# pingooio/pingoo

Hardware: AMD Instinct MI355X
Metric: requests/sec matched (whole node), 1k-rule WAF (higher is better)
Workload: dtype u8

## Files before the change

### pingoo_amd/build.py

```python
from __future__ import annotations

import os
import shutil
import subprocess
import sys

HERE = os.path.dirname(os.path.abspath(__file__))
CSRC = os.path.join(HERE, "csrc")
LIB = os.path.join(HERE, "libpwaf.so")
SOURCES = ["frontend.cpp", "pattern.cpp", "dfa.cpp", "iptrie.cpp", "filter.cpp", "residual.cpp", "residual_jit.cpp", "rtc.cpp", "compile.cpp", "loaders.cpp", "batcher.cpp", "async.cpp", "node.cpp", "engine.cpp", "kernels.hip", "records.hip"]
HEADERS = ["frontend.h", "program.h", "kernels.h", "residual.h", "confirm.h", "records.h", "lscan_split.h", "dirtable.h", "georec.h", "unicode_data.inc", os.path.join("..", "..", "include", "pwaf.h")]


def hipcc() -> str:
    for cand in (os.environ.get("HIPCC"), shutil.which("hipcc"), "/opt/rocm/bin/hipcc"):
        if cand and os.path.exists(cand):
            return cand
    raise RuntimeError("hipcc not found (needed to build pingoo_amd/libpwaf.so)")


EMBED = os.path.join(CSRC, "residual_h.inc")


def embed() -> str:
    text = open(os.path.join(CSRC, "residual.h")).read()
    assert ')RVMH"' not in text
    out = 'R"RVMH(' + text + ')RVMH"\n'
    if not os.path.exists(EMBED) or open(EMBED).read() != out:
        with open(EMBED, "w") as f:
            f.write(out)
    return EMBED


def is_stale(lib: str = LIB) -> bool:
    if not os.path.exists(lib):
        return True
    t = os.path.getmtime(lib)
    return any(os.path.getmtime(os.path.join(CSRC, f)) > t for f in SOURCES + HEADERS)


def build(force: bool = False, verbose: bool = False, variant: str = "") -> str:
    lib = LIB if not variant else os.path.join(HERE, f"libpwaf_{variant}.so")
    if not force and not is_stale(lib):
        return lib
    embed()
    objs = []
    objdir = os.path.join(HERE, "build" + ("_" + variant if variant else ""))
    os.makedirs(objdir, exist_ok=True)
    cc = hipcc()
    common = ["-O3", "-std=c++17", "-fPIC", "-Wall", "-Wextra", "-Wno-unused-parameter", "-I", os.path.join(HERE, "..", "include")]
    common += os.environ.get("PWAF_EXTRA_CXXFLAGS", "").split()
    if variant == "prof":
        common.append("-DPWAF_PROFILING")
    procs = []
    for src in SOURCES:
        obj = os.path.join(objdir, src + ".o")
        objs.append(obj)
        path = os.path.join(CSRC, src)
        if not force and os.path.exists(obj) and os.path.getmtime(obj) > max(os.path.getmtime(path), *(os.path.getmtime(os.path.join(CSRC, h)) for h in HEADERS)):
            continue
        cmd = [cc, *common, "-c", path, "-o", obj]
        if src.endswith(".hip") or src in ("engine.cpp", "rtc.cpp"):
            cmd[1:1] = ["-x", "hip", "--offload-arch=gfx950"]
        else:
            cmd[1:1] = ["-x", "c++"] + (["-fsanitize=address,undefined", "-fno-omit-frame-pointer", "-g", "-O1"] if variant == "asan" else [])
        if verbose:
            print(" ".join(cmd), file=sys.stderr)
        procs.append((src, subprocess.Popen(cmd, stdout=subprocess.PIPE, stderr=subprocess.STDOUT, text=True)))
    for src, p in procs:
        out, _ = p.communicate()
        if p.returncode != 0:
            raise RuntimeError(f"hipcc failed on {src}:\n{out}")
        if verbose and out.strip():
            print(out, file=sys.stderr)
    link = [cc, "--offload-arch=gfx950", "-shared", "-fPIC", *(["-fsanitize=address,undefined", "-shared-libsan"] if variant == "asan" else []), "-o", lib, *objs]
    r = subprocess.run(link, stdout=subprocess.PIPE, stderr=subprocess.STDOUT, text=True)
    if r.returncode != 0:
        raise RuntimeError(f"link failed:\n{r.stdout}")
    return lib


if __name__ == "__main__":
    print(build(force="--force" in sys.argv, verbose=True, variant="prof" if "--prof" in sys.argv else "asan" if "--asan" in sys.argv else ""))
```

### pingoo_amd/csrc/engine.cpp

```cpp
#include <hip/hip_runtime_api.h>

#include <cstdio>
#include <algorithm>
#include <cstring>
#include <map>
#include <memory>
#include <mutex>
#include <string>
#include <type_traits>
#include <unordered_map>
#include <vector>

#include "dirtable.h"
#include "georec.h"
#include "frontend.h"
#include "kernels.h"
#include "lscan_split.h"
#include "program.h"
#include "records.h"

using namespace pwaf;

struct pwaf_program {
    std::unique_ptr<Program> p;
// ... 690 lines not shown
        pt[e->groups.size()] = PassInfo{P.fcmp_base, 0u};
        pt[e->groups.size() + (P.fcmp.empty() ? 0u : 1u)] = PassInfo{P.residual_base, e->residual_jit.function ? (3u << 24) : 0u};
        uint32_t fi = 0;
        for (size_t k = 0; k < e->groups.size(); k++) {
            const DevGroup &d = e->groups[k];
            pt[k].base = d.atom_base;
            pt[k].kind_slot = 0;
            if (d.short_lit) {
                pt[k].kind_slot = 3u << 24;
            } else if (d.filtered) {
                if (d.filter.heads.empty()) pt[k].kind_slot = (1u << 24) | fi;
                fi++;
            } else if (d.visit_slot >= 0) {
                pt[k].kind_slot = (2u << 24) | (uint32_t)d.visit_slot;
            }
        }
        if ((rc = upload(e->pass_table, pt))) return rc;
    }
    return upload(e->colmask, colmask);
}

Scratch &acquire_context(pwaf_engine *e, bool own, hipStream_t caller, std::unique_lock<std::mutex> &held, bool &must_wait) {
    must_wait = false;
    for (int pass = 0; pass < 2; pass++)
        for (auto &c : e->ctx) {
            std::unique_lock<std::mutex> l(c->mu, std::try_to_lock);
            if (!l.owns_lock()) continue;
            const bool ok = pass == 0 ? (c->used && (own ? c->last_own : (!c->last_own && c->last == caller))) : !c->used;
            if (ok) { held = std::move(l); return *c; }
        }
    size_t k;
    {
        std::lock_guard<std::mutex> lock(e->mu);
        k = e->next_ctx;
        e->next_ctx = (e->next_ctx + 1) % e->ctx.size();
    }
    held = std::unique_lock<std::mutex>(e->ctx[k]->mu);
    must_wait = e->ctx[k]->used;
    return *e->ctx[k];
}


struct Layout {
    size_t used = 0;
    size_t take(size_t bytes) { const size_t at = used; used = (used + bytes + 255) & ~(size_t)255; return at; }
    size_t size() const { return used; }
};

uint32_t slab_count(uint32_t total, uint32_t slab0) { return (uint32_t)(((uint64_t)total + kStreamSlab - 1) / kStreamSlab) - slab0; }
uint32_t slabs_of(const FilterArgs &f) { return slab_count(f.total, f.slab0); }
uint32_t pair_cap_of(uint32_t slabs, uint32_t n) { return (uint32_t)std::min<uint64_t>(0xFFFFFFF0u, (uint64_t)slabs * (kStreamSlab / 16) + n + 64); }

struct KernelTimer {
    pwaf_engine *e;
    hipStream_t stream;
    std::unique_lock<std::mutex> lock;
    size_t ev_i = 0;
    long last_main = -1;
    long open_begin = -1;
    bool streaming = false;
    const bool sync_each = switches().sync_each;
    KernelTimer(pwaf_engine *e_, hipStream_t stream_) : e(e_), stream(stream_) {
        if (!e->profiling) return;
        lock = std::unique_lock<std::mutex>(e->prof_mu);
        ev_i = e->n_timed;
    }
    bool off() const { return !e->profiling || (e->profiling == 2 && !streaming); }
    int record(hipStream_t on) {
        if (e->ev.size() < ev_i + 1) {
            hipEvent_t x;
            HIP_TRY(hipEventCreate(&x));
            e->ev.push_back(x);
        }
        HIP_TRY(hipEventRecord(e->ev[ev_i], on));
        ev_i++;
        return PWAF_OK;
    }
    int begin(hipStream_t side = nullptr) {
        if (off()) return PWAF_OK;
        if (!side && last_main >= 0) { open_begin = last_main; return PWAF_OK; }
        const int rc = record(side ? side : stream);
        if (rc) return rc;
        open_begin = (long)ev_i - 1;
        if (!side) last_main = open_begin;
        return PWAF_OK;
    }
    int end(const char *name, uint64_t alg_bytes, hipStream_t side = nullptr) {
        if (sync_each) {
            hipError_t se = hipStreamSynchronize(side ? side : stream);
            fprintf(stderr, "[pwaf] %s done: %s\n", name, hipGetErrorString(se));
        }
        if (off()) return PWAF_OK;
        const int rc = record(side ? side : stream);
        if (rc) return rc;
        if (!side) last_main = (long)ev_i - 1;
        pwaf_kernel_time t{};
        snprintf(t.name, sizeof t.name, "%s", name);
        t.alg_bytes = alg_bytes;
        e->times.push_back(t);
        e->time_ev.push_back({(size_t)open_begin, ev_i - 1});
        return PWAF_OK;
    }
    void commit() { e->n_timed = ev_i; }
};

struct ArgSlotMark {
    Scratch &S;
    hipStream_t stream;
    int slot = -1;
    int record() {
        if (slot < 0) return PWAF_OK;
        const int k = slot;
        slot = -1;
        S.arg_pending[k] = true;
        HIP_TRY(hipEventRecord(S.arg_ev[k], stream));
        return PWAF_OK;
    }
    ~ArgSlotMark() { (void)record(); }
};

struct BatchRun {
    pwaf_engine *e;
    Scratch &S;
    const Program &P;
    const pwaf_batch &db;
    hipStream_t stream;
    const std::vector<uint32_t> *col_begin;
    const Switches &sw;
    KernelTimer prof;
    ArgSlotMark arg_slot;
    uint32_t n, n_groups, residual_pass, n_passes, bit_words, pair_stride;
    size_t n_slots, ctrl_words;
    uint32_t pool_cap = 0;
    uint32_t *status_word = nullptr;
    bool zero_deferred = false;
    size_t zero_bytes = 0;
    std::vector<pwaf_strcol> cols;
    std::vector<uint32_t> col_bytes;
    std::vector<uint8_t> col_known;
    VerdictArgs v{};
    bool ipres_launched = false, attr_launched = false;
    pwaf_geo *d_geo = nullptr;
    ListShape lshapes[2];
    std::vector<uint32_t> filter_index;
    std::vector<FilterArgs> fall;
    std::vector<FilterArgs> by_stride[2];
    std::vector<ConfirmArgs> call;
    std::vector<ListScanArgs> la[2];
    ColPtrChunk ptrs{};
    uint64_t alg_bytes[3] = {0, 0, 0};
    const FilterArgs *d_all = nullptr, *d_s1 = nullptr, *d_s2 = nullptr;
    const ConfirmArgs *d_c = nullptr;
    const ListScanArgs *d_la[2] = {nullptr, nullptr};
    uint32_t *c_plan = nullptr, *l_plan = nullptr;

    BatchRun(pwaf_engine *e_, Scratch &S_, const pwaf_batch &db_, hipStream_t stream_, const std::vector<uint32_t> *col_begin_)
        : e(e_), S(S_), P(*e_->prog.p), db(db_), stream(stream_), col_begin(col_begin_), sw(switches()), prof(e_, stream_), arg_slot{S_, stream_} {
        n = db.n;
        n_groups = (n + 63) / 64;
        residual_pass = (uint32_t)e->groups.size() + (P.fcmp.empty() ? 0u : 1u);
        n_passes = residual_pass + (P.n_residual ? 1u : 0u);
        bit_words = 2 * n_groups;
        pair_stride = std::max(1u, e->n_bit_atoms + e->n_cmp_atoms + e->n_short);
        n_slots = (size_t)std::max(kGapLists, e->n_gated);
        ctrl_words = 2 + n_slots + e->n_filtered;
    }


    int reserve_scratch(bool sync_status) {
        int rc;
        const uint64_t pool_cap64 = std::max<uint64_t>(std::max<uint64_t>(1u << 20, (uint64_t)n * 8), S.pool_entries);
        pool_cap = (uint32_t)std::min<uint64_t>(pool_cap64, 0x7FFFFFF0u);
        S.pool_entries = pool_cap;
        if (!S.status.p) {
            if ((rc = S.status.reserve(8))) return rc;
            HIP_TRY(hipMemsetAsync(S.status.p, 0, 8, stream));
        }
        status_word = (uint32_t *)S.status.p + (sync_status ? 1 : 0);
        if ((rc = S.rec.reserve((size_t)std::max(1u, n_passes) * n * 4))) return rc;
        if ((rc = S.attr.reserve(((size_t)n_groups * pair_stride + 64) * 16 + (size_t)n_groups * 4))) return rc;
        if ((rc = S.pool.reserve((size_t)pool_cap * sizeof(PoolEntry)))) return rc;
        uint32_t n_conf = 0;
        for (const DevGroup &d : e->groups) n_conf += (d.filtered && d.confirm) ? 1u : 0u;
        Layout z;
        const size_t z_ctrl = z.take(4 * ctrl_words), z_cand = z.take((size_t)e->n_filtered * bit_words * 4), z_visit = z.take((size_t)e->n_visit * bit_words * 4),
                     z_walk = z.take((size_t)n_conf * bit_words * 4);
        zero_bytes = z.size();
        if ((rc = S.zero_block.reserve(zero_bytes))) return rc;
        zero_deferred = e->n_filtered != 0;
        for (const DevGroup &d : e->groups) zero_deferred = zero_deferred && (d.gate >= 0 || d.identity || d.short_lit);
        if (!zero_deferred) HIP_TRY(hipMemsetAsync(S.zero_block.p, 0, zero_bytes, stream));
        char *const zbase = (char *)S.zero_block.p;
        S.ctrl.p = zbase + z_ctrl;
        S.cand_bits.p = zbase + z_cand;
        S.visit_bits.p = zbase + z_visit;
        S.walk_bits.p = zbase + z_walk;
        if (e->n_gated && (rc = S.gate_lists.reserve((size_t)e->n_gated * n * 4))) return rc;
        if (e->n_need && (rc = S.need.reserve((size_t)e->n_need * n * 4))) return rc;
        return PWAF_OK;
    }

    int resolve_columns(bool totals_known) {
        int rc;
        cols.resize(e->n_fields);
        col_bytes.assign(e->n_fields, 0);
        for (int f = 0; f < PWAF_N_FIELDS; f++) {
            cols[(size_t)f] = db.field[f];
            col_bytes[(size_t)f] = db.field_bytes[f];
        }
        bool missing_header = false;
        for (uint32_t f = PWAF_N_FIELDS; f < e->n_fields; f++) {
            const uint32_t k = f - PWAF_N_FIELDS;
            if (k < db.n_headers && db.headers != nullptr && db.headers[k].data != nullptr && db.headers[k].offsets != nullptr) {
                cols[f] = db.headers[k];
                col_bytes[f] = db.header_bytes ? db.header_bytes[k] : 0u;
            } else {
                missing_header = true;
            }
        }
        if (missing_header) {
            if (S.zero_off.cap < (size_t)(n + 1) * 4 + PWAF_ARENA_PAD) {
                if ((rc = S.zero_off.reserve((size_t)(n + 1) * 4 + PWAF_ARENA_PAD))) return rc;
                HIP_TRY(hipMemsetAsync(S.zero_off.p, 0, S.zero_off.cap, stream));
            }
            for (uint32_t f = PWAF_N_FIELDS; f < e->n_fields; f++)
                if (cols[f].data == nullptr) {
                    cols[f].data = (const uint8_t *)S.zero_off.p;
                    cols[f].offsets = (const uint32_t *)S.zero_off.p;
                    col_bytes[f] = 0;
                }
        }
        col_known.assign(e->n_fields, totals_known ? 1 : 0);
        for (uint32_t f = 0; f < e->n_fields; f++)
            if (col_bytes[f] != 0 || cols[f].data == (const uint8_t *)S.zero_off.p) col_known[f] = 1;
        return PWAF_OK;
    }

    int fill_verdict_args(pwaf_verdict *d_out, pwaf_counts *d_counts, uint32_t *d_match_idx, uint32_t *d_n_matches) {
        int rc;
        v.n = n;
        v.n_groups = n_groups;
        v.force_global_tables = (P.flags & PWAF_OPT_GLOBAL_VERDICT_TABLES) ? 1u : 0u;
        v.sparse_mode = verdict_mode(P.flags);
        if (v.sparse_mode) {
            const VerdictShape vs = verdict_shape(P.n_cols, (uint32_t)P.rules.size(), e->n_trig, (uint32_t)P.lits.size(), v.force_global_tables != 0, (int)v.sparse_mode, n_passes);
            v.v_cap = vs.v_cap;
            const bool entry_list = v.sparse_mode >= 3;
            const uint32_t spill_cols = entry_list ? P.n_cols : P.n_cols - std::min(vs.v_cap, P.n_cols);
            if (entry_list || spill_cols) {
                if ((rc = S.verdict_spill.reserve((size_t)verdict_blocks_sp(vs, e->n_cus) * vs.waves * spill_cols * 8))) return rc;
                v.spill = (unsigned long long *)S.verdict_spill.p;
            }
        }
        v.debug_skip = sw.debug_skip | (sw.attr_prio ? 0x80000000u : 0u);
        for (int f = 0; f < PWAF_N_FIELDS; f++) v.off[f] = db.field[f].offsets;
        v.ip = db.ip;
        v.ip_is_v6 = db.ip_is_v6;
        v.port = db.port;
        v.flags = db.flags;
        v.asn = db.asn;
        v.country = db.country;
        v.n_cols = P.n_cols;
        v.n_passes = n_passes;
        v.rec = (const uint32_t *)S.rec.p;
        v.passes = (const PassInfo *)e->pass_table.p;
        if (P.n_residual && e->residual_jit.function) {
            v.res_words = (P.n_residual + 31u) / 32u;
            v.res_base = P.residual_base;
            if ((rc = S.res_words.reserve((size_t)v.res_words * n * 4))) return rc;
            v.res_match = (const uint32_t *)S.res_words.p;
        }
        v.cand_bits = (const uint32_t *)S.cand_bits.p;
        v.visit_bits = (const uint32_t *)S.visit_bits.p;
        v.bit_words = bit_words;
        v.n_hlen = (uint32_t)e->hlen_fields.size();
        for (size_t k = 0; k < e->hlen_fields.size(); k++) v.hoff[k] = cols[e->hlen_fields[k]].offsets;
        v.gpairs = (uint4 *)S.attr.p;
        v.ghdr = (uint32_t *)((char *)S.attr.p + ((size_t)n_groups * pair_stride + 64) * 16);
        v.pair_stride = pair_stride;
        v.attr_blocks = e->n_cus;
        v.pool = (const PoolEntry *)S.pool.p;
        v.cmp = (const CmpAtomDev *)e->num_atoms.p;
        v.n_cmp = e->n_cmp_atoms;
        v.cmp_vars = e->cmp_vars;
        v.lazy = (const CmpAtomDev *)e->lazy_atoms.p;
        v.n_lazy = e->n_lazy;
        v.n_lazy_var = (uint32_t)e->lazy_vars.size();
        for (size_t k = 0; k < e->lazy_vars.size(); k++) v.lazy_var[k] = e->lazy_vars[k];
        v.n_short = e->n_short;
        v.short_atoms = (const ShortAtom *)e->short_atoms.p;
        if (e->n_short) {
            v.short_data = cols[(size_t)e->short_field].data;
            v.short_off = cols[(size_t)e->short_field].offsets;
        }
        v.n_trig = e->n_trig;
        v.n_lits = (uint32_t)P.lits.size();
        v.bit_col = (const uint32_t *)e->bit_atoms.p;
        v.trig_off = (const uint32_t *)e->trig_off.p;
        v.trig_rules = (const uint16_t *)e->trig_rules.p;
        v.always_rules = (const uint32_t *)e->always_rules.p;
        for (int var = 0; var < 2; var++) {
            v.iu_vals[var] = (const int64_t *)e->iu_vals[var].p;
            v.iu_masks[var] = (const uint32_t *)e->iu_masks[var].p;
            v.iu_n[var] = e->iu_n[var];
            v.iu_words[var] = e->iu_words[var];
        }
        v.country_masks = (const uint32_t *)e->country_luts.p;
        v.cc_words = e->cc_words;
        v.rules = (const DevRule *)e->rules.p;
        v.n_rules = (uint32_t)P.rules.size();
        v.lits = (const uint32_t *)e->lits.p;
        set_trie_args(e, v);
        if ((rc = S.ipres.reserve((size_t)n * (v.ipres_packed ? 4 : 8) + 64))) return rc;
        v.ipres = (uint32_t *)S.ipres.p;
        v.out = d_out;
        v.counts = (unsigned long long *)d_counts;
        v.match_idx = d_match_idx;
        v.n_matches = d_n_matches;
        return PWAF_OK;
    }

    int zero_head_records() {
        for (size_t k = 0; k < e->groups.size();) {
            size_t k1 = k;
            while (k1 < e->groups.size() && e->groups[k1].filtered && !e->groups[k1].filter.heads.empty()) k1++;
            if (k1 == k) { k++; continue; }
            HIP_TRY(hipMemsetAsync((uint32_t *)S.rec.p + k * (size_t)n, 0, (k1 - k) * (size_t)n * 4, stream));
            k = k1;
        }
        return PWAF_OK;
    }

    void pick_list_shapes() {
        uint32_t variant[2] = {2, 0};
        bool all_confirm = e->n_filtered != 0;
        for (const DevGroup &d : e->groups) all_confirm = all_confirm && (!d.filtered || d.confirm);
        if (all_confirm) variant[0] = 0;
        if (sw.list_shape >= 0) {
            variant[0] = (uint32_t)sw.list_shape & 15u;
            variant[1] = (uint32_t)sw.list_shape >> 4;
        }
        for (int phase = 0; phase < 2; phase++) lshapes[phase] = list_shape(variant[phase]);
    }


    template <class Launch>
    int timed(const char *name, uint64_t bytes, const char *what, Launch &&launch, hipStream_t side = nullptr) {
        const int rc = prof.begin(side);
        if (rc) return rc;
        const int he = launch();
        if (he) return fail(PWAF_E_DEVICE, std::string(what) + " launch failed: " + hipGetErrorString((hipError_t)he));
        return prof.end(name, bytes, side);
    }

    template <class Launch>
    int side_stage(hipStream_t q, const char *name, uint64_t code, const char *what, Launch &&launch) {
        const hipStream_t side = q != stream ? q : nullptr;
        const int rc = timed(name, code, what, launch, side);
        if (rc) return rc;
        if (side) HIP_TRY(hipEventRecord(S.ev_join, q));
        return PWAF_OK;
    }
    int ipres_stage(hipStream_t q) {
        if (ipres_launched) return PWAF_OK;
        ipres_launched = true;
        if (q != stream) {
            HIP_TRY(hipEventRecord(S.ev_fork, stream));
            HIP_TRY(hipStreamWaitEvent(q, S.ev_fork, 0));
        }
        const int rc = side_stage(q, "ipres", 0xFAu, "ipres kernel", [&] { return sw.skip_ipres ? (int)hipMemsetAsync(v.ipres, 0, (size_t)n * (v.ipres_packed ? 4 : 8), q) : launch_ipres(v, q); });
        if (rc || !d_geo) return rc;
        GeoRecArgs ga{};
        set_georec_args(e, ga);
        ga.ip = db.ip;
        ga.ip_is_v6 = db.ip_is_v6;
        ga.asn = db.asn;
        ga.country = db.country;
        ga.n = n;
        ga.out = (uint2 *)d_geo;
        return side_stage(q, "georec", 25ull * n, "georec kernel", [&] { return launch_georec(ga, q); });
    }
    int attr_stage(hipStream_t q) {
        if (attr_launched) return PWAF_OK;
        attr_launched = true;
        if (q == stream && sw.placement == 0) HIP_TRY(hipStreamWaitEvent(stream, S.ev_join, 0));
        return side_stage(q, "attr", 0xFEu, "attribute kernel", [&] { return sw.skip_attr ? (int)hipMemsetAsync(v.ghdr, 0, (size_t)n_groups * 4, q) : launch_attr(v, q); });
    }
    int attr_at_start() {
        int rc;
        if (sw.placement == 0) return ipres_stage(S.side);
        if (sw.placement == 3) return (rc = ipres_stage(S.side)) ? rc : attr_stage(S.side);
        return PWAF_OK;
    }
    int attr_after_filter() {
        int rc;
        switch (sw.placement) {
        case 0: return attr_stage(stream);
        case 1: return (rc = ipres_stage(stream)) ? rc : attr_stage(stream);
        case 2: return (rc = ipres_stage(S.side)) ? rc : attr_stage(S.side);
        default: return PWAF_OK;
        }
    }
    int join_side() {
        if (sw.placement >= 2) HIP_TRY(hipStreamWaitEvent(stream, S.ev_join, 0));
        return PWAF_OK;
    }

    int launch_plain_scans() {
        static const char *fn[5] = {"host", "url", "path", "method", "user_agent"};
        for (size_t gi = 0; gi < e->groups.size(); gi++) {
            const DevGroup &d = e->groups[gi];
            if (d.gate >= 0 || d.identity || d.short_lit) continue;
            const ScanArgs a = scan_args(gi);
            char nm[48];
            if (d.field < PWAF_N_FIELDS) snprintf(nm, sizeof nm, "scan_%s_g%zu", fn[d.field], gi);
            else snprintf(nm, sizeof nm, "scan_hdr%u_g%zu", d.field - PWAF_N_FIELDS, gi);
            prof.streaming = true;
            const int rc = timed(nm, (uint64_t)col_bytes[d.field] + 4ull * (n + 1), "scan kernel", [&] { return launch_scan(a, stream); });
            prof.streaming = false;
            if (rc) return rc;
        }
        return PWAF_OK;
    }

    int launch_filter_stage() {
        prof.streaming = true;
        const int rc = timed(by_stride[1].empty() ? "filter_s1" : by_stride[0].empty() ? "filter_s2" : "filter_mix", alg_bytes[1] + alg_bytes[2], "filter kernel", [&] {
            return launch_filter(by_stride[0].data(), (uint32_t)by_stride[0].size(), d_s1, by_stride[1].data(), (uint32_t)by_stride[1].size(), d_s2, stream);
        });
        prof.streaming = false;
        return rc;
    }
    int launch_resolve_stage() {
        bool any_list = false;
        for (const DevGroup &d : e->groups) any_list = any_list || (d.filtered && !d.confirm);
        return timed("resolve+compact", 0xFCu, "resolve / compact kernel", [&] {
            const int he = launch_resolve(fall.data(), (uint32_t)fall.size(), d_all, stream);
            return !he && any_list ? launch_compact(fall.data(), (uint32_t)fall.size(), d_all, stream) : he;
        });
    }
    int launch_confirm_stage() {
        if (call.empty()) return PWAF_OK;
        return timed("confirm", 0xF8u, "confirm kernel", [&] { return launch_confirm(call.data(), (uint32_t)call.size(), d_c, c_plan, e->n_cus, stream); });
    }
    int launch_list_scans() {
        uint32_t *plan_at = l_plan;
        for (int phase = 0; phase < 2; phase++) {
            uint32_t first = 0;
            for (const uint32_t cnt : e->lscan_launches[phase]) {
                char nm[48];
                snprintf(nm, sizeof nm, "lscan_x%u", cnt);
                const int rc = timed(nm, 0xFDu, "gated scan kernel", [&] { return launch_scan_gated(la[phase].data() + first, cnt, d_la[phase] + first, plan_at, lshapes[phase], stream); });
                if (rc) return rc;
                plan_at += 2 * cnt + 1;
                first += cnt;
            }
        }
        return PWAF_OK;
    }
    int launch_fcmp_stage() {
        if (P.fcmp.empty()) return PWAF_OK;
        FcmpArgs fa{};
        std::vector<uint32_t> slots;
        for (size_t k = 0; k < P.fcmp.size(); k++) {
            uint32_t sl[2];
            const uint32_t fld[2] = {P.fcmp[k].a, P.fcmp[k].b};
            for (int q = 0; q < 2; q++) {
                size_t at = std::find(slots.begin(), slots.end(), fld[q]) - slots.begin();
                if (at == slots.size()) slots.push_back(fld[q]);
                sl[q] = (uint32_t)at;
            }
            fa.atoms[k] = P.fcmp[k].op | (sl[0] << 8) | (sl[1] << 16);
        }
        for (size_t q = 0; q < slots.size() && q < kMaxFcmpFields; q++) {
            fa.data[q] = cols[slots[q]].data;
            fa.off[q] = cols[slots[q]].offsets;
        }
        fa.n = n;
        fa.n_atoms = (uint32_t)P.fcmp.size();
        fa.rec = (uint32_t *)S.rec.p + e->groups.size() * (size_t)n;
        set_pool(fa);
        return timed("fcmp", 0xFBu, "field comparison kernel", [&] { return launch_fcmp(fa, stream); });
    }
    template <class Args>
    int residual_inputs(Args &a) {
        a.data = (const uint8_t *const *)S.res_cols.p;
        a.off = (const uint32_t *const *)((const char *)S.res_cols.p + (size_t)e->n_fields * 8);
        a.blob = (const uint8_t *)e->residual_blob.p;
        a.n = n;
        a.n_rules = P.n_residual;
        a.ip = db.ip;
        a.ip_is_v6 = db.ip_is_v6;
        a.port = db.port;
        a.asn = db.asn;
        a.country = db.country;
        a.has_geo = (P.has_geo && P.residual_needs_geo) ? 1u : 0u;
        a.geo_root4 = (const uint32_t *)e->geo_rec_root4.p;
        a.geo_root6 = (const uint32_t *)e->geo_rec_root6.p;
        a.geo_nodes = (const uint32_t *)e->geo_rec_nodes.p;
        a.geo_recs = (const GeoRec *)e->geo_recs.p;
        a.rule_errors = (unsigned long long *)e->residual_errors.p;
        if (S.retry) {
            const int rc = S.err_sink.reserve((size_t)P.n_residual * 8);
            if (rc) return rc;
            a.rule_errors = (unsigned long long *)S.err_sink.p;
        }
        return PWAF_OK;
    }
    int launch_residual_stage() {
        if (!P.n_residual) return PWAF_OK;
        int rc;
        if (e->residual_jit.function) {
            ResidualJitArgs ja{};
            if ((rc = residual_inputs(ja))) return rc;
            ja.match_words = (uint32_t *)S.res_words.p;
            return timed("residual_jit", 0xF9u, "specialized residual kernel", [&] { return launch_residual_jit(e->residual_jit, ja, e->n_cus, stream); });
        }
        ResidualArgs ra{};
        if ((rc = residual_inputs(ra))) return rc;
        ra.rec = (uint32_t *)S.rec.p + (size_t)residual_pass * n;
        set_pool(ra);
        return timed("residual", 0xF9u, "residual kernel", [&] { return launch_residual(ra, stream); });
    }
    int launch_verdict_stage() { return timed("verdict", 0xFFu, "verdict kernel", [&] { return launch_verdict(v, stream); }); }
    int dump_counts() {
        std::vector<uint32_t> cw(ctrl_words);
        HIP_TRY(hipStreamSynchronize(stream));
        HIP_TRY(hipMemcpy(cw.data(), S.ctrl.p, 4 * ctrl_words, hipMemcpyDeviceToHost));
        fprintf(stderr, "[pwaf] n %u pool %u status %u |", n, cw[0], cw[1]);
        for (size_t k = 0; k < e->groups.size(); k++) {
            const DevGroup &d = e->groups[k];
            if (d.gate >= 0) fprintf(stderr, " pass %zu field %u %s list %u", k, d.field, d.filtered ? (d.confirm ? "confirm" : "filtered") : "gap", cw[2 + (size_t)d.gate]);
        }
        for (uint32_t k = 0; k < e->n_filtered; k++) fprintf(stderr, " pairs[%u] %u", k, cw[2 + n_slots + k]);
        fprintf(stderr, "\n");
        return PWAF_OK;
    }


    template <class Args>
    void set_pool(Args &a) const {
        a.pool = (PoolEntry *)S.pool.p;
        a.pool_count = (uint32_t *)S.ctrl.p;
        a.pool_cap = pool_cap;
        a.status = status_word;
    }
    bool feeds_gates(size_t gi) const { return e->n_gap && e->owns_factors[gi]; }
    template <class Args>
    void set_gate_feed(Args &a, const DevGroup &d) const {
        a.colmask_local = (const uint32_t *)e->colmask.p + d.atom_base;
        a.n_local = d.n_local;
        a.gate_lists = (uint32_t *)S.gate_lists.p;
        a.gate_count = (uint32_t *)S.ctrl.p + 2;
        if constexpr (!std::is_same<Args, ScanArgs>::value) {
            a.enq_bits = (uint32_t *)S.visit_bits.p;
            a.enq_words = bit_words;
        }
    }

    ScanArgs scan_args(size_t gi) const {
        const DevGroup &d = e->groups[gi];
        ScanArgs a{};
        if (feeds_gates(gi)) set_gate_feed(a, d);
        a.data = cols[d.field].data;
        a.off = cols[d.field].offsets;
        a.n = n;
        a.tab = (const uint16_t *)d.tab.p;
        a.classmap = (const uint8_t *)d.classmap.p;
        a.umap = d.scalar_mode ? (const uint8_t *)d.classmap.p + kUmapAt : nullptr;
        a.ill_class = d.ill_class;
        a.special = (const SpecialCell *)d.special.p;
        a.list_off = (const uint32_t *)d.list_off.p;
        a.list = (const uint16_t *)d.list.p;
        a.start_emit = d.start_emit;
        a.emit_base = d.emit_base;
        a.n_cus = e->n_cus;
        a.chunks = d.chunks;
        a.special_base = d.special_base;
        a.n_states = d.n_states;
        a.stride = d.stride;
        a.n_classes = d.n_classes;
        a.n_hot = d.n_hot;
        a.rec = (uint32_t *)S.rec.p + gi * (size_t)n;
        set_pool(a);
        return a;
    }

    int learn_arena_sizes() {
        bool ask = false;
        for (const DevGroup &d : e->groups)
            if (d.filtered && !col_known[d.field]) {
                HIP_TRY(hipMemcpyAsync(&col_bytes[d.field], cols[d.field].offsets + n, 4, hipMemcpyDeviceToHost, stream));
                ask = true;
            }
        if (ask) HIP_TRY(hipStreamSynchronize(stream));
        return PWAF_OK;
    }

    uint32_t slab0_of(uint32_t field) const { return col_begin ? (*col_begin)[field] / kStreamSlab : 0u; }

    int build_filter_args() {
        int rc;
        filter_index.assign(e->groups.size(), 0);
        if (!e->n_filtered) return PWAF_OK;
        const uint32_t words = (n + 31) / 32, n_cblocks = (words + kCompactWords - 1) / kCompactWords;
        uint64_t sub_entries = 0, n_slabs_all = 0, pair_bytes = 0;
        for (const DevGroup &d : e->groups)
// ... 69 lines not shown
        }
        return PWAF_OK;
    }

    ConfirmArgs confirm_args(const FilterArgs &f, const DevGroup &d, size_t gi, uint32_t wi) const {
        ConfirmArgs c{};
        c.data = f.data;
        c.off = f.off;
        c.n = n;
        c.total = f.total;
        c.pairs = f.pairs;
        c.pair_count = f.pair_count;
        c.pair_cap = f.pair_cap;
        c.mul = f.mul;
        c.stride = f.stride;
        c.init = f.init;
        c.ftable = f.table;
        c.c_head = (const uint32_t *)d.c_head.p;
        c.c_entries = (const ConfirmEntry *)d.c_entries.p;
        c.c_bytes = (const uint8_t *)d.c_bytes.p;
        c.c_classes = (const uint32_t *)d.c_classes.p;
        c.n_entries = (uint32_t)d.filter.confirm.entries.size();
        c.n_bytes = (uint32_t)d.filter.confirm.bytes.size() & ~3u;
        c.n_class_words = (uint32_t)d.filter.confirm.classes.size();
        c.rec = f.rec;
        c.valid_bits = f.bitmap;
        c.dense_flag = f.dense_flag;
        c.dense_thresh = f.dense_thresh;
        c.walk_bits = (uint32_t *)S.walk_bits.p + (size_t)wi * bit_words;
        if (d.confirm_walk) {
            c.walk_list = f.list;
            c.walk_count = f.list_count;
        }
        set_pool(c);
        if (feeds_gates(gi)) {
            set_gate_feed(c, d);
            c.shared_bits = d.shared_bits;
        }
        return c;
    }
    void build_confirm_args() {
        for (size_t gi = 0; gi < e->groups.size(); gi++) {
            const DevGroup &d = e->groups[gi];
            if (d.filtered && d.confirm) call.push_back(confirm_args(fall[filter_index[gi]], d, gi, (uint32_t)call.size()));
        }
    }

    ListScanArgs list_args(size_t gi, const ListShape &lshape, bool full_table = false) const {
        const DevGroup &d = e->groups[gi];
        ListScanArgs a{};
        const DevGroup &src = d.share_owner >= 0 ? e->groups[(size_t)d.share_owner] : d;
        if (!d.identity) {
            a.req_list = (const uint32_t *)S.gate_lists.p + (size_t)src.gate * n;
            a.n_list = (const uint32_t *)S.ctrl.p + 2 + src.gate;
        }
        if (d.visit_slot >= 0) a.visited = (uint32_t *)S.visit_bits.p + (size_t)d.visit_slot * bit_words;
        if (d.share_owner >= 0) {
            a.need_in = (const uint32_t *)S.need.p + (size_t)src.need_slot * n;
            a.need_bit = (uint32_t)d.gate;
        }
        if (feeds_gates(gi)) {
            set_gate_feed(a, d);
            if (d.need_slot >= 0) {
                a.need_out = (uint32_t *)S.need.p + (size_t)d.need_slot * n;
                a.shared_bits = d.shared_bits;
            }
        }
        if (d.confirm) a.merge_rec = 1;
        a.behind_filter = d.filtered ? 1u : 0u;
        a.data = cols[d.field].data;
        a.off = cols[d.field].offsets;
        a.n = n;
        const FlatDev &F = (d.confirm && d.rt.n_states && !full_table) ? d.rt : d.fl;
        a.flat = (const uint16_t *)F.flat.p;
        a.classmap = (const uint8_t *)F.flat_classmap.p;
        a.umap = F.scalar_mode ? (const uint8_t *)F.flat_classmap.p + kUmapAt : nullptr;
        a.ill_class = F.ill_class;
        a.n_classes = F.n_classes;
        const uint32_t row_bytes = 2u * (F.n_classes + 3u), hb = list_hot_bytes(lshape);
        if (F.n_delta && (uint64_t)F.n_full * row_bytes + 48u + 8ull * F.n_delta <= hb) {
            a.n_hot = F.n_full;
            a.n_delta = F.n_delta;
            a.delta = (const uint64_t *)F.delta.p;
        } else {
            a.n_hot = std::min<uint32_t>(F.n_delta ? F.n_full : F.n_states, (hb - 48u) / row_bytes);
        }
        a.emit_off = (const uint32_t *)F.emit_off.p;
        a.emit_list = (const uint16_t *)F.emit_list.p;
        a.end_off = (const uint32_t *)F.end_off.p;
        a.end_list = (const uint16_t *)F.end_list.p;
        a.rec = (uint32_t *)S.rec.p + gi * (size_t)n;
        set_pool(a);
        a.n_cus = e->n_cus;
        return a;
    }
    const FilterArgs *dense_of(size_t gi) const {
        const FilterArgs *f = e->groups[gi].filtered ? &fall[filter_index[gi]] : nullptr;
        return f && f->dense_flag ? f : nullptr;
    }
    static void set_dense(ListScanArgs &a, const FilterArgs &f, uint32_t mode) {
        a.dense_flag = f.dense_flag;
        a.dense_thresh = f.dense_thresh;
        a.dense_mode = mode;
    }
    void build_list_args() {
        for (int phase = 0; phase < 2; phase++)
            for (size_t gi = 0; gi < e->groups.size(); gi++) {
                const DevGroup &d = e->groups[gi];
                if (d.identity ? phase != 0 : (d.gate < 0 || d.filtered != (phase == 0))) continue;
                const FilterArgs *const dense = phase == 0 && d.confirm ? dense_of(gi) : nullptr;
                const FilterArgs *const owner_dense = d.share_owner >= 0 ? dense_of((size_t)d.share_owner) : nullptr;
                if (dense) {
                    ListScanArgs a = list_args(gi, lshapes[phase], true);
                    a.req_list = nullptr;
                    a.n_list = nullptr;
                    a.merge_rec = 0;
                    a.visited = (uint32_t *)S.cand_bits.p + (size_t)filter_index[gi] * bit_words;
                    set_dense(a, *dense, 1);
                    la[phase].push_back(a);
                }
                if (d.confirm && !d.confirm_walk) continue;
                if (sw.skip_identity && d.identity) continue;
                ListScanArgs a = list_args(gi, lshapes[phase]);
                if (dense) set_dense(a, *dense, 2);
                else if (owner_dense) set_dense(a, *owner_dense, 3);
                la[phase].push_back(a);
            }
    }
    int check_list_plan() const {
        for (int phase = 0; phase < 2; phase++) {
            size_t planned = 0;
            for (const uint32_t c : e->lscan_launches[phase]) planned += c;
            if (planned != la[phase].size()) return fail(PWAF_E_DEVICE, "list-scan launch plan does not match the batch's descriptors");
        }
        return PWAF_OK;
    }
    void build_column_pointers() {
        if (!P.n_residual) return;
        const size_t nc = e->n_fields;
        ptrs.count = (uint32_t)(2 * nc);
        for (size_t f = 0; f < nc; f++) { ptrs.p[f] = cols[f].data; ptrs.p[nc + f] = cols[f].offsets; }
    }

    int upload_descriptors() {
        int rc;
        struct Part { size_t at; const void *src; size_t bytes; };
        const size_t b_all = fall.size() * sizeof(FilterArgs), b_s1 = by_stride[0].size() * sizeof(FilterArgs), b_s2 = by_stride[1].size() * sizeof(FilterArgs),
                     b_c = call.size() * sizeof(ConfirmArgs), b_l0 = la[0].size() * sizeof(ListScanArgs), b_l1 = la[1].size() * sizeof(ListScanArgs),
                     b_ptrs = (size_t)ptrs.count * sizeof(void *);
        Layout L;
        const Part up[7] = {{L.take(b_all), fall.data(), b_all}, {L.take(b_s1), by_stride[0].data(), b_s1}, {L.take(b_s2), by_stride[1].data(), b_s2}, {L.take(b_c), call.data(), b_c},
                            {L.take(b_l0 + sizeof(ListScanArgs)), la[0].data(), b_l0}, {L.take(b_l1 + sizeof(ListScanArgs)), la[1].data(), b_l1}, {L.take(b_ptrs), ptrs.p, b_ptrs}};
        const size_t up_bytes = L.size();
        const size_t a_cplan = L.take((call.size() + 2) * 4), a_lplan = L.take((lsplit::plan_words(e->lscan_launches[0]) + lsplit::plan_words(e->lscan_launches[1])) * 4);
        if ((rc = S.args.reserve(L.size()))) return rc;
        char *const abase = (char *)S.args.p;
        d_all = (const FilterArgs *)(abase + up[0].at);
        d_s1 = (const FilterArgs *)(abase + up[1].at);
        d_s2 = (const FilterArgs *)(abase + up[2].at);
        d_c = (const ConfirmArgs *)(abase + up[3].at);
        d_la[0] = (const ListScanArgs *)(abase + up[4].at);
        d_la[1] = (const ListScanArgs *)(abase + up[5].at);
        S.res_cols.p = abase + up[6].at;
        c_plan = (uint32_t *)(abase + a_cplan);
        l_plan = (uint32_t *)(abase + a_lplan);
        if (up_bytes) {
            const uint32_t slot = S.arg_next++ % Scratch::kArgSlots;
            if (S.arg_pending[slot]) HIP_TRY(hipEventSynchronize(S.arg_ev[slot]));
            if ((rc = S.arg_slot[slot].reserve(up_bytes))) return rc;
            char *const hb = (char *)S.arg_slot[slot].p;
            for (const Part &p : up)
                if (p.bytes) memcpy(hb + p.at, p.src, p.bytes);
            arg_slot.slot = (int)slot;
            const int he = upload_args_block(hb, S.args.p, up_bytes, zero_deferred ? S.zero_block.p : nullptr, zero_deferred ? zero_bytes : 0, stream);
            if (he) return fail(PWAF_E_DEVICE, std::string("descriptor upload failed: ") + hipGetErrorString((hipError_t)he));
        } else if (zero_deferred) {
            HIP_TRY(hipMemsetAsync(S.zero_block.p, 0, zero_bytes, stream));
        }
        zero_deferred = false;
        return PWAF_OK;
    }
};

int run_pipeline(pwaf_engine *e, Scratch &S, const pwaf_batch &db , pwaf_verdict *d_out, pwaf_counts *d_counts, uint32_t *d_match_idx,
                 uint32_t *d_n_matches, hipStream_t stream, bool totals_known = false, const std::vector<uint32_t> *col_begin = nullptr, bool sync_status = false,
                 pwaf_geo *d_geo = nullptr, const HitOut *d_hits = nullptr) {
    if (db.n == 0) return PWAF_OK;
    BatchRun b(e, S, db, stream, col_begin);
    b.d_geo = d_geo;
    int rc;
    if ((rc = b.reserve_scratch(sync_status)) || (rc = b.resolve_columns(totals_known))) return rc;
    if ((rc = b.fill_verdict_args(d_out, d_counts, d_match_idx, d_n_matches)) || (rc = b.zero_head_records())) return rc;
    if (d_hits && d_hits->any()) {
        b.v.hits = d_hits->hits;
        b.v.hits_cap = d_hits->cap;
        b.v.n_hits = d_hits->n_hits;
        b.v.rule_hits = (unsigned long long *)d_hits->rule_hits;
    }
    b.pick_list_shapes();
    if ((rc = b.attr_at_start()) || (rc = b.launch_plain_scans())) return rc;
    if ((rc = b.learn_arena_sizes()) || (rc = b.build_filter_args())) return rc;
    b.build_confirm_args();
    b.build_list_args();
    b.build_column_pointers();
    if ((rc = b.check_list_plan()) || (rc = b.upload_descriptors())) return rc;
    if (e->n_filtered) {
        if ((rc = b.launch_filter_stage())) return rc;
        if (!b.sw.attr_after_compact && (rc = b.attr_after_filter())) return rc;
        if ((rc = b.launch_resolve_stage()) || (rc = b.launch_confirm_stage())) return rc;
    }
    if ((rc = b.attr_after_filter())) return rc;
    if ((rc = b.launch_list_scans()) || (rc = b.launch_fcmp_stage()) || (rc = b.launch_residual_stage())) return rc;
    if ((rc = b.join_side()) || (rc = b.launch_verdict_stage())) return rc;
    if (b.sw.dump_counts && (rc = b.dump_counts())) return rc;
    if ((rc = b.arg_slot.record())) return rc;
    b.prof.commit();
    return PWAF_OK;
}

hipError_t mark_context_used(Scratch &S, hipStream_t s, bool own) {
    S.used = true;
    S.last = s;
    S.last_own = own;
    return hipEventRecord(S.done, s);
}

int device_error(const char *call, hipError_t he) { return fail(PWAF_E_DEVICE, std::string(call) + ": " + hipGetErrorString(he)); }

template <class After>
int run_with_retry(pwaf_engine *e, Scratch &S, const pwaf_batch &db, pwaf_verdict *d_out, pwaf_counts *d_counts, bool known, const std::vector<uint32_t> *begins, bool counts_zero,
                   After &&after, pwaf_geo *d_geo = nullptr, const HitOut *d_hits = nullptr) {
    const hipStream_t s = S.stream;
    int r = S.pin_status.reserve(16);
    volatile uint32_t *const st = (volatile uint32_t *)S.pin_status.p;
    for (int attempt = 0;; attempt++) {
        hipError_t he = hipSuccess;
        if (!r && d_counts && !(counts_zero && attempt == 0) && (he = hipMemsetAsync(d_counts, 0, sizeof *d_counts, s)) != hipSuccess) r = device_error("hipMemsetAsync", he);
        if (!r && d_hits && d_hits->n_hits && (he = hipMemsetAsync(d_hits->n_hits, 0, 4, s)) != hipSuccess) r = device_error("hipMemsetAsync", he);
        if (!r && d_hits && d_hits->rule_hits && e->prog.p->n_user_rules && (he = hipMemsetAsync(d_hits->rule_hits, 0, (size_t)e->prog.p->n_user_rules * 8, s)) != hipSuccess)
            r = device_error("hipMemsetAsync", he);
        if (!r) {
            S.retry = attempt > 0;
            r = run_pipeline(e, S, db, d_out, d_counts, nullptr, nullptr, s, known, begins, true, d_geo, d_hits);
            S.retry = false;
        }
        if (!r) {
            he = hipMemcpyAsync((void *)&st[0], (uint32_t *)S.status.p + 1, 4, hipMemcpyDeviceToHost, s);
            if (he == hipSuccess) he = hipMemcpyAsync((void *)&st[1], S.ctrl.p, 4, hipMemcpyDeviceToHost, s);
            r = he != hipSuccess ? device_error("hipMemcpyAsync", he) : after();
        }
        const hipError_t re = mark_context_used(S, s, true), se = hipStreamSynchronize(s);
        if (r) return r;
        if (re != hipSuccess) return device_error("hipEventRecord", re);
        if (se != hipSuccess) return device_error("hipStreamSynchronize", se);
        if (!st[0]) return PWAF_OK;
        HIP_TRY(hipMemsetAsync((uint32_t *)S.status.p + 1, 0, 4, s));
        if (attempt >= 2 || st[1] >= 0x7FFFFFF0u) return fail(PWAF_E_NOMEM, "scan overflow pool exhausted: verdicts of this batch are incomplete");
        S.pool_entries = (uint64_t)st[1] + st[1] / 4 + 1024;
    }
}

struct DeviceBatch {
    pwaf_batch db{};
    std::vector<pwaf_strcol> hdr_cols;
    std::vector<uint32_t> hdr_bytes;
    DeviceBatch(uint32_t n, uint32_t n_fields) : hdr_cols(n_fields - PWAF_N_FIELDS, pwaf_strcol{nullptr, nullptr}), hdr_bytes(n_fields - PWAF_N_FIELDS, 0) {
        db.struct_size = sizeof db;
        db.n = n;
        db.memory = PWAF_MEM_DEVICE;
        db.n_headers = (uint32_t)hdr_cols.size();
        db.headers = hdr_cols.empty() ? nullptr : hdr_cols.data();
        db.header_bytes = hdr_bytes.empty() ? nullptr : hdr_bytes.data();
    }
    DeviceBatch(const DeviceBatch &) = delete;
    void set_col(uint32_t f, const void *data, const void *offsets, uint32_t bytes) {
        const pwaf_strcol c{(const uint8_t *)data, (const uint32_t *)offsets};
        if (f < PWAF_N_FIELDS) {
            db.field[f] = c;
            db.field_bytes[f] = bytes;
        } else {
            hdr_cols[f - PWAF_N_FIELDS] = c;
            hdr_bytes[f - PWAF_N_FIELDS] = bytes;
        }
    }
    void set_fixed(const void *ip, const void *ip_is_v6, const void *port, const void *flags, const void *asn, const void *country) {
        db.ip = (const uint8_t *)ip;
        db.ip_is_v6 = (const uint8_t *)ip_is_v6;
        db.port = (const uint16_t *)port;
        db.flags = (const uint8_t *)flags;
        db.asn = (const uint32_t *)asn;
        db.country = (const uint16_t *)country;
    }
};

}

extern "C" {

uint32_t pwaf_abi_version(void) { return PWAF_ABI_VERSION; }
const char *pwaf_last_error(void) { return g_last_error.c_str(); }

int pwaf_compile_expression(const char *expression, char *errbuf, size_t errbuf_len) {
    Syntax syn;
    std::string err;
    bool ok = expression && parse_expression(expression, syn, err);
    if (!ok) {
        std::string m = "Expression is not valid: " + (expression ? err : std::string("null expression"));
        if (errbuf && errbuf_len) snprintf(errbuf, errbuf_len, "%s", m.c_str());
        return fail(PWAF_E_SYNTAX, m);
    }
    return PWAF_OK;
}

int pwaf_validate_expression(const char *expression, char *errbuf, size_t errbuf_len) {
    auto bad = [&](const std::string &why) {
        std::string m = "Expression is not valid: " + why;
        if (errbuf && errbuf_len) snprintf(errbuf, errbuf_len, "%s", m.c_str());
        return fail(PWAF_E_SYNTAX, m);
// ... 1418 lines not shown
```

### pingoo_amd/csrc/kernels.h

```cpp
#pragma once
#include <cstdint>
#include <string>
#include <vector>

#include "program.h"

namespace pwaf {

static constexpr int kMaxPasses = 250;
static constexpr int kVerdictPre = 12;
static constexpr uint32_t kGapLists = 32;
static constexpr uint32_t kMaxHeaderLens = 8;
static constexpr uint32_t kDirChunkWords = 32;

static constexpr uint32_t REC_OVERFLOW = 0x80000000u;
struct PoolEntry {
    uint32_t atom;
    uint32_t next;
};

struct SpecialCell {
    uint32_t next_off;
    uint32_t emit;
};
struct ScanArgs {
    const uint8_t *data;
    const uint32_t *off;
    uint32_t n;
    const uint16_t *tab;
    const uint8_t *classmap;
    const uint8_t *umap;
    uint32_t ill_class;
    const SpecialCell *special;
    const uint32_t *list_off;
    const uint16_t *list;
    uint32_t n_states, stride, n_classes, n_hot;
    uint32_t start_emit;
    uint32_t emit_base, special_base;
    uint32_t n_cus;
    uint32_t chunks;
    uint32_t *rec;
    PoolEntry *pool;
    uint32_t *pool_count;
    uint32_t pool_cap;
    uint32_t *status;
    const uint32_t *colmask_local;
    uint32_t n_local;
    uint32_t *gate_lists;
    uint32_t *gate_count;
};

static constexpr uint32_t kListThreads = 512;
static constexpr uint32_t kListWalks = 1;
static constexpr uint32_t kListHotBytes = 48 * 1024;
struct ListScanArgs {
    const uint8_t *data;
    const uint32_t *off;
    uint32_t n;
    const uint16_t *flat;
    const uint8_t *classmap;
    const uint8_t *umap;
    uint32_t ill_class;
    uint32_t n_classes;
    uint32_t n_hot;
    const uint64_t *delta;
    uint32_t n_delta;
    const uint32_t *emit_off;
    const uint16_t *emit_list;
    const uint32_t *end_off;
    const uint16_t *end_list;
    uint32_t *rec;
    PoolEntry *pool;
    uint32_t *pool_count;
    uint32_t pool_cap;
    uint32_t *status;
    const uint32_t *colmask_local;
    uint32_t n_local;
    uint32_t *gate_lists;
    uint32_t *gate_count;
    uint32_t *enq_bits;
    uint32_t enq_words;
    uint32_t behind_filter;
    const uint32_t *req_list;
    const uint32_t *n_list;
    uint32_t *visited;
    uint32_t *need_out;
    uint32_t shared_bits;
    const uint32_t *need_in;
    uint32_t need_bit;
    uint32_t merge_rec;
    uint32_t n_cus;
    const uint32_t *dense_flag;
    uint32_t dense_thresh;
    uint32_t dense_mode;
};
struct ListOf {
    const uint32_t *req_list;
    uint32_t n_l;
};

struct ConfirmArgs {
    const uint8_t *data;
    const uint32_t *off;
    uint32_t n;
    uint32_t total;
    const uint2 *pairs;
    const uint32_t *pair_count;
    uint32_t pair_cap;
    uint32_t mul, stride, init;
    const uint32_t *ftable;
    const uint32_t *c_head;
    const ConfirmEntry *c_entries;
    const uint8_t *c_bytes;
    const uint32_t *c_classes;
    uint32_t n_entries, n_bytes, n_class_words;
    uint32_t *rec;
    uint32_t *valid_bits;
    uint32_t *walk_bits;
    uint32_t *walk_list;
    uint32_t *walk_count;
    PoolEntry *pool;
    uint32_t *pool_count;
    uint32_t pool_cap;
    uint32_t *status;
    const uint32_t *colmask_local;
    uint32_t n_local;
    uint32_t *gate_lists;
    uint32_t *gate_count;
    uint32_t *enq_bits;
    uint32_t enq_words;
    uint32_t shared_bits;
    const uint32_t *dense_flag;
    uint32_t dense_thresh;
};
static constexpr uint32_t kConfirmThreads = 1024;
static constexpr uint32_t kConfirmPoolBytes = 40 * 1024;
struct ConfirmTableDev {
    const ConfirmArgs *c;
    uint32_t count;
};
int launch_confirm(const ConfirmArgs *host, uint32_t count, const ConfirmArgs *dev, uint32_t *plan, uint32_t n_cus, void *stream);

static constexpr uint32_t kStreamSlab = 128 * 1024;
static constexpr uint32_t kStreamIter = 4096;
static constexpr uint32_t kFilterWaves = 4;
static constexpr uint32_t kCompactWords = 2048;
struct FilterArgs {
    const uint8_t *data;
    const uint32_t *off;
    uint32_t n;
    uint32_t total;
    uint32_t slab0;
    uint32_t init;
    uint32_t mul;
    uint32_t stride;
    const uint32_t *table;
    uint32_t n_heads;
    uint32_t head_w[2][4];
    uint32_t head_m[2][4];
    uint32_t head_len[2];
    uint32_t head_code[2];
    uint32_t *rec;
    uint32_t *chunk_bits;
    uint32_t *sub_count;
    uint32_t *bitmap;
    uint32_t *block_count;
    uint32_t *list;
    uint32_t *list_count;
    uint2 *pairs;
    uint32_t *pair_count;
    uint32_t pair_cap;
    uint32_t *pair_base;
    const uint32_t *dense_flag;
    uint32_t dense_thresh;
    uint32_t first_block;
    uint32_t debug;
};
int upload_args_block(const void *host_pinned, void *dev, size_t bytes, void *zero , size_t zero_bytes, void *stream);
struct FilterTable {
    const FilterArgs *f;
    uint32_t count;
};
struct FilterMix {
    const FilterArgs *f1, *f2;
    uint32_t count1, count2, blocks1, blocks2;
};
int launch_filter(const FilterArgs *host1, uint32_t count1, const FilterArgs *dev1, const FilterArgs *host2, uint32_t count2, const FilterArgs *dev2, void *stream);
int launch_resolve(const FilterArgs *host, uint32_t count, const FilterArgs *dev, void *stream);
int launch_compact(const FilterArgs *host, uint32_t count, const FilterArgs *dev, void *stream);
int configure_kernels(int device);

static constexpr uint32_t kSrcSet = 0, kSetWordsMax = 16, kSrcCc = 16, kCcWordsMax = 8, kSrcPort = 24, kSrcAsn = 28, kIntWordsMax = 4, kSrcAcmp = 32, kAcmpWordsMax = 4,
                          kSrcWords = 36;
struct PassInfo {
    uint32_t base;
    uint32_t kind_slot;
};
struct FcmpArgs {
    const uint8_t *data[kMaxFcmpFields];
    const uint32_t *off[kMaxFcmpFields];
    uint32_t atoms[kMaxFcmpAtoms];
    uint32_t n, n_atoms;
    uint32_t *rec;
    PoolEntry *pool;
    uint32_t *pool_count;
    uint32_t pool_cap;
    uint32_t *status;
};
int launch_fcmp(const FcmpArgs &a, void *stream);
struct ResidualArgs {
    const uint8_t *const *data;
    const uint32_t *const *off;
    const uint8_t *blob;
    uint32_t n, n_rules;
    const uint8_t *ip;
    const uint8_t *ip_is_v6;
    const uint16_t *port;
    const uint32_t *asn;
    const uint16_t *country;
    uint32_t has_geo;
    const uint32_t *geo_root4, *geo_root6, *geo_nodes;
    const GeoRec *geo_recs;
    uint32_t *rec;
    PoolEntry *pool;
    uint32_t *pool_count;
    uint32_t pool_cap;
    uint32_t *status;
    unsigned long long *rule_errors;
};
int launch_residual(const ResidualArgs &a, void *stream);
struct ResidualJitArgs {
    const uint8_t *const *data;
    const uint32_t *const *off;
    const uint8_t *blob;
    uint32_t n, n_rules;
    const uint8_t *ip;
    const uint8_t *ip_is_v6;
    const uint16_t *port;
    const uint32_t *asn;
    const uint16_t *country;
    uint32_t has_geo, pad;
    const uint32_t *geo_root4, *geo_root6, *geo_nodes;
    const GeoRec *geo_recs;
    uint32_t *match_words;
    unsigned long long *rule_errors;
};
struct JitKernel {
    void *module = nullptr, *function = nullptr;
};
static constexpr uint32_t kMaxJitRules = 256;
bool rvm_specialize(const uint8_t *blob, size_t len, std::string &out, std::string &why);
bool rvm_jit_program(const uint8_t *blob, size_t len, std::string &out, std::string &why);
bool rtc_compile(const std::string &source, const std::string &arch, std::vector<char> &code, std::string &why);
bool jit_load(const std::vector<char> &code, JitKernel &out, std::string &why);
void jit_release(JitKernel &k);
int launch_residual_jit(const JitKernel &k, const ResidualJitArgs &a, uint32_t n_cus, void *stream);
struct ColPtrChunk {
    const void *p[2 * (PWAF_N_FIELDS + kMaxHeaders)];
    uint32_t count;
};
struct CmpAtomDev {
    uint32_t col, c;
};
struct ShortAtom {
    uint32_t col;
    uint32_t len_exact;
    uint32_t lit_lo, lit_hi;
};
struct VerdictArgs {
    uint32_t n, n_groups;
    uint32_t debug_skip;
    uint32_t force_global_tables;
    uint32_t sparse_mode;
    uint32_t v_cap;
    unsigned long long *spill;
    const uint32_t *off[PWAF_N_FIELDS];
    const uint8_t *ip;
    const uint8_t *ip_is_v6;
    const uint16_t *port;
    const uint8_t *flags;
    const uint32_t *asn;
    const uint16_t *country;
    uint32_t n_passes;
    const uint32_t *rec;
    const PassInfo *passes;
    const uint32_t *res_match;
    uint32_t res_words, res_base;
    const uint32_t *cand_bits, *visit_bits;
    uint32_t bit_words;
    const uint32_t *hoff[kMaxHeaderLens];
    const ShortAtom *short_atoms;
    uint32_t n_short;
    const uint8_t *short_data;
    const uint32_t *short_off;
    uint32_t n_hlen;
    const PoolEntry *pool;
    uint32_t n_cols;
    const CmpAtomDev *cmp;
    uint32_t n_cmp;
    uint32_t cmp_vars;
    const CmpAtomDev *lazy;
    uint32_t n_lazy;
    uint32_t lazy_var[4], n_lazy_var;
    const uint32_t *bit_col;
    const int64_t *iu_vals[2];
    const uint32_t *iu_masks[2];
    uint32_t iu_n[2], iu_words[2];
    const uint32_t *country_masks;
    uint32_t cc_words;
    const DevRule *rules;
    uint32_t n_rules;
    const uint32_t *lits;
    uint32_t n_lits, n_trig;
    const uint32_t *trig_off;
    const uint16_t *trig_rules;
    const uint32_t *always_rules;
    const uint32_t *ip_root4, *ip_root6, *ip_nodes;
    const uint32_t *set_masks;
    uint32_t set_words;
    uint32_t n_ip_lists;
    const uint32_t *geo_root4, *geo_root6, *geo_nodes;
    const uint32_t *dir24;
    const uint32_t *dir_chunks, *dir_vals;
    const uint32_t *dir_summary;
    uint32_t dir_sum_shift, dir_common;
    const uint2 *dir_esc;
    const uint32_t *class_rows;
    uint32_t class_words;
    uint32_t acmp_words;
    uint32_t geo_default;
    uint32_t *ipres;
    uint32_t ipres_packed;
    uint32_t has_geo;
    uint4 *gpairs;
    uint32_t *ghdr;
    uint32_t pair_stride;
    uint32_t attr_blocks;
    pwaf_verdict *out;
    unsigned long long *counts;
    uint32_t *match_idx;
    uint32_t *n_matches;
    pwaf_rule_hit *hits;
    uint32_t hits_cap;
    uint32_t *n_hits;
    unsigned long long *rule_hits;
};

int launch_scan(const ScanArgs &a, void *stream);
struct GatedTable {
    const ListScanArgs *g;
    uint32_t count;
    uint32_t debug;
};
struct ListShape {
    uint32_t threads, hot_bytes, wg_per_cu;
};
ListShape list_shape(uint32_t variant);
uint32_t list_hot_bytes(const ListShape &shape);
int launch_scan_gated(const ListScanArgs *host, uint32_t count, const ListScanArgs *dev, uint32_t *plan, const ListShape &shape, void *stream);
int launch_verdict(const VerdictArgs &a, void *stream);
int launch_ipres(const VerdictArgs &a, void *stream);
int launch_attr(const VerdictArgs &a, void *stream);
int launch_dir24(const VerdictArgs &a, void *out , void *esc, void *esc_count, void *stream);
struct GeoRecArgs {
    const uint8_t *ip, *ip_is_v6;
    const uint32_t *asn;
    const uint16_t *country;
    uint32_t n, has_geo;
    const uint32_t *root4, *root6, *nodes;
    const GeoRec *recs;
    const uint32_t *chunks, *vals, *summary;
    uint32_t sum_shift, common;
    uint32_t n_cus;
    uint2 *out;
};
int launch_georec(const GeoRecArgs &a, void *stream);
uint32_t scan_lds_bytes(uint32_t n_hot, uint32_t stride, uint32_t n_gate_atoms);
struct VerdictShape {
    uint32_t waves, lds_bytes, lds_tables;
    uint32_t sparse, v_cap, per_cu;
};
VerdictShape verdict_shape(uint32_t n_cols, uint32_t n_rules, uint32_t n_trig, uint32_t n_lits, bool force_global = false, int mode = 3, uint32_t n_passes = 0);
uint32_t verdict_blocks_sp(const VerdictShape &sh, uint32_t n_cus);

}
```

### pingoo_amd/csrc/kernels.hip

```cpp
#include <hip/hip_runtime.h>

#include <cstdlib>
#include <mutex>
#include <set>

#include "confirm.h"
#include "utf8.h"
#include "kernels.h"
#include "residual.h"

namespace pwaf {

static constexpr int kScanThreads = 1024;
static constexpr int kScanWaves = kScanThreads / 64;
static constexpr uint32_t kNone = 0xFFFFFFFFu;

#define PWAF_LDS __attribute__((address_space(3)))
#define PWAF_GLOBAL __attribute__((address_space(1)))
typedef const PWAF_LDS uint16_t *lds_u16_ptr;
typedef const PWAF_GLOBAL uint16_t *glb_u16_ptr;
typedef const PWAF_LDS uint32_t *lds_u32_ptr;
typedef const PWAF_LDS uint8_t *lds_u8_ptr;
typedef unsigned int u32x4 __attribute__((ext_vector_type(4)));
typedef u32x4 u32x4_u __attribute__((aligned(1)));

static constexpr uint32_t kClsBytes = 1024;
uint32_t scan_lds_bytes(uint32_t n_hot, uint32_t stride, uint32_t n_gate_atoms) {
    const uint32_t need = (((n_hot + 1) * stride * 2 + 15) & ~15u) + kClsBytes + n_gate_atoms * 4;
    const uint32_t reach = ((0xFFFFu << 1) + stride * 2 + kClsBytes + 15) & ~15u;
    return need > reach ? need : reach;
}


struct Hits {
    uint32_t a0, a1;
    uint32_t ovf;
};

struct SlowCtx {
    const uint32_t *list_off;
    const uint16_t *list;
    PoolEntry *pool;
    uint32_t *pool_count;
    uint32_t *status;
    uint32_t pool_cap;
};

__device__ __forceinline__ Hits pool_push(const SlowCtx &c, uint32_t atom, Hits h) {
    const uint32_t idx = atomicAdd(c.pool_count, 1u);
    if (idx >= c.pool_cap) {
        atomicOr(c.status, 1u);
        return h;
    }
    c.pool[idx].atom = atom;
    c.pool[idx].next = h.ovf;
    h.ovf = idx;
    return h;
}

__device__ __forceinline__ Hits record_atom(const SlowCtx &c, uint32_t atom, Hits h) {
    if (h.ovf == kNone) {
        if (h.a0 == atom + 1 || h.a1 == atom + 1) return h;
        if (h.a0 == 0) { h.a0 = atom + 1; return h; }
        if (h.a1 == 0) { h.a1 = atom + 1; return h; }
        const uint32_t x0 = h.a0 - 1, x1 = h.a1 - 1;
        h = pool_push(c, x0, h);
        h = pool_push(c, x1, h);
        return pool_push(c, atom, h);
    }
    for (uint32_t i = h.ovf; i != kNone;) {
        const uint32_t at = __hip_atomic_load(&c.pool[i].atom, __ATOMIC_RELAXED, __HIP_MEMORY_SCOPE_AGENT);
        if (at == atom) return h;
        i = __hip_atomic_load(&c.pool[i].next, __ATOMIC_RELAXED, __HIP_MEMORY_SCOPE_AGENT);
    }
    return pool_push(c, atom, h);
}

__device__ __noinline__ Hits emit_list(const uint32_t *list_off, const uint16_t *list, PoolEntry *pool, uint32_t *pool_count, uint32_t *status,
                                       uint32_t pool_cap, uint32_t id, Hits h) {
    const SlowCtx c{list_off, list, pool, pool_count, status, pool_cap};
    const uint32_t b = list_off[id], e = list_off[id + 1];
    for (uint32_t k = b; k < e; k++) h = record_atom(c, list[k], h);
    return h;
}
struct Walk {
    uint32_t row, crow;
    Hits h;
};
__device__ __noinline__ Walk careful_step(const PWAF_GLOBAL unsigned char *gtab, const SpecialCell *special, const uint32_t *list_off, const uint16_t *list,
                                          PoolEntry *pool, uint32_t *ctrl , uint32_t pool_cap, uint32_t hot_emit ,
                                          uint32_t special_col , uint32_t prev, uint32_t crow, uint32_t c2k, uint32_t t, uint32_t a0,
                                          uint32_t a1, uint32_t ovf) {
    const SlowCtx c{list_off, list, pool, ctrl, ctrl + 1, pool_cap};
    const uint32_t hot_elems = hot_emit & 0xFFFFu, emit_base = hot_emit >> 16, special_base = special_col & 0xFFFFu, emit_col2 = special_col >> 16;
    const Hits h{a0, a1, ovf};
    uint32_t cell = t;
    if (prev == hot_elems) cell = *reinterpret_cast<glb_u16_ptr>(gtab + crow + c2k);
    Walk w{cell, crow, h};
    if (cell >= special_base) {
        const SpecialCell sp = special[cell - special_base];
        w.row = hot_elems;
        w.crow = sp.next_off;
        if (sp.emit) {
            const uint32_t b = list_off[sp.emit - 1], e = list_off[sp.emit];
            for (uint32_t k = b; k < e; k++) w.h = record_atom(c, list[k], w.h);
        }
    } else if (cell >= emit_base) {
        const uint32_t code = *reinterpret_cast<lds_u16_ptr>((uintptr_t)((cell << 1) + emit_col2 + kClsBytes));
        if (code & 0x8000u) {
            w.h = record_atom(c, code & 0x7FFFu, w.h);
        } else {
            const uint32_t b = list_off[code - 1], e = list_off[code];
            for (uint32_t k = b; k < e; k++) w.h = record_atom(c, list[k], w.h);
        }
    }
    return w;
}
__device__ __forceinline__ Hits hits_of_record(const uint32_t rv) {
    if (rv & REC_OVERFLOW) return Hits{0, 0, rv & ~REC_OVERFLOW};
    return Hits{rv & 0x7FFFu, (rv >> 15) & 0x7FFFu, kNone};
}
__device__ __noinline__ uint32_t gate_mask(const uint32_t *colmask_local, const PoolEntry *pool, Hits h) {
    uint32_t need = 0;
    if (h.ovf != kNone) {
        for (uint32_t i = h.ovf; i != kNone;) {
            need |= colmask_local[__hip_atomic_load(&pool[i].atom, __ATOMIC_RELAXED, __HIP_MEMORY_SCOPE_AGENT)];
            i = __hip_atomic_load(&pool[i].next, __ATOMIC_RELAXED, __HIP_MEMORY_SCOPE_AGENT);
        }
    } else {
        if (h.a0) need |= colmask_local[h.a0 - 1];
        if (h.a1) need |= colmask_local[h.a1 - 1];
    }
    return need;
}
__device__ __noinline__ void enqueue_mask(uint32_t *gate_lists, uint32_t *gate_count, uint32_t n, uint32_t r, uint32_t need) {
    while (need) {
        const uint32_t g = (uint32_t)__builtin_ctz(need);
        need &= need - 1;
        gate_lists[(size_t)g * n + atomicAdd(&gate_count[g], 1u)] = r;
    }
}
__device__ __noinline__ void enqueue_mask_once(uint32_t *gate_lists, uint32_t *gate_count, uint32_t n, uint32_t r, uint32_t need, uint32_t *enq_bits, uint32_t enq_words) {
    while (need) {
        const uint32_t g = (uint32_t)__builtin_ctz(need);
        need &= need - 1;
        if (enq_bits != nullptr) {
            const uint32_t bit = 1u << (r & 31u);
            if (atomicOr(&enq_bits[(size_t)g * enq_words + (r >> 5)], bit) & bit) continue;
        }
        gate_lists[(size_t)g * n + atomicAdd(&gate_count[g], 1u)] = r;
    }
}
__device__ __forceinline__ void enqueue_gated(const uint32_t *colmask_local, const PoolEntry *pool, uint32_t *gate_lists, uint32_t *gate_count, uint32_t n,
                                              uint32_t r, Hits h) {
    enqueue_mask(gate_lists, gate_count, n, r, gate_mask(colmask_local, pool, h));
}

__device__ __forceinline__ uint32_t wave_index() { return (uint32_t)__builtin_amdgcn_readfirstlane((int)(threadIdx.x >> 6)); }

// ... 106 lines not shown
        if (want != 0 && next < w1) {
            const uint32_t avail = min(w1 - next, blk + 64 - next);
            const uint32_t rank = (uint32_t)__builtin_popcountll(want & lt_mask);
            const bool take = last && r2 == kNone && rank < avail;
            const uint32_t j = take ? next + rank - blk : 0;
            const uint32_t lo = (uint32_t)__builtin_amdgcn_ds_bpermute((int)(j << 2), (int)o_lo);
            const uint32_t hi = (uint32_t)__builtin_amdgcn_ds_bpermute((int)(j << 2), (int)o_hi);
            if (take) {
                r2 = next + rank;
                p2 = lo;
                end2 = hi;
            }
            next += min((uint32_t)__builtin_popcountll(want), avail);
            if (next == blk + 64 && next < w1) {
                blk += 64;
                if (n_base == blk) {
                    o_lo = n_lo;
                    o_hi = n_hi;
                } else {
                    load_off(blk, o_lo, o_hi);
                }
            }
        }
        if (__ballot(r != kNone || r2 != kNone) == 0) break;
        {
            const bool have = last ? (r2 != kNone && p2 < end2) : true;
            const uint32_t np = have ? (last ? p2 : p + kStep) : 0u;
            const uint32_t nend = last ? end2 : end;
#pragma unroll
            for (int q = 0; q < CH; q++) {
                const uint32_t at = (q == 0 || (have && np + 16u * q < nend)) ? np + 16u * q : 0u;
                wn[q] = *reinterpret_cast<const PWAF_GLOBAL u32x4_u *>(gdata + at);
            }
        }

        const bool act = r != kNone && p < end;
        const uint32_t cnt_all = act ? min(kStep, end - p) : 0u;
#pragma unroll
        for (int q = 0; q < CH; q++) {
        const uint32_t cnt = cnt_all > 16u * q ? min(16u, cnt_all - 16u * q) : 0u;
        const uint32_t wd[4] = {w[q].x, w[q].y, w[q].z, w[q].w};
        uint32_t c2[16];
#pragma unroll
        for (int k = 0; k < 16; k++) {
            const uint32_t byte = (wd[k >> 2] >> ((k & 3) * 8)) & 0xFFu;
            const uint32_t c = WIDE ? *reinterpret_cast<lds_u32_ptr>((uintptr_t)(byte << 2)) : (uint32_t)*reinterpret_cast<lds_u8_ptr>((uintptr_t)byte);
            c2[k] = (uint32_t)k < cnt ? c : stay2;
        }
        if (a.umap != nullptr && __ballot(cnt != 0u && window_has_high(w[q])) != 0ull) {
            const uint32_t f_start = r != kNone ? a.off[r] : 0u;
#pragma unroll
            for (int k = 0; k < 16; k++) {
                const uint32_t byte = (wd[k >> 2] >> ((k & 3) * 8)) & 0xFFu;
                if (byte >= 0xC0u && (uint32_t)k < cnt) c2[k] = 2u * lead_class(a.umap, a.ill_class, gdata, byte, p + 16u * (uint32_t)q + (uint32_t)k, end);
                else if (byte >= 0x80u && (uint32_t)k < cnt) c2[k] = cont_class(c2[k], 2u * a.ill_class, gdata, p + 16u * (uint32_t)q + (uint32_t)k, f_start, end);
            }
        }
#pragma unroll
        for (int k0 = 0; k0 < 16; k0 += 4) {
            const uint32_t t1 = *reinterpret_cast<lds_u16_ptr>((uintptr_t)((row << 1) + c2[k0] + kClsBytes));
            const uint32_t t2 = *reinterpret_cast<lds_u16_ptr>((uintptr_t)((t1 << 1) + c2[k0 + 1] + kClsBytes));
            const uint32_t t3 = *reinterpret_cast<lds_u16_ptr>((uintptr_t)((t2 << 1) + c2[k0 + 2] + kClsBytes));
            const uint32_t t4 = *reinterpret_cast<lds_u16_ptr>((uintptr_t)((t3 << 1) + c2[k0 + 3] + kClsBytes));
            if (max(max(t1, t2), max(t3, t4)) >= emit_base) {
                uint32_t cur = row;
                bool chain = true;
                auto redo = [&](const uint32_t ts, const uint32_t cls, const bool in_range) {
                    const uint32_t t = chain ? ts : (uint32_t)*reinterpret_cast<lds_u16_ptr>((uintptr_t)((cur << 1) + cls + kClsBytes));
                    if (in_range) {
                        bool slow = t >= special_base;
                        if (!slow && t >= emit_base) {
                            const uint32_t code = *reinterpret_cast<lds_u16_ptr>((uintptr_t)((t << 1) + emit_col2 + kClsBytes));
                            const uint32_t x = (code & 0x7FFFu) + 1;
                            if (!(code & 0x8000u) || h.ovf != kNone) slow = true;
                            else if (h.a0 == x || h.a1 == x) {}
                            else if (h.a0 == 0) h.a0 = x;
                            else if (h.a1 == 0) h.a1 = x;
                            else slow = true;
                        }
                        if (slow) {
                            const Walk wk = careful_step(gtab, a.special, a.list_off, a.list, a.pool, a.pool_count, a.pool_cap, hot_elems | (emit_base << 16),
                                                         special_base | (emit_col2 << 16), cur, crow, cls, t, h.a0, h.a1, h.ovf);
                            chain = chain && wk.row == t;
                            cur = wk.row;
                            crow = wk.crow;
                            h = wk.h;
                        } else {
                            cur = t;
                        }
                    } else {
                        chain = chain && t < special_base;
                    }
                };
                redo(t1, c2[k0], (uint32_t)k0 < cnt);
                redo(t2, c2[k0 + 1], (uint32_t)(k0 + 1) < cnt);
                redo(t3, c2[k0 + 2], (uint32_t)(k0 + 2) < cnt);
                redo(t4, c2[k0 + 3], (uint32_t)(k0 + 3) < cnt);
                row = cur;
            } else {
                row = t4;
            }
        }
        }
        p += cnt_all;

        if (r != kNone && p >= end) {
            const uint32_t e = row == hot_elems ? (uint32_t)*reinterpret_cast<glb_u16_ptr>(gtab + crow + (end_col << 1))
                                                : (uint32_t)*reinterpret_cast<lds_u16_ptr>((uintptr_t)(((row + end_col) << 1) + kClsBytes));
            if (e & 0x8000u) {
                const uint32_t x = (e & 0x7FFFu) + 1;
                if (h.ovf == kNone && (h.a0 == x || h.a1 == x)) {
                } else if (h.ovf == kNone && h.a0 == 0) {
                    h.a0 = x;
                } else if (h.ovf == kNone && h.a1 == 0) {
                    h.a1 = x;
                } else {
                    const SlowCtx sc{a.list_off, a.list, a.pool, a.pool_count, a.status, a.pool_cap};
                    h = record_atom(sc, x - 1, h);
                }
            } else if (e) {
                PWAF_EMIT(e - 1);
            }
            a.rec[r] = h.ovf != kNone ? (REC_OVERFLOW | h.ovf) : (h.a0 | (h.a1 << 15));
            if (a.colmask_local != nullptr && (h.a0 | (h.ovf + 1u)) != 0) {
                uint32_t need = 1;
                if (h.ovf == kNone) {
                    need = *reinterpret_cast<lds_u32_ptr>((uintptr_t)(gate_base + (h.a0 - 1) * 4));
                    if (h.a1) need |= *reinterpret_cast<lds_u32_ptr>((uintptr_t)(gate_base + (h.a1 - 1) * 4));
                }
                if (need) enqueue_gated(a.colmask_local, a.pool, a.gate_lists, a.gate_count, a.n, r, h);
            }
            r = kNone;
        }
        if (r == kNone && r2 != kNone) {
            r = r2;
            p = p2;
            end = end2;
            r2 = kNone;
            row = 0;
            h = Hits{0, 0, kNone};
            if (start_emit) PWAF_EMIT(start_emit - 1);
        }
#pragma unroll
        for (int q = 0; q < CH; q++) w[q] = wn[q];
        n_lo = f_lo;
        n_hi = f_hi;
        n_base = f_base;
    }
}

template <int CH, bool WIDE>
__global__ __launch_bounds__(kScanThreads) void scan_kernel(ScanArgs a) { scan_body<CH, WIDE>(a); }

__device__ __forceinline__ ListOf list_of(const ListScanArgs &a) {
    ListOf l{a.req_list, a.req_list != nullptr ? min(*a.n_list, a.n) : a.n};
    if (a.dense_mode != 0u) {
        const bool dense = *a.dense_flag > a.dense_thresh;
        if (a.dense_mode == 1u && !dense) l.n_l = 0u;
        if (a.dense_mode == 2u && dense) l.n_l = 0u;
        if (a.dense_mode == 3u && dense) l = ListOf{nullptr, a.n};
    }
    return l;
}

__global__ __launch_bounds__(256) void lscan_plan_kernel(GatedTable b, uint32_t *plan , uint32_t n_waves) {
    __shared__ uint32_t part[256];
    __shared__ unsigned long long all_entries;
    const uint32_t t = threadIdx.x;
    uint32_t items = 0;
    const uint32_t n_l = t < b.count ? list_of(b.g[t]).n_l : 0u;
    if (t == 0) all_entries = 0ull;
    __syncthreads();
    if (n_l != 0u) atomicAdd(&all_entries, (unsigned long long)n_l);
    __syncthreads();
    if (t < b.count) {
        const uint32_t room = n_waves > b.count ? n_waves - b.count : 1u;
        const unsigned long long per_wave = (all_entries + room - 1u) / room;
        uint32_t epi = 1;
        while (epi < 16u && epi < per_wave) epi <<= 1;
        while (epi < 64u * kListWalks && (n_l + epi - 1) / epi > n_waves) epi <<= 1;
        items = (n_l + epi - 1) / epi;
        plan[b.count + 1 + t] = epi;
    }
    part[t] = items;
    __syncthreads();
    for (uint32_t d = 1; d < 256; d <<= 1) {
        const uint32_t v = t >= d ? part[t - d] : 0u;
        __syncthreads();
        part[t] += v;
        __syncthreads();
    }
    if (t < b.count) plan[t] = part[t] - items;
    if (t == 0) plan[b.count] = part[255];
}

__device__ __forceinline__ uint32_t list_step_slow(const uint16_t *hot, const PWAF_GLOBAL uint16_t *flat, const uint64_t *delta, const uint32_t state, const uint32_t c,
                                                   const uint32_t stride, const uint32_t n_hot, const uint32_t n_delta) {
    if (state < n_hot) return hot[state * stride + c];
    const uint32_t k = state - n_hot;
    if (k < n_delta) {
        if (c + 2u == stride) return state;
        const uint64_t rec = delta[k];
        const uint32_t lo = (uint32_t)rec, hi = (uint32_t)(rec >> 32);
        if (c == ((lo >> 16) & 0xFFu)) return hi & 0xFFFFu;
        if (c == (lo >> 24)) return hi >> 16;
        return hot[(lo & 0xFFFFu) * stride + c];
    }
    return flat[state * stride + c];
}

template <uint32_t THREADS>
__device__ __forceinline__ void lscan_async(const ListScanArgs &a, const uint16_t *hot, const unsigned char *cls, const uint64_t *delta, uint32_t it, const uint32_t it_end,
                                            const uint32_t first, const uint32_t n_l, const uint32_t hot_elems, const uint32_t epi) {
    const uint32_t ncls = a.n_classes, stride = ncls + 3u;
    const PWAF_GLOBAL unsigned char *gdata = (const PWAF_GLOBAL unsigned char *)a.data;
    const PWAF_GLOBAL uint16_t *flat = (const PWAF_GLOBAL uint16_t *)a.flat;
    auto record_emit = [&](const uint32_t st, Hits &hh) {
        const uint32_t ei = st * stride + ncls;
        const uint32_t code = ei < hot_elems ? (uint32_t)hot[ei] : (uint32_t)flat[ei];
        const uint32_t x = (code & 0x7FFFu) + 1u;
        bool slow = !(code & 0x8000u) || hh.ovf != kNone;
        if (!slow) {
            if (hh.a0 == x || hh.a1 == x) {}
            else if (hh.a0 == 0) hh.a0 = x;
            else if (hh.a1 == 0) hh.a1 = x;
            else slow = true;
        }
        if (slow) hh = emit_list(a.emit_off, a.emit_list, a.pool, a.pool_count, a.status, a.pool_cap, st, hh);
    };
    for (it += wave_index(); it < it_end; it += THREADS / 64u) {
        const uint32_t li = (it - first) * epi + (threadIdx.x & 63u);
        bool live = (threadIdx.x & 63u) < epi && li < n_l;
        if (live && a.need_in != nullptr) live = ((a.need_in[li] >> a.need_bit) & 1u) != 0;
        const uint32_t r = live ? (a.req_list != nullptr ? a.req_list[li] : li) : 0u;
        if (live && a.visited != nullptr) atomicOr(&a.visited[r >> 5], 1u << (r & 31u));
        uint32_t p = live ? a.off[r] : 0u;
        const uint32_t end = live ? a.off[r + 1] : 0u;
        uint32_t state = 0, wp = p;
        Hits h{0, 0, kNone};
        uint32_t need_init = 0;
        if (live && a.merge_rec) {
            h = hits_of_record(a.rec[r]);
            if (a.colmask_local != nullptr && (h.a0 | (h.ovf + 1u)) != 0) need_init = gate_mask(a.colmask_local, a.pool, h);
        }
        if (live && a.emit_off[1] != a.emit_off[0]) h = emit_list(a.emit_off, a.emit_list, a.pool, a.pool_count, a.status, a.pool_cap, 0u, h);
        u32x4 w = *reinterpret_cast<const PWAF_GLOBAL u32x4_u *>(gdata + wp);
        u32x4 wn = *reinterpret_cast<const PWAF_GLOBAL u32x4_u *>(gdata + (wp + 16u < end ? wp + 16u : 0u));
        for (;;) {
            const bool active = p < end;
            const unsigned long long am = __ballot(active);
            if (am == 0) break;
            if (active && p - wp >= 16u) {
                w = wn;
                wp += 16u;
                wn = *reinterpret_cast<const PWAF_GLOBAL u32x4_u *>(gdata + (wp + 16u < end ? wp + 16u : 0u));
            }
            const uint32_t j = (p - wp) >> 2;
            const uint32_t wd = j == 0 ? w.x : j == 1 ? w.y : j == 2 ? w.z : w.w;
            const uint32_t cnt = active ? min(4u, end - p) : 0u;
            uint32_t c[4], t[4], sv[4];
#pragma unroll
            for (uint32_t k = 0; k < 4; k++) c[k] = cls[(wd >> (k * 8)) & 0xFFu];
            asm volatile("" : "+v"(c[0]), "+v"(c[1]), "+v"(c[2]), "+v"(c[3]));
            if (a.umap != nullptr && __ballot(active && (wd & 0x80808080u) != 0u) != 0ull) {
                const uint32_t f_start = active ? a.off[r] : 0u;
#pragma unroll
                for (uint32_t k = 0; k < 4; k++) {
                    const uint32_t byte = (wd >> (k * 8)) & 0xFFu;
                    if (byte >= 0xC0u && k < cnt) c[k] = lead_class(a.umap, a.ill_class, gdata, byte, p + k, end);
                    else if (byte >= 0x80u && k < cnt) c[k] = cont_class(c[k], a.ill_class, gdata, p + k, f_start, end);
                }
            }
#pragma unroll
            for (uint32_t k = 0; k < 4; k++) c[k] = k < cnt ? c[k] : ncls + 1u;
#pragma unroll
            for (uint32_t k = 0; k < 4; k++) {
                t[k] = *reinterpret_cast<lds_u16_ptr>((uintptr_t)min(__umul24(k == 0 ? state : sv[k - 1], 2u * stride) + 2u * c[k], 2u * hot_elems));
                sv[k] = t[k] & 0x7FFFu;
            }
            const uint32_t any = t[0] | t[1] | t[2] | t[3], top = max(max(t[0], t[1]), max(t[2], t[3]));
            const bool blocked = active && top == 0xFFFFu;
            const unsigned long long bm = __ballot(blocked);
            const uint32_t n_blocked = (uint32_t)__builtin_popcountll(bm);
            if (n_blocked < 32u && bm != am) {
                if (active && !blocked) {
                    if (any & 0x8000u) {
#pragma unroll
                        for (uint32_t k = 0; k < 4; k++)
                            if (t[k] & 0x8000u) record_emit(sv[k], h);
                    }
                    state = sv[3];
                    p += 4u;
                }
            } else if (blocked) {
#pragma unroll
                for (uint32_t k = 0; k < 4; k++) {
                    const uint32_t tt = list_step_slow(hot, flat, delta, state, c[k], stride, a.n_hot, a.n_delta);
                    state = tt & 0x7FFFu;
                    if (tt & 0x8000u) record_emit(state, h);
                }
                p += 4u;
            }
        }
        if (live) {
            if (a.end_off[state + 1] != a.end_off[state]) h = emit_list(a.end_off, a.end_list, a.pool, a.pool_count, a.status, a.pool_cap, state, h);
            a.rec[r] = h.ovf != kNone ? (REC_OVERFLOW | h.ovf) : (h.a0 | (h.a1 << 15));
            if (a.colmask_local != nullptr) {
                uint32_t need = 0;
                if ((h.a0 | (h.ovf + 1u)) != 0) need = gate_mask(a.colmask_local, a.pool, h);
                if (a.need_out != nullptr) a.need_out[li] = need;
                need &= ~(a.shared_bits | need_init);
                if (need) enqueue_mask_once(a.gate_lists, a.gate_count, a.n, r, need, a.enq_bits, a.enq_words);
            }
        }
    }
}

template <uint32_t THREADS>
__global__ __launch_bounds__(THREADS, THREADS == 512 ? 6 : 4) void lscan_kernel(GatedTable b, const uint32_t *plan, uint32_t hot_bytes) {
    extern __shared__ uint32_t lscan_lds[];
    __builtin_amdgcn_s_setprio(3);
    if ((uint32_t)(uintptr_t)(PWAF_LDS unsigned char *)lscan_lds != 0u) __builtin_trap();
    const uint32_t total = plan[b.count];
    const uint32_t it0 = (uint32_t)((uint64_t)total * blockIdx.x / gridDim.x), it1 = (uint32_t)((uint64_t)total * (blockIdx.x + 1) / gridDim.x);
    const unsigned char *cls = reinterpret_cast<const unsigned char *>(lscan_lds + (hot_bytes + 16u) / 4);
    const uint16_t *hot = reinterpret_cast<const uint16_t *>(lscan_lds);
    for (uint32_t it = it0; it < it1;) {
        uint32_t ps = 0;
        for (uint32_t lo = 0, hi = b.count; lo + 1 < hi;) {
            const uint32_t mid = (lo + hi) >> 1;
            if (plan[mid] <= it) lo = mid;
            else hi = mid;
            ps = lo;
        }
        const uint32_t first = plan[ps], it_end = min(it1, plan[ps + 1]), epi = plan[b.count + 1 + ps];
        ListScanArgs a = load_descriptor(&b.g[ps]);
        const ListOf lst = list_of(a);
        a.req_list = lst.req_list;
        const uint32_t ncls = a.n_classes, stride = ncls + 3u;
        const uint32_t hot_elems = a.n_hot * stride;
        uint64_t *delta_lds = reinterpret_cast<uint64_t *>(lscan_lds) + (hot_elems * 2u + 2u + 15u) / 16u * 2u;
        __syncthreads();
        {
            const uint4 *src = reinterpret_cast<const uint4 *>(a.flat);
            uint4 *dst = reinterpret_cast<uint4 *>(lscan_lds);
            const uint32_t units = (hot_elems * 2u + 15u) / 16u;
            for (uint32_t k = threadIdx.x; k < units; k += THREADS * 4u) {
                uint4 v[4];
#pragma unroll
                for (uint32_t q = 0; q < 4; q++) v[q] = k + q * THREADS < units ? src[k + q * THREADS] : make_uint4(0u, 0u, 0u, 0u);
#pragma unroll
                for (uint32_t q = 0; q < 4; q++)
                    if (k + q * THREADS < units) dst[k + q * THREADS] = v[q];
            }
            if (threadIdx.x < 64) lscan_lds[(hot_bytes + 16u) / 4 + threadIdx.x] = reinterpret_cast<const uint32_t *>(a.classmap)[threadIdx.x];
            for (uint32_t k = threadIdx.x; k < a.n_delta; k += THREADS) delta_lds[k] = a.delta[k];
        }
        __syncthreads();
        if (threadIdx.x == 0) reinterpret_cast<uint16_t *>(lscan_lds)[hot_elems] = 0xFFFFu;
        __syncthreads();
        const uint32_t n_l = lst.n_l;
#ifdef PWAF_PROFILING
        const bool long_list = (b.debug & 1u) ? false : (b.debug & 2u) ? true : (a.behind_filter != 0u && (uint64_t)n_l * 8u >= a.n);
#else
        const bool long_list = a.behind_filter != 0u && (uint64_t)n_l * 8u >= a.n;
#endif
        if (long_list) {
            lscan_async<THREADS>(a, hot, cls, delta_lds, it, it_end, first, n_l, hot_elems, epi);
            it = it_end;
            continue;
        }
        const PWAF_GLOBAL unsigned char *gdata = (const PWAF_GLOBAL unsigned char *)a.data;
        const PWAF_GLOBAL uint16_t *flat = (const PWAF_GLOBAL uint16_t *)a.flat;
        for (uint32_t iw = it + wave_index(); iw < it_end; iw += THREADS / 64u) {
            uint32_t li[kListWalks], r[kListWalks], p[kListWalks], end[kListWalks], state[kListWalks], need_init[kListWalks];
            bool live[kListWalks];
            Hits h[kListWalks];
            u32x4 w[kListWalks];
#pragma unroll
            for (uint32_t u = 0; u < kListWalks; u++) {
                li[u] = (iw - first) * epi + u * 64u + (threadIdx.x & 63u);
                live[u] = (threadIdx.x & 63u) + u * 64u < epi && li[u] < n_l;
                if (live[u] && a.need_in != nullptr) live[u] = ((a.need_in[li[u]] >> a.need_bit) & 1u) != 0;
                r[u] = live[u] ? (a.req_list != nullptr ? a.req_list[li[u]] : li[u]) : 0u;
            }
#pragma unroll
            for (uint32_t u = 0; u < kListWalks; u++) {
                if (live[u] && a.visited != nullptr) atomicOr(&a.visited[r[u] >> 5], 1u << (r[u] & 31));
                p[u] = live[u] ? a.off[r[u]] : 0u;
                end[u] = live[u] ? a.off[r[u] + 1] : 0u;
                state[u] = 0;
                h[u] = Hits{0, 0, kNone};
                need_init[u] = 0;
                if (live[u] && a.merge_rec) {
                    h[u] = hits_of_record(a.rec[r[u]]);
                    if (a.colmask_local != nullptr && (h[u].a0 | (h[u].ovf + 1u)) != 0) need_init[u] = gate_mask(a.colmask_local, a.pool, h[u]);
                }
            }
#pragma unroll
            for (uint32_t u = 0; u < kListWalks; u++) {
                if (live[u] && a.emit_off[1] != a.emit_off[0]) h[u] = emit_list(a.emit_off, a.emit_list, a.pool, a.pool_count, a.status, a.pool_cap, 0u, h[u]);
                w[u] = *reinterpret_cast<const PWAF_GLOBAL u32x4_u *>(gdata + p[u]);
            }
            auto record_emit = [&](const uint32_t st, Hits &hh) {
                const uint32_t ei = st * stride + ncls;
                const uint32_t code = ei < hot_elems ? (uint32_t)hot[ei] : (uint32_t)flat[ei];
                const uint32_t x = (code & 0x7FFFu) + 1u;
                bool slow = !(code & 0x8000u) || hh.ovf != kNone;
                if (!slow) {
                    if (hh.a0 == x || hh.a1 == x) {}
                    else if (hh.a0 == 0) hh.a0 = x;
                    else if (hh.a1 == 0) hh.a1 = x;
                    else slow = true;
                }
                if (slow) hh = emit_list(a.emit_off, a.emit_list, a.pool, a.pool_count, a.status, a.pool_cap, st, hh);
            };
            for (;;) {
                bool more = false;
#pragma unroll
                for (uint32_t u = 0; u < kListWalks; u++) more = more || p[u] < end[u];
                if (!more) break;
                u32x4 wn[kListWalks];
                uint32_t cnt[kListWalks];
                bool lead_here = false;
#pragma unroll
                for (uint32_t u = 0; u < kListWalks; u++) {
                    const uint32_t pn = p[u] + 16u;
                    wn[u] = *reinterpret_cast<const PWAF_GLOBAL u32x4_u *>(gdata + (pn < end[u] ? pn : 0u));
                    cnt[u] = p[u] < end[u] ? min(16u, end[u] - p[u]) : 0u;
                    if (a.umap != nullptr) lead_here = lead_here || (cnt[u] != 0u && window_has_high(w[u]));
                }
                const bool fix_classes = a.umap != nullptr && __ballot(lead_here) != 0ull;
#pragma unroll
                for (uint32_t k0 = 0; k0 < 16; k0 += 4) {
                    uint32_t c[kListWalks][4], t[kListWalks][4], sv[kListWalks][4];
#pragma unroll
                    for (uint32_t u = 0; u < kListWalks; u++) {
                        const uint32_t wd = k0 == 0 ? w[u].x : k0 == 4 ? w[u].y : k0 == 8 ? w[u].z : w[u].w;
#pragma unroll
                        for (uint32_t k = 0; k < 4; k++) {
                            const uint32_t cl = cls[(wd >> (k * 8)) & 0xFFu];
                            c[u][k] = k0 + k < cnt[u] ? cl : ncls + 1u;
                        }
                        if (fix_classes) {
#pragma unroll
                            for (uint32_t k = 0; k < 4; k++) {
                                const uint32_t byte = (wd >> (k * 8)) & 0xFFu;
                                if (byte >= 0xC0u && k0 + k < cnt[u]) c[u][k] = lead_class(a.umap, a.ill_class, gdata, byte, p[u] + k0 + k, end[u]);
                                else if (byte >= 0x80u && k0 + k < cnt[u]) c[u][k] = cont_class(c[u][k], a.ill_class, gdata, p[u] + k0 + k, live[u] ? a.off[r[u]] : 0u, end[u]);
                            }
                        }
                    }
#pragma unroll
                    for (uint32_t k = 0; k < 4; k++) {
#pragma unroll
                        for (uint32_t u = 0; u < kListWalks; u++) {
                    t[u][k] = *reinterpret_cast<lds_u16_ptr>((uintptr_t)min(__umul24(k == 0 ? state[u] : sv[u][k - 1], 2u * stride) + 2u * c[u][k], 2u * hot_elems));
                            sv[u][k] = t[u][k] & 0x7FFFu;
                        }
                    }
                    uint32_t any = 0, top = 0;
#pragma unroll
                    for (uint32_t u = 0; u < kListWalks; u++)
#pragma unroll
                        for (uint32_t k = 0; k < 4; k++) { any |= t[u][k]; top = max(top, t[u][k]); }
                    if (any & 0x8000u) {
                        if (top == 0xFFFFu) {
#pragma unroll
                            for (uint32_t k = 0; k < 4; k++) {
#pragma unroll
                                for (uint32_t u = 0; u < kListWalks; u++) {
                                    const uint32_t tt = list_step_slow(hot, flat, delta_lds, state[u], c[u][k], stride, a.n_hot, a.n_delta);
                                    state[u] = tt & 0x7FFFu;
                                    if (tt & 0x8000u) record_emit(state[u], h[u]);
                                }
                            }
                        } else {
#pragma unroll
                            for (uint32_t u = 0; u < kListWalks; u++) {
#pragma unroll
                                for (uint32_t k = 0; k < 4; k++)
                                    if (t[u][k] & 0x8000u) record_emit(sv[u][k], h[u]);
                                state[u] = sv[u][3];
                            }
                        }
                    } else {
#pragma unroll
                        for (uint32_t u = 0; u < kListWalks; u++) state[u] = sv[u][3];
                    }
                }
#pragma unroll
                for (uint32_t u = 0; u < kListWalks; u++) {
                    if (p[u] < end[u]) p[u] += 16u;
                    w[u] = wn[u];
                }
            }
#pragma unroll
            for (uint32_t u = 0; u < kListWalks; u++) {
                if (!live[u]) continue;
                if (a.end_off[state[u] + 1] != a.end_off[state[u]]) h[u] = emit_list(a.end_off, a.end_list, a.pool, a.pool_count, a.status, a.pool_cap, state[u], h[u]);
                a.rec[r[u]] = h[u].ovf != kNone ? (REC_OVERFLOW | h[u].ovf) : (h[u].a0 | (h[u].a1 << 15));
                if (a.colmask_local != nullptr) {
                    uint32_t need = 0;
                    if ((h[u].a0 | (h[u].ovf + 1u)) != 0) need = gate_mask(a.colmask_local, a.pool, h[u]);
                    if (a.need_out != nullptr) a.need_out[li[u]] = need;
                    need &= ~(a.shared_bits | need_init[u]);
                    if (need) enqueue_mask_once(a.gate_lists, a.gate_count, a.n, r[u], need, a.enq_bits, a.enq_words);
                }
            }
        }
        it = it_end;
    }
}

__global__ __launch_bounds__(256) void confirm_plan_kernel(ConfirmTableDev b, uint32_t *plan ) {
    __shared__ uint32_t part[256];
    const uint32_t t = threadIdx.x;
    uint32_t items = 0;
    if (t < b.count) {
        const ConfirmArgs *pa = &b.c[t];
        const bool dense = pa->dense_flag != nullptr && *pa->dense_flag > pa->dense_thresh;
        items = dense ? 0u : (min(*pa->pair_count, pa->pair_cap) + kConfirmThreads - 1) / kConfirmThreads;
    }
    part[t] = items;
    __syncthreads();
    for (uint32_t d = 1; d < 256; d <<= 1) {
        const uint32_t v = t >= d ? part[t - d] : 0u;
        __syncthreads();
        part[t] += v;
        __syncthreads();
    }
    if (t < b.count) plan[t] = part[t] - items;
    if (t == 0) plan[b.count] = part[255];
}

__device__ __noinline__ void merge_atom(PoolEntry *pool, uint32_t *pool_count, uint32_t *status, uint32_t pool_cap, uint32_t *rec, uint32_t atom) {
    auto rmw_read = [](uint32_t *p) { return atomicOr(p, 0u); };
    auto publish = [&](uint32_t idx, uint32_t at, uint32_t next) {
        const uint32_t t0 = atomicExch(&pool[idx].atom, at), t1 = atomicExch(&pool[idx].next, next);
        asm volatile("" ::"v"(t0), "v"(t1));
    };
    uint32_t old = rmw_read(rec);
    for (;;) {
        uint32_t upd;
        const uint32_t x = atom + 1u;
        if (!(old & REC_OVERFLOW)) {
            const uint32_t a0 = old & 0x7FFFu, a1 = (old >> 15) & 0x7FFFu;
            if (a0 == x || a1 == x) return;
            if (a0 == 0u) upd = old | x;
            else if (a1 == 0u) upd = old | (x << 15);
            else {
                const uint32_t idx = atomicAdd(pool_count, 3u);
                if (idx + 3u > pool_cap) { atomicOr(status, 1u); return; }
                publish(idx, a0 - 1u, kNone);
                publish(idx + 1u, a1 - 1u, idx);
                publish(idx + 2u, atom, idx + 1u);
                upd = REC_OVERFLOW | (idx + 2u);
            }
        } else {
            const uint32_t head = old & ~REC_OVERFLOW;
            for (uint32_t i = head; i != kNone; i = rmw_read(&pool[i].next))
                if (rmw_read(&pool[i].atom) == atom) return;
            const uint32_t idx = atomicAdd(pool_count, 1u);
            if (idx >= pool_cap) { atomicOr(status, 1u); return; }
            publish(idx, atom, head);
            upd = REC_OVERFLOW | idx;
        }
        const uint32_t seen = atomicCAS(rec, old, upd);
        if (seen == old) return;
        old = seen;
    }
}

__global__ __launch_bounds__(kConfirmThreads, 8) void confirm_kernel(ConfirmTableDev b, const uint32_t *plan) {
    __shared__ uint32_t head[kFilterEntries], ftab[kFilterEntries];
    __shared__ uint32_t pool[kConfirmPoolBytes / 4];
    constexpr uint32_t kConfirmQueue = 1024;
    __shared__ uint32_t app_cnt, app_base, app_queue[kConfirmQueue];
    __builtin_amdgcn_s_setprio(3);
    if (threadIdx.x == 0) app_cnt = 0;
    const uint32_t total = plan[b.count];
    const uint32_t it0 = (uint32_t)((uint64_t)total * blockIdx.x / gridDim.x), it1 = (uint32_t)((uint64_t)total * (blockIdx.x + 1) / gridDim.x);
    for (uint32_t it = it0; it < it1;) {
        uint32_t ps = 0;
        for (uint32_t lo = 0, hi = b.count; lo + 1 < hi;) {
            const uint32_t mid = (lo + hi) >> 1;
            if (plan[mid] <= it) lo = mid;
            else hi = mid;
            ps = lo;
        }
        const uint32_t first_item = plan[ps], it_end = min(it1, plan[ps + 1]);
        const ConfirmArgs a = load_descriptor(&b.c[ps]);
        __syncthreads();
        {
            const uint4 *sh = reinterpret_cast<const uint4 *>(a.c_head), *sf = reinterpret_cast<const uint4 *>(a.ftable);
            constexpr uint32_t kPer = kFilterEntries / 4 / kConfirmThreads;
            uint4 vh[kPer], vf[kPer];
#pragma unroll
            for (uint32_t q = 0; q < kPer; q++) { vh[q] = sh[q * kConfirmThreads + threadIdx.x]; vf[q] = sf[q * kConfirmThreads + threadIdx.x]; }
#pragma unroll
            for (uint32_t q = 0; q < kPer; q++) {
                reinterpret_cast<uint4 *>(head)[q * kConfirmThreads + threadIdx.x] = vh[q];
                reinterpret_cast<uint4 *>(ftab)[q * kConfirmThreads + threadIdx.x] = vf[q];
            }
        }
        const uint32_t e_words = a.n_entries * 3u, b_words = a.n_bytes / 4u, c_words = a.n_class_words;
        const bool in_lds = (uint64_t)e_words + b_words + c_words <= kConfirmPoolBytes / 4;
        const ConfirmEntry *t_entries = a.c_entries;
        const uint8_t *t_bytes = a.c_bytes;
        const uint32_t *t_classes = a.c_classes;
        if (in_lds) {
            const uint32_t *se = reinterpret_cast<const uint32_t *>(a.c_entries), *sb = reinterpret_cast<const uint32_t *>(a.c_bytes);
            for (uint32_t k = threadIdx.x; k < e_words; k += kConfirmThreads) pool[k] = se[k];
            for (uint32_t k = threadIdx.x; k < b_words; k += kConfirmThreads) pool[e_words + k] = sb[k];
            for (uint32_t k = threadIdx.x; k < c_words; k += kConfirmThreads) pool[e_words + b_words + k] = a.c_classes[k];
            t_entries = reinterpret_cast<const ConfirmEntry *>(pool);
            t_bytes = reinterpret_cast<const uint8_t *>(pool + e_words);
            t_classes = pool + e_words + b_words;
        }
        __syncthreads();
        const ConfirmView cv{nullptr, t_entries, t_bytes, t_classes, a.mul, a.stride, a.init};
        const uint32_t n_p = min(*a.pair_count, a.pair_cap);
        auto pair_of = [&](const uint32_t item) -> uint2 {
            const uint32_t k = (item - first_item) * kConfirmThreads + threadIdx.x;
            return (item < it_end && k < n_p) ? a.pairs[k] : make_uint2(kNone, 0u);
        };
        uint2 pr_next = pair_of(it), pr_after = pair_of(it + 1u);
        uint32_t fs_next = 0u, fe_next = 0u;
        ConfirmBytes tb_next{};
        if (pr_next.x != kNone) {
            confirm_load64(reinterpret_cast<const uint8_t *>(a.off + pr_next.x), fs_next, fe_next);
            tb_next = confirm_chunk_bytes(a.data, pr_next.y, a.total + PWAF_ARENA_PAD);
        }
        for (; it < it_end; it++) {
            const uint2 pr = pr_next;
            const bool live = pr.x != kNone;
            uint32_t r = live ? pr.x : 0u;
            uint32_t fs = fs_next, fe = fe_next;
            const ConfirmBytes tb = tb_next;
            pr_next = pr_after;
            if (pr_next.x != kNone) {
                confirm_load64(reinterpret_cast<const uint8_t *>(a.off + pr_next.x), fs_next, fe_next);
                tb_next = confirm_chunk_bytes(a.data, pr_next.y, a.total + PWAF_ARENA_PAD);
            }
            pr_after = pair_of(it + 2u);
            ConfirmChunk ch{0u, 0ull};
            if (live) ch = confirm_windows_of(cv, tb, 0u, 0xFFFFFFFFu, pr.y, [&](const uint32_t bin) { return ftab[bin]; });
            uint32_t mask = ch.mask, cnt = 0, j = 0, e0 = 0, pos = 0, widx = 0;
            bool walk = false;
            auto settle = [&](const uint32_t rq, const uint32_t need_lits, const bool wk, const bool aggregated) -> bool {
                bool w2 = wk;
                if (need_lits & a.shared_bits) w2 = true;
                const uint32_t direct = need_lits & ~a.shared_bits;
                if (direct) enqueue_mask_once(a.gate_lists, a.gate_count, a.n, rq, direct, a.enq_bits, a.enq_words);
                if (!w2 || a.walk_list == nullptr) return false;
                const uint32_t bit = 1u << (rq & 31u);
                if (atomicOr(&a.walk_bits[rq >> 5], bit) & bit) return false;
                atomicOr(&a.valid_bits[rq >> 5], bit);
                if (aggregated) return true;
                a.walk_list[atomicAdd(a.walk_count, 1u)] = rq;
                return false;
            };
            uint32_t need = 0;
            for (;;) {
                if (__ballot(j < cnt || mask != 0u) == 0) break;
                while (j >= cnt && mask != 0u) {
                    const uint32_t k = (uint32_t)__builtin_ctz(mask);
                    mask &= mask - 1u;
                    pos = pr.y * 16u + k;
                    const uint32_t bin = confirm_bin_of(ch, widx++, a.data, pos, a.mul);
                    while (pos >= fe && r + 1u < a.n) {
                        settle(r, need, walk, false);
                        need = 0;
                        walk = false;
                        r++;
                        fs = fe;
                        fe = a.off[r + 1];
                    }
                    if (pos >= fe) continue;
                    const uint32_t hd = head[bin];
                    e0 = hd & 0xFFFFFu;
                    cnt = hd >> 20;
                    j = 0;
                }
                if (j < cnt) {
                    const uint32_t res = in_lds ? confirm_entry<3>(t_entries, t_bytes, t_classes, e0 + j, a.data, fs, fe, pos)
                                                : confirm_entry<1>(t_entries, t_bytes, t_classes, e0 + j, a.data, fs, fe, pos);
                    j++;
                    if (res == 2u) {
                        walk = true;
                    } else if (res & 1u) {
                        const uint32_t atom = res >> 8;
                        merge_atom(a.pool, a.pool_count, a.status, a.pool_cap, a.rec + r, atom);
                        atomicOr(&a.valid_bits[r >> 5], 1u << (r & 31u));
                        if (a.colmask_local != nullptr) need |= a.colmask_local[atom];
                    }
                }
            }
            const bool append = live && settle(r, need, walk, true);
            if (append) {
                const uint32_t slot = atomicAdd(&app_cnt, 1u);
                if (slot < kConfirmQueue) app_queue[slot] = r;
                else a.walk_list[atomicAdd(a.walk_count, 1u)] = r;
            }
        }
        __syncthreads();
        {
            const uint32_t queued = min(app_cnt, kConfirmQueue);
            if (threadIdx.x == 0 && queued != 0) app_base = atomicAdd(a.walk_count, queued);
            __syncthreads();
            for (uint32_t k = threadIdx.x; k < queued; k += kConfirmThreads) a.walk_list[app_base + k] = app_queue[k];
            __syncthreads();
            if (threadIdx.x == 0) app_cnt = 0;
        }
    }
}

int launch_scan(const ScanArgs &a, void *stream) {
    const uint32_t lds = scan_lds_bytes(a.n_hot, a.stride, a.colmask_local ? a.n_local : 0u);
    const bool wide = a.n_classes > 127;
    const int v = (a.chunks == 4 ? 2 : a.chunks == 2 ? 1 : 0) + (wide ? 3 : 0);
    const void *fns[6] = {reinterpret_cast<const void *>(scan_kernel<1, false>), reinterpret_cast<const void *>(scan_kernel<2, false>),
                          reinterpret_cast<const void *>(scan_kernel<4, false>), reinterpret_cast<const void *>(scan_kernel<1, true>),
                          reinterpret_cast<const void *>(scan_kernel<2, true>), reinterpret_cast<const void *>(scan_kernel<4, true>)};
    const void *fn = fns[v];
    if (a.n == 0) return 0;
    uint32_t waves = (a.n + 255) / 256;
    uint32_t blocks = (waves + kScanWaves - 1) / kScanWaves;
#ifdef PWAF_PROFILING
    static const uint32_t forced_cap = getenv("PWAF_SCAN_BLOCKS") ? (uint32_t)atoi(getenv("PWAF_SCAN_BLOCKS")) : 0u;
#else
    const uint32_t forced_cap = 0;
#endif
    const uint32_t cap = forced_cap ? forced_cap : std::max(1u, a.n_cus);
    if (blocks > cap) blocks = cap;
    if (blocks == 0) blocks = 1;
    void *args[] = {const_cast<ScanArgs *>(&a)};
    hipError_t e = hipLaunchKernel(fn, dim3(blocks), dim3(kScanThreads), args, lds, (hipStream_t)stream);
    return (int)(e != hipSuccess ? e : hipGetLastError());
}

__global__ __launch_bounds__(256) void copy_args_kernel(const uint4 *__restrict__ src, uint4 *__restrict__ dst, uint32_t n16, uint4 *__restrict__ zero, uint32_t z16) {
    for (uint32_t i = blockIdx.x * 256u + threadIdx.x; i < n16; i += gridDim.x * 256u) dst[i] = src[i];
    for (uint32_t i = blockIdx.x * 256u + threadIdx.x; i < z16; i += gridDim.x * 256u) zero[i] = make_uint4(0u, 0u, 0u, 0u);
}
int upload_args_block(const void *host_pinned, void *dev, size_t bytes, void *zero, size_t zero_bytes, void *stream) {
    const uint32_t n16 = (uint32_t)((bytes + 15) / 16), z16 = (uint32_t)(zero_bytes / 16);
    if (n16 == 0 && z16 == 0) return 0;
    const uint32_t blocks = std::max(std::min<uint32_t>((n16 + 255) / 256, 64u), std::min<uint32_t>((z16 + 2047) / 2048, 1024u));
    hipLaunchKernelGGL(copy_args_kernel, dim3(std::max(1u, blocks)), dim3(256), 0, (hipStream_t)stream, (const uint4 *)host_pinned, (uint4 *)dev, n16, (uint4 *)zero, z16);
    return (int)hipGetLastError();
}

int launch_confirm(const ConfirmArgs *host, uint32_t count, const ConfirmArgs *dev, uint32_t *plan, uint32_t n_cus, void *stream) {
    if (count == 0 || host[0].n == 0) return 0;
    if (count > 256) return (int)hipErrorInvalidValue;
    ConfirmTableDev b{dev, count};
    hipLaunchKernelGGL(confirm_plan_kernel, dim3(1), dim3(256), 0, (hipStream_t)stream, b, plan);
    hipError_t e = hipGetLastError();
    if (e != hipSuccess) return (int)e;
    uint64_t max_items = 0;
    for (uint32_t k = 0; k < count; k++) max_items += ((uint64_t)host[k].pair_cap + kConfirmThreads - 1) / kConfirmThreads;
    const uint32_t blocks = (uint32_t)std::min<uint64_t>(max_items, (uint64_t)std::max(1u, n_cus) * 2u);
    const uint32_t *cplan = plan;
    hipLaunchKernelGGL(confirm_kernel, dim3(blocks), dim3(kConfirmThreads), 0, (hipStream_t)stream, b, cplan);
    return (int)hipGetLastError();
}

static const void *lscan_fn(bool wide) { return wide ? reinterpret_cast<const void *>(lscan_kernel<1024>) : reinterpret_cast<const void *>(lscan_kernel<512>); }

int launch_scan_gated(const ListScanArgs *host, uint32_t count, const ListScanArgs *dev, uint32_t *plan, const ListShape &shape, void *stream) {
    if (count == 0 || host[0].n == 0) return 0;
    if (count > 256) return (int)hipErrorInvalidValue;
    GatedTable b{dev, count, 0u};
#ifdef PWAF_PROFILING
    static const uint32_t async_mode = getenv("PWAF_LSCAN_ASYNC") ? (uint32_t)atoi(getenv("PWAF_LSCAN_ASYNC")) : 0u;
    b.debug = async_mode;
#endif
    const uint32_t blocks = std::max(1u, host[0].n_cus) * shape.wg_per_cu;
    hipLaunchKernelGGL(lscan_plan_kernel, dim3(1), dim3(256), 0, (hipStream_t)stream, b, plan, blocks * (shape.threads / 64u));
    hipError_t e = hipGetLastError();
    if (e != hipSuccess) return (int)e;
    const uint32_t *cplan = plan;
    uint32_t hot_bytes = list_hot_bytes(shape);
    void *args[] = {&b, &cplan, &hot_bytes};
    const void *fn = lscan_fn(shape.threads == 1024);
    e = hipLaunchKernel(fn, dim3(blocks), dim3(shape.threads), args, shape.hot_bytes + 16 + 256, (hipStream_t)stream);
    return (int)(e != hipSuccess ? e : hipGetLastError());
}

uint32_t list_hot_bytes(const ListShape &shape) { return shape.hot_bytes; }

ListShape list_shape(uint32_t variant) {
    switch (variant) {
        case 1: return ListShape{512, 72u * 1024u, 2};
        case 2: return ListShape{1024, 144u * 1024u, 1};
        case 3: return ListShape{512, 32u * 1024u, 4};
        default: return ListShape{kListThreads, kListHotBytes, 3};
    }
}

typedef unsigned short u16x2 __attribute__((ext_vector_type(2)));

template <bool HEADS, int STRIDE>
__device__ __forceinline__ void filter_rows(const FilterArgs &a, const uint32_t blk, const uint32_t wave, const uint32_t lane) {
    const PWAF_GLOBAL unsigned char *gdata = (const PWAF_GLOBAL unsigned char *)a.data;
    const uint32_t rel = blk * kFilterWaves + wave, slab = a.slab0 + rel;
    const uint64_t base64 = (uint64_t)slab * kStreamSlab;
    if (base64 >= a.total) return;
    const uint32_t total = a.total, base0 = (uint32_t)base64, slab_end = (uint32_t)min<uint64_t>(total, base64 + kStreamSlab);
    unsigned long long *my_bits = reinterpret_cast<unsigned long long *>(a.chunk_bits) + (size_t)rel * (kStreamSlab / 1024);
    uint32_t n_hit = 0;
    const uint32_t mul2 = a.mul | (a.mul << 16);
    constexpr uint32_t kRow = 1024;

    auto load_row = [&](const uint32_t b, const uint32_t q) {
        const uint32_t p = b + kRow * q + 16u * lane;
        return *reinterpret_cast<const PWAF_GLOBAL u32x4_u *>(gdata + (p < total ? p : 0u));
    };
    auto dword_at = [&](const uint32_t p) {
        return filter_fold4(*reinterpret_cast<const PWAF_GLOBAL uint32_t __attribute__((aligned(1))) *>(gdata + p));
    };
    auto slot_lo = [](const uint32_t masked) {
        uint32_t r;
        asm("v_lshrrev_b32_sdwa %0, 2, %1 dst_sel:DWORD dst_unused:UNUSED_PAD src0_sel:DWORD src1_sel:WORD_0" : "=v"(r) : "v"(masked));
        return r;
    };
    auto slot_hi = [](const uint32_t masked) {
        uint32_t r;
        asm("v_lshrrev_b32_sdwa %0, 2, %1 dst_sel:DWORD dst_unused:UNUSED_PAD src0_sel:DWORD src1_sel:WORD_1" : "=v"(r) : "v"(masked));
        return r;
    };
    auto bins4 = [&](const uint32_t x, const uint32_t next, uint32_t (&mm)[4]) {
        const uint32_t z = __builtin_amdgcn_alignbit(next, x, 8);
        const uint32_t hx = __builtin_bit_cast(uint32_t, __builtin_bit_cast(u16x2, x) * __builtin_bit_cast(u16x2, mul2));
        const uint32_t hz = __builtin_bit_cast(uint32_t, __builtin_bit_cast(u16x2, z) * __builtin_bit_cast(u16x2, mul2));
#ifdef PWAF_PROFILING
        if (a.debug & 1u) { mm[0] = hx | 0xFF000000u; mm[1] = hz | 0xFF000000u; mm[2] = (hx >> 3) | 0xFF000000u; mm[3] = (hz >> 5) | 0xFF000000u; return; }
#endif
        const uint32_t kx = hx & 0xFFF0FFF0u, kz = hz & 0xFFF0FFF0u;
        mm[0] = *reinterpret_cast<lds_u32_ptr>((uintptr_t)slot_lo(kx));
        mm[1] = *reinterpret_cast<lds_u32_ptr>((uintptr_t)slot_lo(kz));
        mm[2] = *reinterpret_cast<lds_u32_ptr>((uintptr_t)slot_hi(kx));
        mm[3] = *reinterpret_cast<lds_u32_ptr>((uintptr_t)slot_hi(kz));
    };
    auto bins2 = [&](const uint32_t x, uint32_t (&mm)[2]) {
        const uint32_t hx = __builtin_bit_cast(uint32_t, __builtin_bit_cast(u16x2, x) * __builtin_bit_cast(u16x2, mul2));
#ifdef PWAF_PROFILING
        if (a.debug & 1u) { mm[0] = hx | 0xFF000000u; mm[1] = (hx >> 3) | 0xFF000000u; return; }
#endif
        const uint32_t kx = hx & 0xFFF0FFF0u;
        mm[0] = *reinterpret_cast<lds_u32_ptr>((uintptr_t)slot_lo(kx));
        mm[1] = *reinterpret_cast<lds_u32_ptr>((uintptr_t)slot_hi(kx));
    };
    auto push = [](uint32_t &st, const uint32_t m) { asm("v_lshl_or_b32 %0, %1, 8, %2" : "=v"(st) : "v"(st), "v"(m)); };

    uint32_t rq = 0, ho[2] = {0xFFFFFFFFu, 0xFFFFFFFFu}, hn[2] = {0xFFFFFFFFu, 0xFFFFFFFFu};
    auto load_offs = [&](const uint32_t r0) {
        ho[0] = a.off[min(r0 + lane, a.n)];
        ho[1] = a.off[min(r0 + 64u + lane, a.n)];
        const uint32_t e1 = a.off[min(r0 + 128u, a.n)];
        hn[0] = (uint32_t)__builtin_amdgcn_update_dpp(__builtin_amdgcn_readfirstlane((int)ho[1]), (int)ho[0], 0x130 , 0xF, 0xF, false);
        hn[1] = (uint32_t)__builtin_amdgcn_update_dpp(__builtin_amdgcn_readfirstlane((int)e1), (int)ho[1], 0x130, 0xF, 0xF, false);
    };
    auto head_record = [&](const u32x4 w, const uint32_t flen) {
        uint32_t hrec = 0;
#pragma unroll
        for (int hq = 0; hq < 2; hq++) {
            if ((uint32_t)hq < a.n_heads) {
                const uint32_t diff = ((w.x ^ a.head_w[hq][0]) & a.head_m[hq][0]) | ((w.y ^ a.head_w[hq][1]) & a.head_m[hq][1]) |
                                      ((w.z ^ a.head_w[hq][2]) & a.head_m[hq][2]) | ((w.w ^ a.head_w[hq][3]) & a.head_m[hq][3]);
                const uint32_t hl = a.head_len[hq] & 0xFFu;
                const bool len_ok = (a.head_len[hq] >> 8) ? flen == hl : flen >= hl;
                if (diff == 0 && len_ok) hrec |= a.head_code[hq];
            }
        }
        return hrec;
    };
    const bool heads = HEADS && a.n_heads != 0;
    if (heads) {
        uint32_t lo = 0, hi = a.n;
        while (lo < hi) {
            const uint32_t span = hi - lo, step = (span + 63) / 64;
            const uint32_t probe = lo + lane * step;
            const bool ok = probe >= hi || a.off[probe] >= base0;
            const unsigned long long m = __ballot(ok);
            if (m == 0) {
                lo += 63u * step + 1u;
                continue;
            }
            const uint32_t f = (uint32_t)__builtin_ctzll(m);
            const uint32_t nh = min(hi, lo + f * step);
            lo = f == 0 ? lo : lo + (f - 1u) * step + 1u;
            hi = nh;
        }
        rq = lo;
        load_offs(rq);
    }

    uint32_t carry = a.init;
    if (STRIDE == 1) {
        if (base0 >= 4) {
            uint32_t mw[4];
            bins4(dword_at(base0 - 4), dword_at(base0), mw);
            push(carry, mw[1]); push(carry, mw[2]); push(carry, mw[3]);
        }
    } else if (base0 >= 8) {
        uint32_t m0[2], m1[2];
        bins2(dword_at(base0 - 8), m0);
        bins2(dword_at(base0 - 4), m1);
        push(carry, m0[1]); push(carry, m1[0]); push(carry, m1[1]);
    }
    carry = __builtin_amdgcn_readfirstlane(carry);
    const uint32_t after = (STRIDE == 1 && slab_end < total) ? __builtin_amdgcn_readfirstlane(dword_at(slab_end)) : 0u;

    u32x4 w[4];
#pragma unroll
    for (uint32_t q = 0; q < 4; q++) w[q] = load_row(base0, q);
    for (uint32_t b = base0; b < slab_end; b += kStreamIter) {
        const bool more = b + kStreamIter < slab_end;
        u32x4 hw[2];
        uint32_t hlen[2] = {0xFFFFFFFFu, 0xFFFFFFFFu};
        uint32_t rq_here = rq;
#ifdef PWAF_PROFILING
        if (heads && !(a.debug & 4u)) {
#else
        if (heads) {
#endif
            const uint32_t lim = min(b + kStreamIter, slab_end);
            const bool in0 = ho[0] < lim;
            const uint32_t c0 = (uint32_t)__builtin_popcountll(__ballot(in0));
            if (in0) {
                hw[0] = *reinterpret_cast<const PWAF_GLOBAL u32x4_u *>(gdata + ho[0]);
                hlen[0] = hn[0] - ho[0];
            }
            uint32_t c1 = 0;
            if (c0 == 64) {
                const bool in1 = ho[1] < lim;
                c1 = (uint32_t)__builtin_popcountll(__ballot(in1));
                if (in1) {
// ... 22 lines not shown
        unsigned long long hm[4];
#pragma unroll
        for (uint32_t q = 0; q < 4; q++) {
            const uint32_t x0 = filter_fold4(w[q].x), x1 = filter_fold4(w[q].y), x2 = filter_fold4(w[q].z), x3 = filter_fold4(w[q].w);
            uint32_t st, seen = 0xFFFFFFFFu, tail;
            if (STRIDE == 1) {
                const uint32_t first_next = (q == 3 && !more) ? after : filter_fold4(__builtin_amdgcn_readfirstlane(w[(q + 1) & 3].x));
                const uint32_t x4 = (uint32_t)__builtin_amdgcn_update_dpp((int)first_next, (int)x0, 0x130 , 0xF, 0xF, false);
                uint32_t m[16];
                {
                    uint32_t mm[4];
                    bins4(x0, x1, mm); m[0] = mm[0]; m[1] = mm[1]; m[2] = mm[2]; m[3] = mm[3];
                    bins4(x1, x2, mm); m[4] = mm[0]; m[5] = mm[1]; m[6] = mm[2]; m[7] = mm[3];
                    bins4(x2, x3, mm); m[8] = mm[0]; m[9] = mm[1]; m[10] = mm[2]; m[11] = mm[3];
                    bins4(x3, x4, mm); m[12] = mm[0]; m[13] = mm[1]; m[14] = mm[2]; m[15] = mm[3];
                }
#ifdef PWAF_PROFILING
                if (more && !(a.debug & 2u)) w[q] = load_row(b + kStreamIter, q);
#else
                if (more) w[q] = load_row(b + kStreamIter, q);
#endif
                tail = m[13]; push(tail, m[14]); push(tail, m[15]);
                st = (uint32_t)__builtin_amdgcn_update_dpp((int)carry, (int)tail, 0x138 , 0xF, 0xF, false);
#pragma unroll
                for (int i = 0; i < 16; i++) { push(st, m[i]); seen &= st; }
            } else {
                uint32_t m[8];
                {
                    uint32_t mm[2];
                    bins2(x0, mm); m[0] = mm[0]; m[1] = mm[1];
                    bins2(x1, mm); m[2] = mm[0]; m[3] = mm[1];
                    bins2(x2, mm); m[4] = mm[0]; m[5] = mm[1];
                    bins2(x3, mm); m[6] = mm[0]; m[7] = mm[1];
                }
#ifdef PWAF_PROFILING
                if (more && !(a.debug & 2u)) w[q] = load_row(b + kStreamIter, q);
#else
                if (more) w[q] = load_row(b + kStreamIter, q);
#endif
                tail = m[5]; push(tail, m[6]); push(tail, m[7]);
                st = (uint32_t)__builtin_amdgcn_update_dpp((int)carry, (int)tail, 0x138 , 0xF, 0xF, false);
#pragma unroll
                for (int i = 0; i < 8; i++) { push(st, m[i]); seen &= st; }
            }
            carry = __builtin_amdgcn_readlane(tail, 63);
            const bool hit = ((~seen) & 0xFF000000u) != 0 && b + kRow * q + 16u * lane < total;
            hm[q] = __ballot(hit);
            __builtin_amdgcn_sched_barrier(0);
        }
        if (lane < 4) my_bits[(b - base0) / kRow + lane] = lane == 0 ? hm[0] : lane == 1 ? hm[1] : lane == 2 ? hm[2] : hm[3];
        n_hit += (uint32_t)(__builtin_popcountll(hm[0]) + __builtin_popcountll(hm[1]) + __builtin_popcountll(hm[2]) + __builtin_popcountll(hm[3]));

        if (heads) {
#pragma unroll
            for (uint32_t q = 0; q < 2; q++) {
                if (hlen[q] != 0xFFFFFFFFu) {
                    const uint32_t hrec = head_record(hw[q], hlen[q]);
                    if (hrec) a.rec[rq_here + 64u * q + lane] = hrec;
                }
            }
        }
    }
    for (uint32_t wd = (slab_end - base0 + kStreamIter - 1) / kStreamIter * 4 + lane; wd < kStreamSlab / kRow; wd += 64) my_bits[wd] = 0;
    if (lane == 0) {
        a.sub_count[rel] = n_hit;
        if (a.pairs != nullptr) a.pair_base[rel] = n_hit ? atomicAdd(a.pair_count, n_hit) : 0u;
    }
}

template <bool HEADS>
__global__ __launch_bounds__(kFilterWaves * 64) void filter_kernel(FilterMix M) {
    extern __shared__ __align__(16) unsigned char lds[];
    __builtin_amdgcn_s_setprio(3);
    const uint32_t n_all = M.blocks1 + M.blocks2;
    const uint32_t before = (uint32_t)(((uint64_t)blockIdx.x * M.blocks1) / n_all), upto = (uint32_t)(((uint64_t)(blockIdx.x + 1) * M.blocks1) / n_all);
    const bool one = upto > before;
    const uint32_t blk = one ? before : blockIdx.x - before;
    const FilterArgs *tab = one ? M.f1 : M.f2;
    uint32_t k = 0;
    for (uint32_t lo = 0, hi = one ? M.count1 : M.count2; lo + 1 < hi;) {
        const uint32_t mid = (lo + hi) >> 1;
        if (blk >= tab[mid].first_block) lo = mid;
        else hi = mid;
        k = lo;
    }
    const FilterArgs a = load_descriptor(&tab[k]);
    const uint32_t tid = threadIdx.x, wave = wave_index(), lane = tid & 63;
    {
        const uint4 *src = reinterpret_cast<const uint4 *>(a.table);
        uint4 *dst = reinterpret_cast<uint4 *>(lds);
        for (uint32_t i = tid; i < kFilterEntries / 4; i += kFilterWaves * 64) dst[i] = src[i];
    }
    __syncthreads();
    if ((uint32_t)(uintptr_t)(PWAF_LDS unsigned char *)lds != 0u) __builtin_trap();
    if (one) filter_rows<HEADS, 1>(a, blk - a.first_block, wave, lane);
    else filter_rows<HEADS, 2>(a, blk - a.first_block, wave, lane);
}

template <uint32_t PARTS>
__global__ void resolve_kernel(FilterTable B);

__global__ __launch_bounds__(256) void bitcount_kernel(FilterTable B) {
    __builtin_amdgcn_s_setprio(3);
    __shared__ uint32_t red[256];
    const FilterArgs a = load_descriptor(&B.f[blockIdx.y]);
    const uint32_t words = (a.n + 31) / 32, w0 = blockIdx.x * kCompactWords;
    if (w0 >= words) return;
    uint32_t c = 0;
    for (uint32_t w = w0 + threadIdx.x; w < min(words, w0 + kCompactWords); w += 256) c += (uint32_t)__builtin_popcount(a.bitmap[w]);
    red[threadIdx.x] = c;
    __syncthreads();
    for (uint32_t h = 128; h > 0; h >>= 1) {
        if (threadIdx.x < h) red[threadIdx.x] += red[threadIdx.x + h];
        __syncthreads();
    }
    if (threadIdx.x == 0) a.block_count[blockIdx.x] = red[0];
}

__global__ void compact_kernel(FilterTable B);

static uint32_t filter_blocks(const FilterArgs *host, uint32_t count, bool *heads) {
    uint32_t blocks = 0;
    for (uint32_t k = 0; k < count; k++) {
        const uint32_t slabs = (uint32_t)(((uint64_t)host[k].total + kStreamSlab - 1) / kStreamSlab) - host[k].slab0;
        blocks += (slabs + kFilterWaves - 1) / kFilterWaves;
        *heads = *heads || host[k].n_heads != 0;
    }
    return blocks;
}

int launch_filter(const FilterArgs *host1, uint32_t count1, const FilterArgs *dev1, const FilterArgs *host2, uint32_t count2, const FilterArgs *dev2, void *stream) {
    bool heads = false;
    FilterMix m{dev1, dev2, count1, count2, filter_blocks(host1, count1, &heads), filter_blocks(host2, count2, &heads)};
    if (m.blocks1 + m.blocks2 == 0) return 0;
    void *args[] = {&m};
    const void *fn = heads ? reinterpret_cast<const void *>(filter_kernel<true>) : reinterpret_cast<const void *>(filter_kernel<false>);
    hipError_t e = hipLaunchKernel(fn, dim3(m.blocks1 + m.blocks2), dim3(kFilterWaves * 64), args, kFilterEntries * 4, (hipStream_t)stream);
    return (int)(e != hipSuccess ? e : hipGetLastError());
}

int launch_resolve(const FilterArgs *host, uint32_t count, const FilterArgs *dev, void *stream) {
    uint32_t max_slabs = 0;
    uint64_t all_slabs = 0;
    for (uint32_t k = 0; k < count; k++) {
        const uint32_t slabs = (uint32_t)(((uint64_t)host[k].total + kStreamSlab - 1) / kStreamSlab) - host[k].slab0;
        max_slabs = max(max_slabs, slabs);
        all_slabs += slabs;
    }
    if (count == 0 || max_slabs == 0) return 0;
    FilterTable t{dev, count};
    void *args[] = {&t};
    const char *forced = getenv("PWAF_RESOLVE_PARTS");
    const bool split = forced ? atoi(forced) == 4 : all_slabs < 4096u;
    hipError_t e = split ? hipLaunchKernel(reinterpret_cast<const void *>(resolve_kernel<4>), dim3(max_slabs, count), dim3(256), args, 0, (hipStream_t)stream)
                         : hipLaunchKernel(reinterpret_cast<const void *>(resolve_kernel<1>), dim3((max_slabs + 3) / 4, count), dim3(256), args, 0, (hipStream_t)stream);
    return (int)(e != hipSuccess ? e : hipGetLastError());
}

int launch_compact(const FilterArgs *host, uint32_t count, const FilterArgs *dev, void *stream) {
    if (count == 0 || host[0].n == 0) return 0;
    const uint32_t words = (host[0].n + 31) / 32, n_blocks = (words + kCompactWords - 1) / kCompactWords;
    FilterTable t{dev, count};
    void *args[] = {&t};
    hipError_t e = hipLaunchKernel(reinterpret_cast<const void *>(bitcount_kernel), dim3(n_blocks, count), dim3(256), args, 0, (hipStream_t)stream);
    if (e == hipSuccess) e = hipLaunchKernel(reinterpret_cast<const void *>(compact_kernel), dim3(n_blocks, count), dim3(256), args, 0, (hipStream_t)stream);
    return (int)(e != hipSuccess ? e : hipGetLastError());
}

__global__ __launch_bounds__(256) void fcmp_kernel(FcmpArgs a) {
    const SlowCtx ctx{nullptr, nullptr, a.pool, a.pool_count, a.status, a.pool_cap};
    for (uint32_t r = blockIdx.x * 256u + threadIdx.x; r < a.n; r += gridDim.x * 256u) {
        Hits h{0, 0, kNone};
        for (uint32_t k = 0; k < a.n_atoms; k++) {
            const uint32_t op = a.atoms[k] & 0xFFu, sa = (a.atoms[k] >> 8) & 0xFFu, sb = (a.atoms[k] >> 16) & 0xFFu;
            const uint32_t a0 = a.off[sa][r], la = a.off[sa][r + 1] - a0, b0 = a.off[sb][r], lb = a.off[sb][r + 1] - b0;
            const uint8_t *x = a.data[sa] + a0, *y = a.data[sb] + b0;
            bool holds = false;
            auto same = [&](const uint8_t *p, const uint8_t *q, uint32_t len) {
                for (uint32_t i = 0; i < len; i++)
                    if (p[i] != q[i]) return false;
                return true;
            };
            switch (op) {
                case FC_EQ: holds = la == lb && same(x, y, la); break;
                case FC_STARTS: holds = la >= lb && same(x, y, lb); break;
                case FC_ENDS: holds = la >= lb && same(x + (la - lb), y, lb); break;
                case FC_CONTAINS:
                    if (la >= lb)
                        for (uint32_t s = 0; s + lb <= la && !holds; s++) holds = same(x + s, y, lb);
                    break;
                case FC_LEN_EQ: holds = la == lb; break;
                case FC_LEN_LT: holds = la < lb; break;
                default: holds = la <= lb; break;
            }
            if (holds) h = record_atom(ctx, k, h);
        }
        a.rec[r] = h.ovf != kNone ? (REC_OVERFLOW | h.ovf) : (h.a0 | (h.a1 << 15));
    }
}

int launch_fcmp(const FcmpArgs &a, void *stream) {
    if (a.n == 0 || a.n_atoms == 0) return 0;
    hipLaunchKernelGGL(fcmp_kernel, dim3(std::min<uint32_t>((a.n + 255) / 256, 4096u)), dim3(256), 0, (hipStream_t)stream, a);
    return (int)hipGetLastError();
}

__global__ __launch_bounds__(128) void residual_kernel(ResidualArgs a) {
    const SlowCtx ctx{nullptr, nullptr, a.pool, a.pool_count, a.status, a.pool_cap};
    rvm::Machine m;
    m.blob = a.blob;
    m.h = reinterpret_cast<const rvm::Header *>(a.blob);
    m.q.data = a.data;
    m.q.off = a.off;
    for (uint32_t r = blockIdx.x * 128u + threadIdx.x; r < a.n; r += gridDim.x * 128u) {
        m.q.r = r;
        m.q.ip = a.ip + (size_t)r * 16;
        m.q.v6 = a.ip_is_v6[r];
        m.q.port = a.port[r];
        uint32_t asn = 0, country = (uint32_t)'X' | ((uint32_t)'X' << 8);
        if (a.asn != nullptr) {
            asn = a.asn[r];
            const uint32_t cc = a.country[r], c0 = (cc & 0xFFu) - 'A', c1 = (cc >> 8) - 'A';
            if (c0 < 26u && c1 < 26u) country = cc;
        } else if (a.has_geo) {
            const uint8_t *ip = m.q.ip;
            bool walk;
            if (!m.q.v6) walk = !(ip[0] == 127u || (ip[0] & 0xF0u) == 0xE0u);
            else {
                bool loopback = ip[15] == 1;
                for (int k = 0; k < 15; k++) loopback = loopback && ip[k] == 0;
                walk = !(loopback || ip[0] == 0xFFu);
            }
            if (walk) {
                uint32_t e = (m.q.v6 ? a.geo_root6 : a.geo_root4)[((uint32_t)ip[0] << 8) | ip[1]];
                for (uint32_t k = 2; !(e & TRIE_LEAF); k++) e = a.geo_nodes[(size_t)e * 256 + ip[k]];
                const GeoRec g = a.geo_recs[e & ~TRIE_LEAF];
                asn = g.asn;
                country = g.country;
            }
        }
        m.q.asn = asn;
        m.q.country = country;
        Hits h{0, 0, kNone};
        for (uint32_t k = 0; k < a.n_rules; k++) {
            const uint32_t res = rvm::run_rule(m, k);
            if (res == 1u) h = record_atom(ctx, k, h);
            const unsigned long long em = __ballot(res == 2u);
            if (em != 0 && (threadIdx.x & 63u) == (uint32_t)__builtin_ctzll(em)) atomicAdd(&a.rule_errors[k], (unsigned long long)__builtin_popcountll(em));
        }
        a.rec[r] = h.ovf != kNone ? (REC_OVERFLOW | h.ovf) : (h.a0 | (h.a1 << 15));
    }
}

int launch_residual(const ResidualArgs &a, void *stream) {
    if (a.n == 0 || a.n_rules == 0) return 0;
    hipLaunchKernelGGL(residual_kernel, dim3(std::min<uint32_t>((a.n + 127) / 128, 8192u)), dim3(128), 0, (hipStream_t)stream, a);
    return (int)hipGetLastError();
}

__device__ __forceinline__ uint32_t ip_byte(const uint32_t w[4], uint32_t k) {
    uint32_t word = k < 4 ? w[0] : k < 8 ? w[1] : k < 12 ? w[2] : w[3];
    return (word >> ((k & 3) * 8)) & 0xFFu;
}

__device__ __forceinline__ uint32_t wave_or(uint32_t x) {
#define PWAF_DPP_OR(ctrl, rows) x |= (uint32_t)__builtin_amdgcn_update_dpp(0, (int)x, (ctrl), (rows), 0xF, true)
    PWAF_DPP_OR(0x111, 0xF);
    PWAF_DPP_OR(0x112, 0xF);
    PWAF_DPP_OR(0x114, 0xF);
    PWAF_DPP_OR(0x118, 0xF);
    PWAF_DPP_OR(0x142, 0xA);
    PWAF_DPP_OR(0x143, 0xC);
#undef PWAF_DPP_OR
    return (uint32_t)__builtin_amdgcn_readlane((int)x, 63);
}

#pragma clang diagnostic push
#pragma clang diagnostic ignored "-Winline-asm"
__device__ __forceinline__ void park64(uint32_t &lo, uint32_t &hi, const unsigned long long m, const uint32_t l) {
    asm volatile("s_mov_b32 m0, %3\n\ts_nop 0\n\tv_writelane_b32 %0, %2, m0\n\tv_writelane_b32 %1, %4, m0"
                 : "+v"(lo), "+v"(hi)
                 : "s"((uint32_t)m), "s"(l), "s"((uint32_t)(m >> 32))
                 : "m0");
}
#pragma clang diagnostic pop

__device__ __forceinline__ uint32_t wave_scan_add(uint32_t x) {
#define PWAF_DPP_ADD(ctrl, rows) x += (uint32_t)__builtin_amdgcn_update_dpp(0, (int)x, (ctrl), (rows), 0xF, true)
    PWAF_DPP_ADD(0x111, 0xF);
    PWAF_DPP_ADD(0x112, 0xF);
    PWAF_DPP_ADD(0x114, 0xF);
    PWAF_DPP_ADD(0x118, 0xF);
    PWAF_DPP_ADD(0x142, 0xA);
    PWAF_DPP_ADD(0x143, 0xC);
#undef PWAF_DPP_ADD
    return x;
}

template <uint32_t PARTS>
__global__ __launch_bounds__(256) void resolve_kernel(FilterTable B) {
    __builtin_amdgcn_s_setprio(3);
    constexpr uint32_t kChunks = kStreamSlab / 16, kWords = kChunks / 32;
    constexpr uint32_t kResolveSparse = 128;
    __shared__ uint32_t s_bits[4][kWords], s_rank[4][kWords];
    const FilterArgs *pa = &B.f[blockIdx.y];
    if ((uint64_t)(pa->slab0 + blockIdx.x * 4 / PARTS) * kStreamSlab >= pa->total) return;
    const FilterArgs a = load_descriptor(pa);
    if (a.dense_flag != nullptr && *a.dense_flag > a.dense_thresh) return;
    const uint32_t wave = wave_index(), rel = (blockIdx.x * 4 + wave) / PARTS, part = (blockIdx.x * 4 + wave) % PARTS, slab = a.slab0 + rel, lane = threadIdx.x & 63;
    constexpr uint32_t kPartChunks = kChunks / PARTS;
    if ((uint64_t)slab * kStreamSlab >= a.total) return;
    const uint32_t cnt = a.sub_count[rel];
    if (cnt == 0) return;
    const bool sparse = a.pairs != nullptr && cnt <= kResolveSparse;
    if (sparse && part != 0u) return;
    const uint32_t lo_c = sparse ? 0u : part * kPartChunks, hi_c = sparse ? kChunks : lo_c + kPartChunks;
    const uint32_t *slab_bits = a.chunk_bits + (size_t)rel * kWords;
    uint32_t *bits = s_bits[wave], *rank = s_rank[wave];
#pragma unroll
    for (uint32_t q = 0; q < kWords / 64; q++) bits[q * 64 + lane] = slab_bits[q * 64 + lane];
    __builtin_amdgcn_fence(__ATOMIC_ACQ_REL, "wavefront");
    {
        uint32_t w[kWords / 64], mine = 0;
#pragma unroll
        for (uint32_t q = 0; q < kWords / 64; q++) {
            w[q] = bits[lane * (kWords / 64) + q];
            mine += (uint32_t)__builtin_popcount(w[q]);
        }
        uint32_t before = wave_scan_add(mine) - mine;
#pragma unroll
        for (uint32_t q = 0; q < kWords / 64; q++) {
            rank[lane * (kWords / 64) + q] = before;
            before += (uint32_t)__builtin_popcount(w[q]);
        }
    }
    __builtin_amdgcn_fence(__ATOMIC_ACQ_REL, "wavefront");
    auto rank_of = [&](const uint32_t c) {
        if (c >= kChunks) return rank[kWords - 1] + (uint32_t)__builtin_popcount(bits[kWords - 1]);
        return rank[c >> 5] + (uint32_t)__builtin_popcount(bits[c >> 5] & ((1u << (c & 31u)) - 1u));
    };
    const uint32_t back = 3u * a.stride;
    const uint64_t slab_b0 = (uint64_t)slab * kStreamSlab, b0 = slab_b0 + (uint64_t)lo_c * 16u;
    const uint32_t c_first = (uint32_t)(slab_b0 / 16);
    uint32_t lo = 0, hi = a.n;
    while (lo < hi) {
        const uint32_t span = hi - lo, step = (span + 63) / 64;
        const uint32_t probe = lo + lane * step;
        const bool ok = probe >= hi || (uint64_t)a.off[probe + 1] + back > b0;
        const unsigned long long m = __ballot(ok);
        if (m == 0) {
            lo += 63u * step + 1u;
            continue;
        }
        const uint32_t f = (uint32_t)__builtin_ctzll(m);
        const uint32_t nh = min(hi, lo + f * step);
        lo = f == 0 ? lo : lo + (f - 1u) * step + 1u;
        hi = nh;
    }
    const uint64_t b1 = slab_b0 + (uint64_t)hi_c * 16u;
    const uint32_t pair_base = a.pairs != nullptr ? a.pair_base[rel] : 0u;
    const uint32_t begin = __builtin_amdgcn_readfirstlane(a.off[0]);
    if (part == 0 && a.pairs != nullptr && (uint64_t)begin > slab_b0) {
        const uint32_t n_before = min((uint32_t)(((uint64_t)begin - slab_b0) >> 4), kChunks);
        for (uint32_t w = lane; w * 32u < n_before; w += 64) {
            uint32_t bw = bits[w];
            if (n_before - w * 32u < 32u) bw &= (1u << (n_before - w * 32u)) - 1u;
            const uint32_t word = bits[w];
            while (bw) {
                const uint32_t bit = (uint32_t)__builtin_ctz(bw);
                bw &= bw - 1u;
                const uint32_t at = pair_base + rank[w] + (uint32_t)__builtin_popcount(word & ((1u << bit) - 1u));
                if (at < a.pair_cap) a.pairs[at] = make_uint2(kNone, 0u);
            }
        }
    }
    if (sparse) {
        bool redo = false;
        for (uint32_t k = lane; k < cnt; k += 64) {
            uint32_t wlo = 0, whi = kWords;
            while (wlo + 1u < whi) {
                const uint32_t mid = (wlo + whi) >> 1;
                if (rank[mid] <= k) wlo = mid;
                else whi = mid;
            }
            uint32_t word = bits[wlo];
            for (uint32_t skip = k - rank[wlo]; skip != 0u; skip--) word &= word - 1u;
            const uint32_t chunk = c_first + wlo * 32u + (uint32_t)__builtin_ctz(word), byte0 = chunk * 16u;
            if (byte0 + 16u <= begin) continue;
            const uint32_t key = max(byte0, begin);
            uint32_t l = lo, h = min(a.n, lo + 4096u);
            const uint32_t h0 = h;
            while (l < h) {
                const uint32_t mid = (l + h) >> 1;
                if (a.off[mid + 1] > key) h = mid;
                else l = mid + 1u;
            }
            if (l == h0) {
                if (h0 < a.n) { redo = true; continue; }
                if (pair_base + k < a.pair_cap) a.pairs[pair_base + k] = make_uint2(kNone, 0u);
                continue;
            }
            if (pair_base + k < a.pair_cap) a.pairs[pair_base + k] = make_uint2(l, chunk);
            if (a.n_heads == 0) {
                uint32_t r = l, steps = 0;
                for (; r < a.n && steps < 48u; r++, steps++) {
                    const uint32_t s = a.off[r];
                    if (s >= byte0 + 16u) break;
                    if (a.off[r + 1] > s) a.rec[r] = 0u;
                }
                if (steps == 48u) redo = true;
            }
        }
        if (__ballot(redo) == 0ull) return;
    }
    {
    uint32_t s_n = 0xFFFFFFFFu, e_n = 0xFFFFFFFFu;
    {
        const uint32_t r = lo + lane;
        if (r < a.n) { s_n = a.off[r]; e_n = a.off[r + 1]; }
    }
    for (uint32_t rb = lo; rb < a.n; rb += 64) {
        const uint32_t r = rb + lane;
        const bool live = r < a.n;
        const uint32_t s = s_n, e = e_n;
        {
            const uint32_t r2 = r + 64;
            s_n = e_n = 0xFFFFFFFFu;
            if (r2 < a.n) { s_n = a.off[r2]; e_n = a.off[r2 + 1]; }
        }
        if (a.pairs != nullptr) {
            if (a.n_heads == 0 && live && e > s) {
                const uint32_t g_lo = s >> 4, g_hi = (e - 1u) >> 4;
                if (g_hi >= c_first + lo_c && g_lo < c_first + hi_c) {
                    const uint32_t y0 = g_lo > c_first + lo_c ? g_lo - c_first : lo_c, y1 = min(g_hi - c_first, hi_c - 1u);
                    if (rank_of(y1 + 1u) != rank_of(y0)) a.rec[r] = 0u;
                }
            }
            if (live && e > s) {
                const uint32_t f_lo = s == begin ? s >> 4 : (s + 15u) >> 4, f_hi = (e - 1u) >> 4;
                if (f_lo <= f_hi && f_hi >= c_first + lo_c && f_lo < c_first + hi_c) {
                    const uint32_t x0 = f_lo > c_first + lo_c ? f_lo - c_first : lo_c, x1 = min(f_hi - c_first, hi_c - 1u);
                    for (uint32_t w = x0 >> 5; w <= (x1 >> 5); w++) {
                        const uint32_t word = bits[w];
                        uint32_t bw = word;
                        if (w == (x0 >> 5)) bw &= ~0u << (x0 & 31u);
                        if (w == (x1 >> 5)) bw &= ~0u >> (31u - (x1 & 31u));
                        while (bw) {
                            const uint32_t bit = (uint32_t)__builtin_ctz(bw);
                            bw &= bw - 1u;
                            const uint32_t at = pair_base + rank[w] + (uint32_t)__builtin_popcount(word & ((1u << bit) - 1u));
                            if (at < a.pair_cap) a.pairs[at] = make_uint2(r, c_first + w * 32u + bit);
                        }
                    }
                }
            }
            if (__ballot(live && (uint64_t)s >= b1) != 0) break;
            continue;
        }
        bool mark = false;
        if (live && (uint64_t)s < b1 + 16) {
            const uint32_t j_lo = s == 0 ? 0u : (s - 1u) / 16u, j_hi = (uint32_t)(((uint64_t)e + back - 1u) / 16u);
            const uint32_t x0 = j_lo > c_first + lo_c ? j_lo - c_first : lo_c;
            if (j_hi >= c_first + lo_c && x0 < hi_c) {
                const uint32_t x1 = min(j_hi - c_first, hi_c - 1u);
                mark = x0 <= x1 && rank_of(x1 + 1u) != rank_of(x0);
            }
        }
        const unsigned long long m = __ballot(mark);
        if (m != 0) {
            const uint32_t sh = rb & 31u, w0 = rb >> 5;
            const uint32_t parts[3] = {(uint32_t)(m << sh), (uint32_t)(sh ? m >> (32u - sh) : m >> 32), sh ? (uint32_t)(m >> (64u - sh)) : 0u};
            if (lane < 3 && parts[lane] != 0) atomicOr(&a.bitmap[w0 + lane], parts[lane]);
        }
        if (__ballot(live && (uint64_t)s >= b1 + 16) != 0) break;
    }
    }
}

__global__ __launch_bounds__(256) void compact_kernel(FilterTable B) {
    __builtin_amdgcn_s_setprio(3);
    __shared__ uint32_t red[256];
    const FilterArgs a = load_descriptor(&B.f[blockIdx.y]);
    const uint32_t words = (a.n + 31) / 32, w0 = blockIdx.x * kCompactWords, tid = threadIdx.x, wave = wave_index(), lane = tid & 63;
    if (w0 >= words) return;
    const uint32_t n_blocks = (words + kCompactWords - 1) / kCompactWords;
    uint32_t acc = 0;
    for (uint32_t bq = tid; bq < blockIdx.x; bq += 256) acc += a.block_count[bq];
    red[tid] = acc;
    __syncthreads();
    for (uint32_t h = 128; h > 0; h >>= 1) {
        if (tid < h) red[tid] += red[tid + h];
        __syncthreads();
    }
    const uint32_t base = red[0];
    __syncthreads();
    constexpr uint32_t kSteps = kCompactWords / 256;
    const uint32_t wave_w0 = w0 + wave * (kSteps * 64);
    uint32_t wv[kSteps], mine = 0;
#pragma unroll
    for (uint32_t q = 0; q < kSteps; q++) {
        const uint32_t w = wave_w0 + q * 64 + lane;
        wv[q] = w < words ? a.bitmap[w] : 0u;
        mine += (uint32_t)__builtin_popcount(wv[q]);
    }
    const uint32_t wave_total = (uint32_t)__builtin_amdgcn_readlane((int)wave_scan_add(mine), 63);
    if (lane == 0) red[wave] = wave_total;
    __syncthreads();
    uint32_t pos0 = base;
    for (uint32_t k = 0; k < wave; k++) pos0 += red[k];
#pragma unroll
    for (uint32_t q = 0; q < kSteps; q++) {
        uint32_t w = wv[q];
        const uint32_t pc = (uint32_t)__builtin_popcount(w), incl = wave_scan_add(pc);
        uint32_t pos = pos0 + incl - pc;
        const uint32_t r0 = (wave_w0 + q * 64 + lane) * 32;
        while (w) {
            a.list[pos++] = r0 + (uint32_t)__builtin_ctz(w);
            w &= w - 1;
        }
        pos0 += (uint32_t)__builtin_amdgcn_readlane((int)incl, 63);
    }
    if (blockIdx.x == n_blocks - 1 && tid == 255) *a.list_count = pos0;
}


__host__ __device__ static inline uint32_t verdict_wave_lds(uint32_t n_cols, uint32_t n_rules) {
    const uint32_t colw = (n_cols + 31) / 32, rulew = (n_rules + 31) / 32;
    return ((n_cols * 8 + colw * 4 + rulew * 4 + n_rules * 2) + 15) & ~15u;
}

__host__ __device__ static inline uint32_t verdict_wave_lds_sp(uint32_t n_cols, uint32_t n_rules, uint32_t v_cap) {
    const uint32_t colw = (n_cols + 31) / 32, rulew = (n_rules + 31) / 32;
    return ((colw * 8 + v_cap * 8 + rulew * 4 + n_rules * 2) + 15) & ~15u;
}
__host__ __device__ static inline uint32_t verdict_v_cap(uint32_t n_cols, bool tiny) {
    const uint32_t v = tiny ? 8u : 256u + n_cols / 16u;
    return v < n_cols ? v : n_cols;
}

struct VerdictTables {
    uint32_t bitcol, trig_off, trig_rules, rules, lits, pub, end;
};
__host__ __device__ static inline VerdictTables verdict_tables(uint32_t n_cols, uint32_t n_rules, uint32_t n_trig, uint32_t n_lits, bool lt) {
    VerdictTables t;
    t.bitcol = 0;
    t.trig_off = 0;
    t.trig_rules = t.trig_off + (lt ? ((n_cols + 1) * 2 + 3) & ~3u : 0u);
    t.rules = t.trig_rules + (lt ? (n_trig * 2 + 7) & ~7u : 0u);
    t.lits = t.rules + (lt ? n_rules * 8 : 0u);
    t.pub = t.lits + (lt ? n_lits * 4 : 0u);
    t.end = t.pub + (lt ? (n_rules * 2 + 3) & ~3u : 0u);
    return t;
}

template <bool LT, int BR, bool SP>
__global__ __launch_bounds__(SP ? 768 : 1024, (SP && BR == 1) ? 6 : 1) void verdict_kernel(VerdictArgs a) {
    extern __shared__ __align__(16) unsigned char lds[];
    const uint32_t tid = threadIdx.x, wave = wave_index(), lane = tid & 63, n_waves = blockDim.x >> 6;
#ifdef PWAF_PROFILING
    const uint32_t dbg_skip = a.debug_skip;
#else
    constexpr uint32_t dbg_skip = 0;
#endif
    const uint32_t colw = (a.n_cols + 31) / 32, rulew = (a.n_rules + 31) / 32;
    const uint32_t v_cap = a.v_cap;
    const uint32_t wave_bytes = SP ? verdict_wave_lds_sp(a.n_cols, a.n_rules, v_cap) : verdict_wave_lds(a.n_cols, a.n_rules);
    unsigned char *mine = lds + (size_t)wave * wave_bytes;
    unsigned long long *col = reinterpret_cast<unsigned long long *>(mine);
    uint32_t *colnz = reinterpret_cast<uint32_t *>(col + a.n_cols);
    uint32_t *nz = reinterpret_cast<uint32_t *>(mine);
    unsigned long long *vals = reinterpret_cast<unsigned long long *>(mine + (size_t)colw * 8);
    unsigned long long *spill = (SP && a.spill != nullptr) ? a.spill + (size_t)(blockIdx.x * n_waves + wave) * (a.n_cols - v_cap) : nullptr;
    uint32_t *rulebm = SP ? reinterpret_cast<uint32_t *>(vals + v_cap) : colnz + colw;
    uint16_t *cand = reinterpret_cast<uint16_t *>(rulebm + rulew);
    unsigned char *tables = lds + (size_t)n_waves * wave_bytes;
    const VerdictTables vt = verdict_tables(a.n_cols, a.n_rules, a.n_trig, a.n_lits, LT);
    uint16_t *l_trig_off = reinterpret_cast<uint16_t *>(tables + vt.trig_off);
    uint16_t *l_trig_rules = reinterpret_cast<uint16_t *>(tables + vt.trig_rules);
    uint2 *l_rules = reinterpret_cast<uint2 *>(tables + vt.rules);
    uint32_t *l_lits = reinterpret_cast<uint32_t *>(tables + vt.lits);
    uint16_t *l_pub = reinterpret_cast<uint16_t *>(tables + vt.pub);
    if (LT) {
        for (uint32_t k = tid; k <= a.n_cols; k += blockDim.x) l_trig_off[k] = (uint16_t)a.trig_off[k];
        for (uint32_t k = tid; k < a.n_trig; k += blockDim.x) l_trig_rules[k] = a.trig_rules[k];
        for (uint32_t k = tid; k < a.n_rules; k += blockDim.x) {
            const DevRule dr = a.rules[k];
            l_rules[k] = make_uint2(dr.lit_off, dr.lit_cnt | ((uint32_t)dr.eff_unverified << 16) | ((uint32_t)dr.eff_verified << 24));
            l_pub[k] = (uint16_t)dr.public_idx;
        }
        for (uint32_t k = tid; k < a.n_lits; k += blockDim.x) l_lits[k] = a.lits[k];
    }
    __syncthreads();
    const unsigned long long mybit = 1ull << lane;
    const unsigned long long lt_mask = mybit - 1;
    unsigned long long cnt_block = 0, cnt_captcha = 0, cnt_bypass = 0, cnt_allow = 0;

    const uint32_t h_always = lane < rulew ? a.always_rules[lane] : 0u;

    constexpr int kPre = kVerdictPre;
    constexpr int kBitRegs = BR;
    struct Bits {
        unsigned long long w[kBitRegs];
    };
    struct Inputs {
        uint32_t rv[kPre];
        uint32_t base[kPre];
        Bits bits;
        unsigned long long rest[kBitRegs];
        uint32_t flags, n_pairs;
        uint4 pair0;
        uint32_t res0;
    };
    const uint32_t *my_bits[kBitRegs];
    uint32_t my_base[kBitRegs];
    bool my_live[kBitRegs];
#pragma unroll
    for (int r = 0; r < kBitRegs; r++) {
        const uint32_t ps = (uint32_t)r * 64 + lane;
        my_live[r] = ps < a.n_passes;
        my_bits[r] = nullptr;
        my_base[r] = 0;
        if (my_live[r]) {
            const PassInfo pi = a.passes[ps];
            const uint32_t kind = pi.kind_slot >> 24, slot = pi.kind_slot & 0xFFFFFFu;
            if (kind == 3) my_live[r] = false;
            my_bits[r] = kind == 1 ? a.cand_bits + (size_t)slot * a.bit_words : kind == 2 ? a.visit_bits + (size_t)slot * a.bit_words : nullptr;
            my_base[r] = pi.base;
        }
    }
// ... 1395 lines not shown
    if (a.n == 0) return 0;
#ifdef PWAF_PROFILING
    static const uint32_t forced = getenv("PWAF_ATTR_BLOCKS") ? (uint32_t)atoi(getenv("PWAF_ATTR_BLOCKS")) : 0u;
#else
    const uint32_t forced = 0;
#endif
    const uint32_t blocks = std::min<uint32_t>((a.n_groups + 3) / 4, forced ? forced : 6 * std::max(1u, a.attr_blocks));
    const bool small = a.set_words <= 4 && a.cc_words <= 2 && a.iu_words[0] <= 1 && a.iu_words[1] <= 1 && a.acmp_words <= 1;
    if (a.ipres_packed && small) hipLaunchKernelGGL((attr_kernel<true, true>), dim3(blocks), dim3(256), 0, (hipStream_t)stream, a);
    else if (a.ipres_packed) hipLaunchKernelGGL((attr_kernel<true, false>), dim3(blocks), dim3(256), 0, (hipStream_t)stream, a);
    else if (small) hipLaunchKernelGGL((attr_kernel<false, true>), dim3(blocks), dim3(256), 0, (hipStream_t)stream, a);
    else hipLaunchKernelGGL((attr_kernel<false, false>), dim3(blocks), dim3(256), 0, (hipStream_t)stream, a);
    return (int)hipGetLastError();
}

static constexpr uint32_t kLdsPerGroup = 160u * 1024u;
VerdictShape verdict_shape(uint32_t n_cols, uint32_t n_rules, uint32_t n_trig, uint32_t n_lits, bool force_global, int mode, uint32_t n_passes) {
    VerdictShape s{};
    const uint32_t t_lds = verdict_tables(n_cols, n_rules, n_trig, n_lits, true).end, t_glb = verdict_tables(n_cols, n_rules, n_trig, n_lits, false).end;
    if (mode >= 3) {
        s.sparse = 2;
        const uint32_t cu_waves = n_passes <= 64 ? 24u : 16u;
        auto fit = [&](uint32_t cap, uint32_t &bw, uint32_t &bk, uint32_t &lt) {
            const uint32_t wave = verdict_wave_lds_el(n_cols, n_rules, cap);
            const bool fits = !force_global && n_trig < 65536 && t_lds + 8 * wave <= kLdsPerGroup;
            const uint32_t tables = fits ? t_lds : t_glb;
            bw = 0; bk = 1; lt = fits ? 1u : 0u;
            for (uint32_t k = 1; k <= 3; k++) {
                const uint32_t share = kLdsPerGroup / k;
                if (share <= tables + wave) continue;
                const uint32_t w = std::min(std::min(12u, cu_waves / k), (share - tables) / wave);
                if (w * k > bw * bk) { bw = w; bk = k; }
            }
        };
        uint32_t cap = 8, bw = 0, bk = 1, lt = 0;
        if (mode == 4) fit(cap, bw, bk, lt);
        else {
            uint32_t w0, k0, l0;
            fit(64, w0, k0, l0);
            for (uint32_t c : {254u, 224u, 192u, 160u, 128u, 96u, 64u}) {
                fit(c, bw, bk, lt);
                cap = c;
                if (bw * bk >= w0 * k0) break;
            }
        }
        s.v_cap = cap;
        s.waves = bw;
        s.per_cu = bk;
        s.lds_tables = lt;
        s.lds_bytes = (lt ? t_lds : t_glb) + bw * verdict_wave_lds_el(n_cols, n_rules, cap);
        return s;
    }
    if (mode != 0) {
        s.sparse = 1;
        s.v_cap = verdict_v_cap(n_cols, mode == 2);
        const uint32_t wave = verdict_wave_lds_sp(n_cols, n_rules, s.v_cap);
        const bool fits = !force_global && n_trig < 65536 && t_lds + 8 * wave <= kLdsPerGroup;
        s.lds_tables = fits ? 1 : 0;
        const uint32_t tables = fits ? t_lds : t_glb;
        const uint32_t cu_waves = n_passes <= 64 ? 24u : 16u;
        uint32_t best_w = 0, best_k = 1;
        for (uint32_t k = 1; k <= 3; k++) {
            const uint32_t share = kLdsPerGroup / k;
            if (share <= tables + wave) continue;
            const uint32_t w = std::min(std::min(12u, cu_waves / k), (share - tables) / wave);
            if (w * k > best_w * best_k) { best_w = w; best_k = k; }
        }
        s.waves = best_w;
        s.per_cu = best_k;
        s.lds_bytes = tables + s.waves * wave;
        return s;
    }
    const uint32_t wave = verdict_wave_lds(n_cols, n_rules);
    const bool fits = !force_global && n_trig < 65536 && t_lds + 4 * wave <= kLdsPerGroup;
    s.lds_tables = fits ? 1 : 0;
    const uint32_t tables = fits ? t_lds : t_glb;
    uint32_t w = tables + wave <= kLdsPerGroup ? (kLdsPerGroup - tables) / wave : 0;
    if (!fits) w = std::min(w, 4u);
    s.waves = std::min(w, 16u);
    s.per_cu = 1;
    s.lds_bytes = tables + s.waves * wave;
    return s;
}

uint32_t verdict_blocks_sp(const VerdictShape &sh, uint32_t n_cus) { return std::max(1u, n_cus) * sh.per_cu; }

int launch_verdict(const VerdictArgs &a, void *stream) {
    VerdictShape sh = verdict_shape(a.n_cols, a.n_rules, a.n_trig, a.n_lits, a.force_global_tables != 0, (int)a.sparse_mode, a.n_passes);
    if (sh.waves == 0 || a.n_cols >= 65536u) return (int)hipErrorInvalidValue;
    if (sh.sparse == 1 && (a.v_cap != sh.v_cap || (sh.v_cap < a.n_cols && a.spill == nullptr))) return (int)hipErrorInvalidValue;
    if (sh.sparse == 2 && (a.v_cap != sh.v_cap || a.spill == nullptr)) return (int)hipErrorInvalidValue;
#ifdef PWAF_PROFILING
    static const uint32_t cap_waves = getenv("PWAF_VERDICT_WAVES") ? (uint32_t)atoi(getenv("PWAF_VERDICT_WAVES")) : 0u;
    if (cap_waves && cap_waves < sh.waves) sh.waves = cap_waves;
#endif
    constexpr int kBRmax = (kMaxPasses + 1 + 63) / 64;
    int variant = a.n_passes <= 64 ? 1 : 0;
#ifdef PWAF_PROFILING
    static const int forced_variant = getenv("PWAF_VERDICT_VARIANT") ? atoi(getenv("PWAF_VERDICT_VARIANT")) : -1;
    if (forced_variant >= 0 && forced_variant < variant) variant = forced_variant;
#endif
    const void *fns[2][2][2] = {{{reinterpret_cast<const void *>(verdict_kernel<false, kBRmax, false>), reinterpret_cast<const void *>(verdict_kernel<false, 1, false>)},
                                 {reinterpret_cast<const void *>(verdict_kernel<true, kBRmax, false>), reinterpret_cast<const void *>(verdict_kernel<true, 1, false>)}},
                                {{reinterpret_cast<const void *>(verdict_kernel<false, kBRmax, true>), reinterpret_cast<const void *>(verdict_kernel<false, 1, true>)},
                                 {reinterpret_cast<const void *>(verdict_kernel<true, kBRmax, true>), reinterpret_cast<const void *>(verdict_kernel<true, 1, true>)}}};
    const void *fns2[2][2][2] = {{{reinterpret_cast<const void *>(verdict2_kernel<false, kBRmax, false>), reinterpret_cast<const void *>(verdict2_kernel<false, 1, false>)},
                                  {reinterpret_cast<const void *>(verdict2_kernel<true, kBRmax, false>), reinterpret_cast<const void *>(verdict2_kernel<true, 1, false>)}},
                                 {{reinterpret_cast<const void *>(verdict2_kernel<false, kBRmax, true>), reinterpret_cast<const void *>(verdict2_kernel<false, 1, true>)},
                                  {reinterpret_cast<const void *>(verdict2_kernel<true, kBRmax, true>), reinterpret_cast<const void *>(verdict2_kernel<true, 1, true>)}}};
    const bool want_hits = a.n_hits != nullptr || a.rule_hits != nullptr;
    if (want_hits && (sh.sparse != 2 || (a.hits == nullptr && a.n_hits != nullptr && a.hits_cap != 0))) return (int)hipErrorInvalidValue;
    const void *fn = sh.sparse == 2 ? fns2[want_hits ? 1 : 0][sh.lds_tables ? 1 : 0][variant] : fns[sh.sparse ? 1 : 0][sh.lds_tables ? 1 : 0][variant];
    uint32_t blocks = (a.n_groups + sh.waves - 1) / sh.waves;
#ifdef PWAF_PROFILING
    static const uint32_t forced_cap = getenv("PWAF_VERDICT_BLOCKS") ? (uint32_t)atoi(getenv("PWAF_VERDICT_BLOCKS")) : 0u;
#else
    const uint32_t forced_cap = 0;
#endif
    const uint32_t cap = (forced_cap && !sh.sparse) ? forced_cap : sh.sparse ? verdict_blocks_sp(sh, a.attr_blocks) : sh.lds_tables ? std::max(1u, a.attr_blocks) : 2048u;
    if (blocks > cap) blocks = cap;
    if (blocks == 0) return 0;
    void *args[] = {const_cast<VerdictArgs *>(&a)};
    hipError_t e = hipLaunchKernel(fn, dim3(blocks), dim3(sh.waves * 64), args, sh.lds_bytes, (hipStream_t)stream);
    return (int)(e != hipSuccess ? e : hipGetLastError());
}

int configure_kernels(int device) {
    static std::mutex mu;
    static std::set<int> done;
    std::lock_guard<std::mutex> lock(mu);
    if (done.count(device)) return 0;
    const void *fns[] = {reinterpret_cast<const void *>(scan_kernel<1, false>), reinterpret_cast<const void *>(scan_kernel<2, false>),
                         reinterpret_cast<const void *>(scan_kernel<4, false>), reinterpret_cast<const void *>(scan_kernel<1, true>),
                         reinterpret_cast<const void *>(scan_kernel<2, true>), reinterpret_cast<const void *>(scan_kernel<4, true>),
                         reinterpret_cast<const void *>(verdict_kernel<true, (kMaxPasses + 1 + 63) / 64, false>), reinterpret_cast<const void *>(verdict_kernel<false, (kMaxPasses + 1 + 63) / 64, false>),
                         reinterpret_cast<const void *>(verdict_kernel<true, 1, false>), reinterpret_cast<const void *>(verdict_kernel<false, 1, false>),
                         reinterpret_cast<const void *>(verdict_kernel<true, (kMaxPasses + 1 + 63) / 64, true>), reinterpret_cast<const void *>(verdict_kernel<false, (kMaxPasses + 1 + 63) / 64, true>),
                         reinterpret_cast<const void *>(verdict_kernel<true, 1, true>), reinterpret_cast<const void *>(verdict_kernel<false, 1, true>),
                         reinterpret_cast<const void *>(verdict2_kernel<true, (kMaxPasses + 1 + 63) / 64, false>), reinterpret_cast<const void *>(verdict2_kernel<false, (kMaxPasses + 1 + 63) / 64, false>),
                         reinterpret_cast<const void *>(verdict2_kernel<true, 1, false>), reinterpret_cast<const void *>(verdict2_kernel<false, 1, false>),
                         reinterpret_cast<const void *>(verdict2_kernel<true, (kMaxPasses + 1 + 63) / 64, true>), reinterpret_cast<const void *>(verdict2_kernel<false, (kMaxPasses + 1 + 63) / 64, true>),
                         reinterpret_cast<const void *>(verdict2_kernel<true, 1, true>), reinterpret_cast<const void *>(verdict2_kernel<false, 1, true>),
                         reinterpret_cast<const void *>(filter_kernel<true>), reinterpret_cast<const void *>(filter_kernel<false>),
                         lscan_fn(false), lscan_fn(true)};
    for (const void *fn : fns) {
        hipError_t e = hipFuncSetAttribute(fn, hipFuncAttributeMaxDynamicSharedMemorySize, (int)kLdsPerGroup);
        if (e != hipSuccess) return (int)e;
    }
    done.insert(device);
    return 0;
}

}
```

Measured before the change: 7.148 billion.

## Fold confirm and list-scan plan kernels into their consumer kernels

Removes the separate single-block plan kernels that ran before the confirm and gated list-scan launches. Each workgroup now recomputes the per-descriptor item counts and prefix sums in LDS, using a wave-shuffle scan instead of a shared-memory Hillis-Steele scan, which drops a launch and a global-memory plan round trip per stage. The cost is redundant planning work in every workgroup and extra LDS for the list scan, which could lower occupancy. The change also adds profiling-only timestamp instrumentation that is compiled out by default.

Result: no change. 7.118 billion (-0.4%).

```diff
diff --git a/pingoo_amd/build.py b/pingoo_amd/build.py
--- a/pingoo_amd/build.py
+++ b/pingoo_amd/build.py
@@ -9,7 +9,7 @@
 CSRC = os.path.join(HERE, "csrc")
 LIB = os.path.join(HERE, "libpwaf.so")
 SOURCES = ["frontend.cpp", "pattern.cpp", "dfa.cpp", "iptrie.cpp", "filter.cpp", "residual.cpp", "residual_jit.cpp", "rtc.cpp", "compile.cpp", "loaders.cpp", "batcher.cpp", "async.cpp", "node.cpp", "engine.cpp", "kernels.hip", "records.hip"]
-HEADERS = ["frontend.h", "program.h", "kernels.h", "residual.h", "confirm.h", "records.h", "lscan_split.h", "dirtable.h", "georec.h", "unicode_data.inc", os.path.join("..", "..", "include", "pwaf.h")]
+HEADERS = ["frontend.h", "program.h", "kernels.h", "residual.h", "confirm.h", "records.h", "lscan_split.h", "plan.h", "dirtable.h", "georec.h", "unicode_data.inc", os.path.join("..", "..", "include", "pwaf.h")]
 
 
 def hipcc() -> str:
diff --git a/pingoo_amd/csrc/engine.cpp b/pingoo_amd/csrc/engine.cpp
--- a/pingoo_amd/csrc/engine.cpp
+++ b/pingoo_amd/csrc/engine.cpp
@@ -866,7 +866,6 @@
     const FilterArgs *d_all = nullptr, *d_s1 = nullptr, *d_s2 = nullptr;
     const ConfirmArgs *d_c = nullptr;
     const ListScanArgs *d_la[2] = {nullptr, nullptr};
-    uint32_t *c_plan = nullptr, *l_plan = nullptr;
 
     BatchRun(pwaf_engine *e_, Scratch &S_, const pwaf_batch &db_, hipStream_t stream_, const std::vector<uint32_t> *col_begin_)
         : e(e_), S(S_), P(*e_->prog.p), db(db_), stream(stream_), col_begin(col_begin_), sw(switches()), prof(e_, stream_), arg_slot{S_, stream_} {
@@ -1155,18 +1154,16 @@
     }
     int launch_confirm_stage() {
         if (call.empty()) return PWAF_OK;
-        return timed("confirm", 0xF8u, "confirm kernel", [&] { return launch_confirm(call.data(), (uint32_t)call.size(), d_c, c_plan, e->n_cus, stream); });
+        return timed("confirm", 0xF8u, "confirm kernel", [&] { return launch_confirm(call.data(), (uint32_t)call.size(), d_c, e->n_cus, stream); });
     }
     int launch_list_scans() {
-        uint32_t *plan_at = l_plan;
         for (int phase = 0; phase < 2; phase++) {
             uint32_t first = 0;
             for (const uint32_t cnt : e->lscan_launches[phase]) {
                 char nm[48];
                 snprintf(nm, sizeof nm, "lscan_x%u", cnt);
-                const int rc = timed(nm, 0xFDu, "gated scan kernel", [&] { return launch_scan_gated(la[phase].data() + first, cnt, d_la[phase] + first, plan_at, lshapes[phase], stream); });
+                const int rc = timed(nm, 0xFDu, "gated scan kernel", [&] { return launch_scan_gated(la[phase].data() + first, cnt, d_la[phase] + first, lshapes[phase], stream); });
                 if (rc) return rc;
-                plan_at += 2 * cnt + 1;
                 first += cnt;
             }
         }
@@ -1542,7 +1539,6 @@
         const Part up[7] = {{L.take(b_all), fall.data(), b_all}, {L.take(b_s1), by_stride[0].data(), b_s1}, {L.take(b_s2), by_stride[1].data(), b_s2}, {L.take(b_c), call.data(), b_c},
                             {L.take(b_l0 + sizeof(ListScanArgs)), la[0].data(), b_l0}, {L.take(b_l1 + sizeof(ListScanArgs)), la[1].data(), b_l1}, {L.take(b_ptrs), ptrs.p, b_ptrs}};
         const size_t up_bytes = L.size();
-        const size_t a_cplan = L.take((call.size() + 2) * 4), a_lplan = L.take((lsplit::plan_words(e->lscan_launches[0]) + lsplit::plan_words(e->lscan_launches[1])) * 4);
         if ((rc = S.args.reserve(L.size()))) return rc;
         char *const abase = (char *)S.args.p;
         d_all = (const FilterArgs *)(abase + up[0].at);
@@ -1552,8 +1548,6 @@
         d_la[0] = (const ListScanArgs *)(abase + up[4].at);
         d_la[1] = (const ListScanArgs *)(abase + up[5].at);
         S.res_cols.p = abase + up[6].at;
-        c_plan = (uint32_t *)(abase + a_cplan);
-        l_plan = (uint32_t *)(abase + a_lplan);
         if (up_bytes) {
             const uint32_t slot = S.arg_next++ % Scratch::kArgSlots;
             if (S.arg_pending[slot]) HIP_TRY(hipEventSynchronize(S.arg_ev[slot]));
diff --git a/pingoo_amd/csrc/kernels.h b/pingoo_amd/csrc/kernels.h
--- a/pingoo_amd/csrc/kernels.h
+++ b/pingoo_amd/csrc/kernels.h
@@ -53,6 +53,7 @@
 static constexpr uint32_t kListThreads = 512;
 static constexpr uint32_t kListWalks = 1;
 static constexpr uint32_t kListHotBytes = 48 * 1024;
+static constexpr uint32_t kListPlanBytes = 2112;
 struct ListScanArgs {
     const uint8_t *data;
     const uint32_t *off;
@@ -138,8 +139,11 @@
 struct ConfirmTableDev {
     const ConfirmArgs *c;
     uint32_t count;
-};
-int launch_confirm(const ConfirmArgs *host, uint32_t count, const ConfirmArgs *dev, uint32_t *plan, uint32_t n_cus, void *stream);
+#ifdef PWAF_PROFILING
+    unsigned long long *stamps;
+#endif
+};
+int launch_confirm(const ConfirmArgs *host, uint32_t count, const ConfirmArgs *dev, uint32_t n_cus, void *stream);
 
 static constexpr uint32_t kStreamSlab = 128 * 1024;
 static constexpr uint32_t kStreamIter = 4096;
@@ -180,6 +184,9 @@
 struct FilterTable {
     const FilterArgs *f;
     uint32_t count;
+#ifdef PWAF_PROFILING
+    unsigned long long *stamps;
+#endif
 };
 struct FilterMix {
     const FilterArgs *f1, *f2;
@@ -351,13 +358,16 @@
     const ListScanArgs *g;
     uint32_t count;
     uint32_t debug;
+#ifdef PWAF_PROFILING
+    unsigned long long *stamps;
+#endif
 };
 struct ListShape {
     uint32_t threads, hot_bytes, wg_per_cu;
 };
 ListShape list_shape(uint32_t variant);
 uint32_t list_hot_bytes(const ListShape &shape);
-int launch_scan_gated(const ListScanArgs *host, uint32_t count, const ListScanArgs *dev, uint32_t *plan, const ListShape &shape, void *stream);
+int launch_scan_gated(const ListScanArgs *host, uint32_t count, const ListScanArgs *dev, const ListShape &shape, void *stream);
 int launch_verdict(const VerdictArgs &a, void *stream);
 int launch_ipres(const VerdictArgs &a, void *stream);
 int launch_attr(const VerdictArgs &a, void *stream);
diff --git a/pingoo_amd/csrc/kernels.hip b/pingoo_amd/csrc/kernels.hip
--- a/pingoo_amd/csrc/kernels.hip
+++ b/pingoo_amd/csrc/kernels.hip
@@ -1,10 +1,12 @@
 #include <hip/hip_runtime.h>
 
 #include <cstdlib>
+#include <cstring>
 #include <mutex>
 #include <set>
 
 #include "confirm.h"
+#include "plan.h"
 #include "utf8.h"
 #include "kernels.h"
 #include "residual.h"
@@ -417,6 +419,49 @@
 template <int CH, bool WIDE>
 __global__ __launch_bounds__(kScanThreads) void scan_kernel(ScanArgs a) { scan_body<CH, WIDE>(a); }
 
+#ifdef PWAF_PROFILING
+static constexpr uint32_t kStampPoints = 6, kStampWgs = 1024, kStampRing = 16;
+enum : uint32_t { kStampEntry = 0, kStampDescriptor = 1, kStampStaged = 2, kStampFirstInputs = 3, kStampItemsDone = 4, kStampFlushDone = 5 };
+enum : uint32_t { kStampResolve = 0, kStampConfirm = 1, kStampListScan = 2 };
+struct StampLaunch { uint32_t kind, count, grid, seq; };
+static std::mutex g_stamp_mu;
+static unsigned long long *g_stamp_dev = nullptr;
+static StampLaunch g_stamp_meta[kStampRing];
+static uint32_t g_stamp_seq = 0;
+static unsigned long long *stamp_slot(uint32_t kind, uint32_t count, uint32_t grid, hipStream_t stream) {
+    static const bool on = getenv("PWAF_STAMPS") != nullptr;
+    if (!on) return nullptr;
+    std::lock_guard<std::mutex> lock(g_stamp_mu);
+    const size_t slot_words = (size_t)kStampWgs * kStampPoints;
+    if (g_stamp_dev == nullptr && hipMalloc((void **)&g_stamp_dev, kStampRing * slot_words * 8) != hipSuccess) return nullptr;
+    const uint32_t slot = g_stamp_seq % kStampRing;
+    unsigned long long *const p = g_stamp_dev + slot * slot_words;
+    if (hipMemsetAsync(p, 0, slot_words * 8, stream) != hipSuccess) return nullptr;
+    g_stamp_meta[slot] = StampLaunch{kind, count, grid, ++g_stamp_seq};
+    return p;
+}
+__device__ __forceinline__ void stamp(unsigned long long *s, const uint32_t point) {
+    if (s != nullptr && threadIdx.x == 0 && blockIdx.y == 0 && blockIdx.x < kStampWgs) s[blockIdx.x * kStampPoints + point] = (unsigned long long)wall_clock64();
+}
+__device__ __forceinline__ void stamp_once(unsigned long long *s, const uint32_t point, uint32_t &done, const bool wait_loads = false) {
+    if (done & (1u << point)) return;
+    done |= 1u << point;
+    if (wait_loads && s != nullptr) asm volatile("s_waitcnt vmcnt(0)" ::: "memory");
+    stamp(s, point);
+}
+#define PWAF_STAMP_STATE uint32_t stamps_done = 0
+#define PWAF_STAMP(tab, point) stamp((tab).stamps, point)
+#define PWAF_STAMP_ONCE(tab, point) stamp_once((tab).stamps, point, stamps_done)
+#define PWAF_STAMP_LOADED(tab, point) stamp_once((tab).stamps, point, stamps_done, true)
+#define PWAF_STAMP_SLOT(tab, kind, count, grid, stream) (tab).stamps = stamp_slot(kind, count, grid, (hipStream_t)(stream))
+#else
+#define PWAF_STAMP_STATE ((void)0)
+#define PWAF_STAMP(tab, point) ((void)0)
+#define PWAF_STAMP_ONCE(tab, point) ((void)0)
+#define PWAF_STAMP_LOADED(tab, point) ((void)0)
+#define PWAF_STAMP_SLOT(tab, kind, count, grid, stream) ((void)0)
+#endif
+
 __device__ __forceinline__ ListOf list_of(const ListScanArgs &a) {
     ListOf l{a.req_list, a.req_list != nullptr ? min(*a.n_list, a.n) : a.n};
     if (a.dense_mode != 0u) {
@@ -428,35 +473,49 @@
     return l;
 }
 
-__global__ __launch_bounds__(256) void lscan_plan_kernel(GatedTable b, uint32_t *plan , uint32_t n_waves) {
-    __shared__ uint32_t part[256];
-    __shared__ unsigned long long all_entries;
+__device__ __forceinline__ void plan_scan(const uint32_t items, uint32_t *prefix , uint32_t *wsum ) {
+    const uint32_t t = threadIdx.x, lane = t & 63u;
+    uint32_t incl = items;
+#pragma unroll
+    for (uint32_t d = 1; d < 64; d <<= 1) {
+        const uint32_t v = __shfl_up(incl, d);
+        if (lane >= d) incl += v;
+    }
+    if (t < plan::kMaxDescriptors && lane == 63u) wsum[t >> 6] = incl;
+    __syncthreads();
+    if (t < plan::kMaxDescriptors) {
+        uint32_t base = 0;
+        for (uint32_t w = 0; w < (t >> 6); w++) base += wsum[w];
+        prefix[t] = base + incl - items;
+        if (t == plan::kMaxDescriptors - 1u) prefix[plan::kMaxDescriptors] = base + incl;
+    }
+    __syncthreads();
+}
+
+struct ListPlan {
+    unsigned long long wave_entries[4];
+    uint32_t wsum[4];
+    uint32_t prefix[plan::kMaxDescriptors + 1];
+    uint32_t pad[3];
+    uint32_t epi[plan::kMaxDescriptors];
+};
+static_assert(sizeof(ListPlan) == kListPlanBytes, "the list scan's plan scratch is sized by kernels.h");
+__device__ __forceinline__ void lscan_plan(const GatedTable &b, ListPlan *ws, const uint32_t n_waves) {
     const uint32_t t = threadIdx.x;
+    const uint32_t n_l = t < b.count ? list_of(b.g[t]).n_l : 0u;
+    unsigned long long sum = n_l;
+#pragma unroll
+    for (uint32_t d = 32; d != 0; d >>= 1) sum += __shfl_xor(sum, d);
+    if (t < plan::kMaxDescriptors && (t & 63u) == 0u) ws->wave_entries[t >> 6] = sum;
+    __syncthreads();
     uint32_t items = 0;
-    const uint32_t n_l = t < b.count ? list_of(b.g[t]).n_l : 0u;
-    if (t == 0) all_entries = 0ull;
-    __syncthreads();
-    if (n_l != 0u) atomicAdd(&all_entries, (unsigned long long)n_l);
-    __syncthreads();
     if (t < b.count) {
-        const uint32_t room = n_waves > b.count ? n_waves - b.count : 1u;
-        const unsigned long long per_wave = (all_entries + room - 1u) / room;
-        uint32_t epi = 1;
-        while (epi < 16u && epi < per_wave) epi <<= 1;
-        while (epi < 64u * kListWalks && (n_l + epi - 1) / epi > n_waves) epi <<= 1;
-        items = (n_l + epi - 1) / epi;
-        plan[b.count + 1 + t] = epi;
-    }
-    part[t] = items;
-    __syncthreads();
-    for (uint32_t d = 1; d < 256; d <<= 1) {
-        const uint32_t v = t >= d ? part[t - d] : 0u;
-        __syncthreads();
-        part[t] += v;
-        __syncthreads();
-    }
-    if (t < b.count) plan[t] = part[t] - items;
-    if (t == 0) plan[b.count] = part[255];
+        const unsigned long long all_entries = ws->wave_entries[0] + ws->wave_entries[1] + ws->wave_entries[2] + ws->wave_entries[3];
+        const uint32_t epi = plan::lscan_epi(n_l, all_entries, b.count, n_waves, 64u * kListWalks);
+        items = plan::lscan_items(n_l, epi);
+        ws->epi[t] = epi;
+    }
+    plan_scan(items, ws->prefix, ws->wsum);
 }
 
 __device__ __forceinline__ uint32_t list_step_slow(const uint16_t *hot, const PWAF_GLOBAL uint16_t *flat, const uint64_t *delta, const uint32_t state, const uint32_t c,
@@ -582,25 +641,26 @@
 }
 
 template <uint32_t THREADS>
-__global__ __launch_bounds__(THREADS, THREADS == 512 ? 6 : 4) void lscan_kernel(GatedTable b, const uint32_t *plan, uint32_t hot_bytes) {
+__global__ __launch_bounds__(THREADS, THREADS == 512 ? 6 : 4) void lscan_kernel(GatedTable b, uint32_t hot_bytes) {
     extern __shared__ uint32_t lscan_lds[];
     __builtin_amdgcn_s_setprio(3);
     if ((uint32_t)(uintptr_t)(PWAF_LDS unsigned char *)lscan_lds != 0u) __builtin_trap();
-    const uint32_t total = plan[b.count];
-    const uint32_t it0 = (uint32_t)((uint64_t)total * blockIdx.x / gridDim.x), it1 = (uint32_t)((uint64_t)total * (blockIdx.x + 1) / gridDim.x);
+    PWAF_STAMP_STATE;
+    PWAF_STAMP(b, kStampEntry);
+    ListPlan *const lp = reinterpret_cast<ListPlan *>(lscan_lds + (hot_bytes + 16u + 256u) / 4);
+    lscan_plan(b, lp, gridDim.x * (THREADS / 64u));
+    const uint32_t *const prefix = lp->prefix;
+    const uint32_t total = prefix[b.count];
+    uint32_t it0, it1;
+    plan::wg_range(total, blockIdx.x, gridDim.x, it0, it1);
     const unsigned char *cls = reinterpret_cast<const unsigned char *>(lscan_lds + (hot_bytes + 16u) / 4);
     const uint16_t *hot = reinterpret_cast<const uint16_t *>(lscan_lds);
     for (uint32_t it = it0; it < it1;) {
-        uint32_t ps = 0;
-        for (uint32_t lo = 0, hi = b.count; lo + 1 < hi;) {
-            const uint32_t mid = (lo + hi) >> 1;
-            if (plan[mid] <= it) lo = mid;
-            else hi = mid;
-            ps = lo;
-        }
-        const uint32_t first = plan[ps], it_end = min(it1, plan[ps + 1]), epi = plan[b.count + 1 + ps];
+        const uint32_t ps = plan::pass_of(prefix, b.count, it);
+        const uint32_t first = prefix[ps], it_end = min(it1, prefix[ps + 1]), epi = lp->epi[ps];
         ListScanArgs a = load_descriptor(&b.g[ps]);
         const ListOf lst = list_of(a);
+        PWAF_STAMP_ONCE(b, kStampDescriptor);
         a.req_list = lst.req_list;
         const uint32_t ncls = a.n_classes, stride = ncls + 3u;
         const uint32_t hot_elems = a.n_hot * stride;
@@ -624,6 +684,7 @@
         __syncthreads();
         if (threadIdx.x == 0) reinterpret_cast<uint16_t *>(lscan_lds)[hot_elems] = 0xFFFFu;
         __syncthreads();
+        PWAF_STAMP_ONCE(b, kStampStaged);
         const uint32_t n_l = lst.n_l;
 #ifdef PWAF_PROFILING
         const bool long_list = (b.debug & 1u) ? false : (b.debug & 2u) ? true : (a.behind_filter != 0u && (uint64_t)n_l * 8u >= a.n);
@@ -632,6 +693,7 @@
 #endif
         if (long_list) {
             lscan_async<THREADS>(a, hot, cls, delta_lds, it, it_end, first, n_l, hot_elems, epi);
+            PWAF_STAMP(b, kStampItemsDone);
             it = it_end;
             continue;
         }
@@ -667,6 +729,7 @@
                 if (live[u] && a.emit_off[1] != a.emit_off[0]) h[u] = emit_list(a.emit_off, a.emit_list, a.pool, a.pool_count, a.status, a.pool_cap, 0u, h[u]);
                 w[u] = *reinterpret_cast<const PWAF_GLOBAL u32x4_u *>(gdata + p[u]);
             }
+            PWAF_STAMP_LOADED(b, kStampFirstInputs);
             auto record_emit = [&](const uint32_t st, Hits &hh) {
                 const uint32_t ei = st * stride + ncls;
                 const uint32_t code = ei < hot_elems ? (uint32_t)hot[ei] : (uint32_t)flat[ei];
@@ -774,29 +837,13 @@
                 }
             }
         }
+        PWAF_STAMP(b, kStampItemsDone);
         it = it_end;
     }
-}
-
-__global__ __launch_bounds__(256) void confirm_plan_kernel(ConfirmTableDev b, uint32_t *plan ) {
-    __shared__ uint32_t part[256];
-    const uint32_t t = threadIdx.x;
-    uint32_t items = 0;
-    if (t < b.count) {
-        const ConfirmArgs *pa = &b.c[t];
-        const bool dense = pa->dense_flag != nullptr && *pa->dense_flag > pa->dense_thresh;
-        items = dense ? 0u : (min(*pa->pair_count, pa->pair_cap) + kConfirmThreads - 1) / kConfirmThreads;
-    }
-    part[t] = items;
+#ifdef PWAF_PROFILING
     __syncthreads();
-    for (uint32_t d = 1; d < 256; d <<= 1) {
-        const uint32_t v = t >= d ? part[t - d] : 0u;
-        __syncthreads();
-        part[t] += v;
-        __syncthreads();
-    }
-    if (t < b.count) plan[t] = part[t] - items;
-    if (t == 0) plan[b.count] = part[255];
+#endif
+    PWAF_STAMP(b, kStampFlushDone);
 }
 
 __device__ __noinline__ void merge_atom(PoolEntry *pool, uint32_t *pool_count, uint32_t *status, uint32_t pool_cap, uint32_t *rec, uint32_t atom) {
@@ -837,25 +884,35 @@
     }
 }
 
-__global__ __launch_bounds__(kConfirmThreads, 8) void confirm_kernel(ConfirmTableDev b, const uint32_t *plan) {
+__global__ __launch_bounds__(kConfirmThreads, 8) void confirm_kernel(ConfirmTableDev b) {
     __shared__ uint32_t head[kFilterEntries], ftab[kFilterEntries];
     __shared__ uint32_t pool[kConfirmPoolBytes / 4];
     constexpr uint32_t kConfirmQueue = 1024;
     __shared__ uint32_t app_cnt, app_base, app_queue[kConfirmQueue];
+    __shared__ uint32_t prefix[plan::kMaxDescriptors + 1], plan_wsum[4];
     __builtin_amdgcn_s_setprio(3);
+    PWAF_STAMP_STATE;
+    PWAF_STAMP(b, kStampEntry);
     if (threadIdx.x == 0) app_cnt = 0;
-    const uint32_t total = plan[b.count];
-    const uint32_t it0 = (uint32_t)((uint64_t)total * blockIdx.x / gridDim.x), it1 = (uint32_t)((uint64_t)total * (blockIdx.x + 1) / gridDim.x);
+    {
+        uint32_t items = 0;
+        if (threadIdx.x < b.count) {
+            const ConfirmArgs *pa = &b.c[threadIdx.x];
+            const uint32_t *const pc = pa->pair_count, *const df = pa->dense_flag;
+            const uint32_t cap = pa->pair_cap, thresh = pa->dense_thresh;
+            const uint32_t pairs = *pc, flag = df != nullptr ? *df : 0u;
+            items = plan::confirm_items(pairs, cap, df != nullptr, flag, thresh, kConfirmThreads);
+        }
+        plan_scan(items, prefix, plan_wsum);
+    }
+    const uint32_t total = prefix[b.count];
+    uint32_t it0, it1;
+    plan::wg_range(total, blockIdx.x, gridDim.x, it0, it1);
     for (uint32_t it = it0; it < it1;) {
-        uint32_t ps = 0;
-        for (uint32_t lo = 0, hi = b.count; lo + 1 < hi;) {
-            const uint32_t mid = (lo + hi) >> 1;
-            if (plan[mid] <= it) lo = mid;
-            else hi = mid;
-            ps = lo;
-        }
-        const uint32_t first_item = plan[ps], it_end = min(it1, plan[ps + 1]);
+        const uint32_t ps = plan::pass_of(prefix, b.count, it);
+        const uint32_t first_item = prefix[ps], it_end = min(it1, prefix[ps + 1]);
         const ConfirmArgs a = load_descriptor(&b.c[ps]);
+        PWAF_STAMP_ONCE(b, kStampDescriptor);
         __syncthreads();
         {
             const uint4 *sh = reinterpret_cast<const uint4 *>(a.c_head), *sf = reinterpret_cast<const uint4 *>(a.ftable);
@@ -884,6 +941,7 @@
             t_classes = pool + e_words + b_words;
         }
         __syncthreads();
+        PWAF_STAMP_ONCE(b, kStampStaged);
         const ConfirmView cv{nullptr, t_entries, t_bytes, t_classes, a.mul, a.stride, a.init};
         const uint32_t n_p = min(*a.pair_count, a.pair_cap);
         auto pair_of = [&](const uint32_t item) -> uint2 {
@@ -897,6 +955,7 @@
             confirm_load64(reinterpret_cast<const uint8_t *>(a.off + pr_next.x), fs_next, fe_next);
             tb_next = confirm_chunk_bytes(a.data, pr_next.y, a.total + PWAF_ARENA_PAD);
         }
+        PWAF_STAMP_LOADED(b, kStampFirstInputs);
         for (; it < it_end; it++) {
             const uint2 pr = pr_next;
             const bool live = pr.x != kNone;
@@ -970,6 +1029,7 @@
             }
         }
         __syncthreads();
+        PWAF_STAMP(b, kStampItemsDone);
         {
             const uint32_t queued = min(app_cnt, kConfirmQueue);
             if (threadIdx.x == 0 && queued != 0) app_base = atomicAdd(a.walk_count, queued);
@@ -979,6 +1039,7 @@
             if (threadIdx.x == 0) app_cnt = 0;
         }
     }
+    PWAF_STAMP(b, kStampFlushDone);
 }
 
 int launch_scan(const ScanArgs &a, void *stream) {
@@ -1017,40 +1078,34 @@
     return (int)hipGetLastError();
 }
 
-int launch_confirm(const ConfirmArgs *host, uint32_t count, const ConfirmArgs *dev, uint32_t *plan, uint32_t n_cus, void *stream) {
+int launch_confirm(const ConfirmArgs *host, uint32_t count, const ConfirmArgs *dev, uint32_t n_cus, void *stream) {
     if (count == 0 || host[0].n == 0) return 0;
-    if (count > 256) return (int)hipErrorInvalidValue;
+    if (count > plan::kMaxDescriptors) return (int)hipErrorInvalidValue;
     ConfirmTableDev b{dev, count};
-    hipLaunchKernelGGL(confirm_plan_kernel, dim3(1), dim3(256), 0, (hipStream_t)stream, b, plan);
-    hipError_t e = hipGetLastError();
-    if (e != hipSuccess) return (int)e;
     uint64_t max_items = 0;
     for (uint32_t k = 0; k < count; k++) max_items += ((uint64_t)host[k].pair_cap + kConfirmThreads - 1) / kConfirmThreads;
     const uint32_t blocks = (uint32_t)std::min<uint64_t>(max_items, (uint64_t)std::max(1u, n_cus) * 2u);
-    const uint32_t *cplan = plan;
-    hipLaunchKernelGGL(confirm_kernel, dim3(blocks), dim3(kConfirmThreads), 0, (hipStream_t)stream, b, cplan);
+    PWAF_STAMP_SLOT(b, kStampConfirm, count, blocks, stream);
+    hipLaunchKernelGGL(confirm_kernel, dim3(blocks), dim3(kConfirmThreads), 0, (hipStream_t)stream, b);
     return (int)hipGetLastError();
 }
 
 static const void *lscan_fn(bool wide) { return wide ? reinterpret_cast<const void *>(lscan_kernel<1024>) : reinterpret_cast<const void *>(lscan_kernel<512>); }
 
-int launch_scan_gated(const ListScanArgs *host, uint32_t count, const ListScanArgs *dev, uint32_t *plan, const ListShape &shape, void *stream) {
+int launch_scan_gated(const ListScanArgs *host, uint32_t count, const ListScanArgs *dev, const ListShape &shape, void *stream) {
     if (count == 0 || host[0].n == 0) return 0;
-    if (count > 256) return (int)hipErrorInvalidValue;
+    if (count > plan::kMaxDescriptors) return (int)hipErrorInvalidValue;
     GatedTable b{dev, count, 0u};
 #ifdef PWAF_PROFILING
     static const uint32_t async_mode = getenv("PWAF_LSCAN_ASYNC") ? (uint32_t)atoi(getenv("PWAF_LSCAN_ASYNC")) : 0u;
     b.debug = async_mode;
 #endif
     const uint32_t blocks = std::max(1u, host[0].n_cus) * shape.wg_per_cu;
-    hipLaunchKernelGGL(lscan_plan_kernel, dim3(1), dim3(256), 0, (hipStream_t)stream, b, plan, blocks * (shape.threads / 64u));
-    hipError_t e = hipGetLastError();
-    if (e != hipSuccess) return (int)e;
-    const uint32_t *cplan = plan;
+    PWAF_STAMP_SLOT(b, kStampListScan, count, blocks, stream);
     uint32_t hot_bytes = list_hot_bytes(shape);
-    void *args[] = {&b, &cplan, &hot_bytes};
+    void *args[] = {&b, &hot_bytes};
     const void *fn = lscan_fn(shape.threads == 1024);
-    e = hipLaunchKernel(fn, dim3(blocks), dim3(shape.threads), args, shape.hot_bytes + 16 + 256, (hipStream_t)stream);
+    const hipError_t e = hipLaunchKernel(fn, dim3(blocks), dim3(shape.threads), args, shape.hot_bytes + 16 + 256 + kListPlanBytes, (hipStream_t)stream);
     return (int)(e != hipSuccess ? e : hipGetLastError());
 }
 
@@ -1379,6 +1434,7 @@
     void *args[] = {&t};
     const char *forced = getenv("PWAF_RESOLVE_PARTS");
     const bool split = forced ? atoi(forced) == 4 : all_slabs < 4096u;
+    PWAF_STAMP_SLOT(t, kStampResolve, count, split ? max_slabs : (max_slabs + 3) / 4, stream);
     hipError_t e = split ? hipLaunchKernel(reinterpret_cast<const void *>(resolve_kernel<4>), dim3(max_slabs, count), dim3(256), args, 0, (hipStream_t)stream)
                          : hipLaunchKernel(reinterpret_cast<const void *>(resolve_kernel<1>), dim3((max_slabs + 3) / 4, count), dim3(256), args, 0, (hipStream_t)stream);
     return (int)(e != hipSuccess ? e : hipGetLastError());
@@ -1530,6 +1586,8 @@
     constexpr uint32_t kChunks = kStreamSlab / 16, kWords = kChunks / 32;
     constexpr uint32_t kResolveSparse = 128;
     __shared__ uint32_t s_bits[4][kWords], s_rank[4][kWords];
+    PWAF_STAMP_STATE;
+    PWAF_STAMP(B, kStampEntry);
     const FilterArgs *pa = &B.f[blockIdx.y];
     if ((uint64_t)(pa->slab0 + blockIdx.x * 4 / PARTS) * kStreamSlab >= pa->total) return;
     const FilterArgs a = load_descriptor(pa);
@@ -1538,6 +1596,7 @@
     constexpr uint32_t kPartChunks = kChunks / PARTS;
     if ((uint64_t)slab * kStreamSlab >= a.total) return;
     const uint32_t cnt = a.sub_count[rel];
+    PWAF_STAMP_ONCE(B, kStampDescriptor);
     if (cnt == 0) return;
     const bool sparse = a.pairs != nullptr && cnt <= kResolveSparse;
     if (sparse && part != 0u) return;
@@ -1562,6 +1621,7 @@
         }
     }
     __builtin_amdgcn_fence(__ATOMIC_ACQ_REL, "wavefront");
+    PWAF_STAMP_ONCE(B, kStampStaged);
     auto rank_of = [&](const uint32_t c) {
         if (c >= kChunks) return rank[kWords - 1] + (uint32_t)__builtin_popcount(bits[kWords - 1]);
         return rank[c >> 5] + (uint32_t)__builtin_popcount(bits[c >> 5] & ((1u << (c & 31u)) - 1u));
@@ -1587,6 +1647,7 @@
     const uint64_t b1 = slab_b0 + (uint64_t)hi_c * 16u;
     const uint32_t pair_base = a.pairs != nullptr ? a.pair_base[rel] : 0u;
     const uint32_t begin = __builtin_amdgcn_readfirstlane(a.off[0]);
+    PWAF_STAMP_LOADED(B, kStampFirstInputs);
     if (part == 0 && a.pairs != nullptr && (uint64_t)begin > slab_b0) {
         const uint32_t n_before = min((uint32_t)(((uint64_t)begin - slab_b0) >> 4), kChunks);
         for (uint32_t w = lane; w * 32u < n_before; w += 64) {
@@ -1638,7 +1699,10 @@
                 if (steps == 48u) redo = true;
             }
         }
-        if (__ballot(redo) == 0ull) return;
+        if (__ballot(redo) == 0ull) {
+            PWAF_STAMP(B, kStampFlushDone);
+            return;
+        }
     }
     {
     uint32_t s_n = 0xFFFFFFFFu, e_n = 0xFFFFFFFFu;
@@ -1702,6 +1766,7 @@
         if (__ballot(live && (uint64_t)s >= b1 + 16) != 0) break;
     }
     }
+    PWAF_STAMP(B, kStampFlushDone);
 }
 
 __global__ __launch_bounds__(256) void compact_kernel(FilterTable B) {
@@ -3403,3 +3468,20 @@
 }
 
 }
+
+#ifdef PWAF_PROFILING
+extern "C" int pwaf_prof_stamps_read(uint32_t *dims, uint32_t *meta, unsigned long long *out) {
+    using namespace pwaf;
+    dims[0] = kStampRing;
+    dims[1] = kStampWgs;
+    dims[2] = kStampPoints;
+    if (meta == nullptr || out == nullptr) return 0;
+    std::lock_guard<std::mutex> lock(g_stamp_mu);
+    hipError_t e = hipDeviceSynchronize();
+    if (e != hipSuccess) return (int)e;
+    memcpy(meta, g_stamp_meta, sizeof g_stamp_meta);
+    const size_t bytes = (size_t)kStampRing * kStampWgs * kStampPoints * 8;
+    if (g_stamp_dev == nullptr) { memset(out, 0, bytes); return 0; }
+    return (int)hipMemcpy(out, g_stamp_dev, bytes, hipMemcpyDeviceToHost);
+}
+#endif
diff --git a/pingoo_amd/csrc/plan.h b/pingoo_amd/csrc/plan.h
--- /dev/null
+++ b/pingoo_amd/csrc/plan.h
@@ -0,0 +1,56 @@
+#pragma once
+#include <stdint.h>
+
+#if defined(__HIPCC__) || defined(__CUDACC__)
+#define PWAF_PLAN_FN __host__ __device__ inline
+#else
+#define PWAF_PLAN_FN inline
+#endif
+
+namespace pwaf {
+namespace plan {
+
+static constexpr uint32_t kMaxDescriptors = 256;
+
+PWAF_PLAN_FN uint32_t confirm_items(uint32_t pair_count, uint32_t pair_cap, bool has_flag, uint32_t flag, uint32_t thresh, uint32_t per_item) {
+    if (has_flag && flag > thresh) return 0u;
+    const uint32_t n = pair_count < pair_cap ? pair_count : pair_cap;
+    return (n + per_item - 1u) / per_item;
+}
+
+PWAF_PLAN_FN uint32_t lscan_epi(uint32_t n_l, uint64_t all_entries, uint32_t count, uint32_t n_waves, uint32_t epi_max) {
+    const uint32_t room = n_waves > count ? n_waves - count : 1u;
+    const uint64_t per_wave = (all_entries + room - 1u) / room;
+    uint32_t epi = 1u;
+    while (epi < 16u && epi < per_wave) epi <<= 1;
+    while (epi < epi_max && (n_l + epi - 1u) / epi > n_waves) epi <<= 1;
+    return epi;
+}
+PWAF_PLAN_FN uint32_t lscan_items(uint32_t n_l, uint32_t epi) { return (n_l + epi - 1u) / epi; }
+
+PWAF_PLAN_FN uint32_t pass_of(const uint32_t *prefix, uint32_t count, uint32_t it) {
+    uint32_t lo = 0u, hi = count;
+    while (lo + 1u < hi) {
+        const uint32_t mid = (lo + hi) >> 1;
+        if (prefix[mid] <= it) lo = mid;
+        else hi = mid;
+    }
+    return lo;
+}
+
+PWAF_PLAN_FN void wg_range(uint32_t total, uint32_t b, uint32_t g, uint32_t &it0, uint32_t &it1) {
+    it0 = (uint32_t)((uint64_t)total * b / g);
+    it1 = (uint32_t)((uint64_t)total * (b + 1u) / g);
+}
+
+inline void prefix_sums(const uint32_t *items, uint32_t count, uint32_t *prefix ) {
+    uint32_t acc = 0u;
+    for (uint32_t d = 0; d < count; d++) {
+        prefix[d] = acc;
+        acc += items[d];
+    }
+    prefix[count] = acc;
+}
+
+}
+}
```
